# Cogito2012/OpenTAL

Hardware: AMD Instinct MI355X
Metric: clips/sec training step, 256-frame THUMOS14 clips (higher is better)
Workload: dtype bf16

## Files before the change

include/opental_hip.h:

```cpp
#ifndef OPENTAL_HIP_H
#define OPENTAL_HIP_H

#include <stdint.h>
#include <stddef.h>

#ifdef __cplusplus
extern "C" {
#endif

#define OTAL_ABI_VERSION 26

#define OTAL_E_NULL      (-1)
#define OTAL_E_SHAPE     (-2)
#define OTAL_E_ODD_C     (-3)
#define OTAL_E_BATCH     (-4)
#define OTAL_E_DTYPE     (-5)
#define OTAL_E_LEVELS    (-6)
#define OTAL_E_UNSUPPORTED (-7)

#define OTAL_F32  0
#define OTAL_BF16 1
#define OTAL_F16  2
#define OTAL_F64  3

#define OTAL_MAX_LEVELS 8

int otal_abi_version(void);
const char* otal_error_string(int code);
int otal_set_option(const char* name, int value);
int otal_get_option(const char* name, int dflt);
int otal_stream_wait(void* waiter, void* signaler);

int otal_bmp_fwd(const void* in, const float* seg, void* out,
                 int B, int C, int T, int N, int seg_batch, int dtype, void* stream);

int otal_bmp_bwd(const void* grad_out, const void* in, const float* seg, void* grad_in,
                 int B, int C, int T, int N, int seg_batch, int compat_ref_stride,
                 int dtype, void* stream);

int otal_bmp_fwd_levels(const void* in, const float* seg, void* out,
                        int B, int C, int nlev, const int* t_start, const int* n_start,
                        int dtype, void* stream);
int otal_bmp_bwd_levels(const void* grad_out, const void* in, const float* seg, void* grad_in,
                        int B, int C, int nlev, const int* t_start, const int* n_start,
                        int dtype, void* stream);

int otal_conv_half_storage(const int* geom, const int64_t* strides, int mode, int precision);
size_t otal_conv_workspace_bytes(const int* geom, int mode);

int otal_conv_fwd(const int* geom, const int64_t* strides, const float* x, const float* w,
                  const float* scale, const float* shift, float* y, int relu, int precision,
                  const void* prologue, void* ws, size_t ws_bytes, void* stream);

int otal_conv_dgrad(const int* geom, const int64_t* strides, const float* dy, const float* wt_packed,
                    float* dx, int accumulate, const float* out_mask, const float* out_scale,
                    int precision, const void* prologue, void* ws, size_t ws_bytes, void* stream);

int otal_conv_wgrad(const int* geom, const int64_t* strides, const float* x, const float* dy,
                    float* dw, int accumulate, int precision, const void* prologue, void* ws, size_t ws_bytes,
                    void* stream);

int otal_conv_fwd_pair(const int* geom, const int64_t* strides, const float* const* x, const float* const* w,
                       const float* const* scale, const float* const* shift, float* const* y, int relu, int precision,
                       const void* const* prologue, void* ws, size_t ws_bytes, void* stream);
int otal_conv_dgrad_pair(const int* geom, const int64_t* strides, const float* const* dy, const float* const* w,
                         float* const* dx, int precision, const void* const* prologue, void* ws, size_t ws_bytes, void* stream);
int otal_conv_wgrad_pair(const int* geom, const int64_t* strides, const float* const* x, const float* const* dy,
                         float* const* dw, int precision, void* ws, size_t ws_bytes, void* stream);

size_t otal_conv_prologue_bytes(const int* geom, const int64_t* strides, int mode, int precision);
size_t otal_conv_prologue_desc_bytes(void);
int otal_conv_prologue(const int* geom, const int64_t* strides, int mode, const float* w, int precision, void* region,
                       size_t region_bytes, void* host_desc, void* stream);
int otal_conv_prologue_batch(int n, const void* device_descs, const int* device_starts, int total_blocks, void* stream);

int otal_conv_defer_reduces(int on);
size_t otal_conv_deferred_end(void);
int otal_conv_deferred_count(void);
int otal_conv_flush_reduces(void* stream);

const char* otal_conv_last_kernel(void);

int otal_conv_pack_wt(const float* w, float* wt, int Cout, int Cin, int kvol, void* stream);

int otal_gn_relu_fwd(const float* x, const float* gamma, const float* beta, float* y, float* stats,
                     int B, int C, int T, int G, float eps, int relu, int nlev, const int* lev, void* stream);
int otal_gn_relu_bwd(const float* dy, int64_t dy_batch_stride, const float* x, const float* gamma, const float* beta,
                     const float* stats, float* dx, float* partial, int B, int C, int T, int G,
                     int relu, int nlev, const int* lev, void* stream);
int otal_gn_relu_fwd_pair(const float* const* x, const float* const* gamma, const float* const* beta, float* const* y,
                          float* const* stats, int B, int C, int T, int G, float eps, int relu, int nlev, const int* lev,
                          void* stream);
int otal_gn_relu_bwd_pair(const float* const* dy, const int64_t* dy_batch_stride, const float* const* x,
                          const float* const* gamma, const float* const* beta, const float* const* stats, float* const* dx,
                          float* const* partial, int B, int C, int T, int G, int relu, int nlev, const int* lev, void* stream);
int otal_sum_partials(int n_items, const float* const* partial, float* const* dst0, float* const* dst1,
                      float* const* dst2, const int* channels, const int* batches, void* stream);

const char* otal_layer_last_kernel(void);

int otal_maxpool3d_fwd(const int* geom, const int64_t* strides, const float* x, float* y,
                       unsigned char* argtap, void* stream);
int otal_maxpool3d_bwd(const int* geom, const int64_t* strides, const float* dy,
                       const unsigned char* argtap, float* dx, int accumulate,
                       const float* out_mask, const float* out_scale, void* stream);
size_t otal_maxpool3d_signbits_bytes(const int* geom, const int64_t* strides);
int otal_maxpool3d_fwd_signbits(const int* geom, const int64_t* strides, const float* x, float* y,
                                unsigned char* argtap, unsigned char* signbits, void* stream);
int otal_maxpool3d_bwd_signbits(const int* geom, const int64_t* strides, const float* dy, const unsigned char* argtap,
                                float* dx, int accumulate, const unsigned char* signbits, const float* out_scale,
                                void* stream);
int otal_maxpool3d_fwd_signbits_h(const int* geom, const int64_t* strides, const void* x_bf16, float* y,
                                  unsigned char* argtap, unsigned char* signbits, void* stream);
int otal_maxpool3d_bwd_signbits_h(const int* geom, const int64_t* strides, const float* dy, const unsigned char* argtap,
                                  void* dx_bf16, const unsigned char* signbits, const float* out_scale, void* stream);
int otal_maxpool3d_fwd_io(const int* geom, const int64_t* strides, const void* x, void* y, unsigned char* argtap,
                          unsigned char* signbits, int io, void* stream);
int otal_maxpool3d_bwd_io(const int* geom, const int64_t* strides, const void* dy, const unsigned char* argtap, void* dx,
                          int accumulate, const void* out_mask, const float* out_scale, const unsigned char* signbits, int io,
                          void* stream);
int otal_convert_storage(const void* src, int64_t src_bs, int64_t src_cs, void* dst, int64_t dst_bs, int64_t dst_cs,
                         int to_bf16, int B, int C, int P, void* stream);

int otal_head_outputs_fwd(int n_items, const int* channels, const int* modes, const float* const* raw, float* const* out,
                          float* const* unct, const float* scales, int B, int N, int nlev, const int* lev,
                          const float* level_strides, void* stream);
int otal_head_outputs_bwd(int n_items, const int* channels, const int* modes, const float* const* raw,
                          const float* const* out, const float* const* unct, const float* const* dout,
                          const float* const* dunct, float* const* draw, const float* scales, float* dscales, int B,
                          int N, int nlev, const int* lev, const float* level_strides, void* stream);

int otal_boundary_bce(const float* x, int64_t x_batch_stride, int64_t x_channel_stride, const float* mask,
                      int64_t mask_batch_stride, int64_t mask_row_stride, int mask_row0, int mask_step, float* terms,
                      float* dx, int B, int C, int T, void* stream);

int otal_boundary_finish(int n, const float* const* terms, const float* weights, const int* T, int B, float* out2, void* stream);
int otal_boundary_scale(int n, const float* const* dx, float* const* out, const float* weights, const int* C, const int* T,
                        int B, const float* g_start, const float* g_end, void* stream);

int otal_proposal_windows(const float* loc, float* seg, float* frame_seg, int B, int nlev,
                          const int* lev, float frame_num, void* stream);

int otal_decode_clips(const float* loc, const float* prop_loc, const float* priors, const float* conf,
                      const float* prop_conf, const float* center, const float* act, const float* prop_act,
                      const float* offsets, const float* fps, float* seg, float* score, float* unct,
                      float* actn, unsigned char* flag, int nclips, int A, int K, float clip_length,
                      float conf_thresh, void* stream);
int otal_decode_clips_ex(const float* loc, const float* prop_loc, const float* priors, const float* conf,
                         const float* prop_conf, const float* center, const float* act, const float* prop_act,
                         const float* offsets, const float* fps, float* seg, float* score, float* unct,
                         float* actn, unsigned char* flag, int nclips, int A, int K, float clip_length,
                         float conf_thresh, int score_fn, int first_class, void* stream);
int otal_softnms_classes(const float* seg, const float* score, const float* unct, const float* actn,
                         const unsigned char* flag, const int* clip_start, int nvideos, int max_clips,
                         int A, int K, float sigma, int top_k, float score_threshold, float* out,
                         int* counts, int* out_index, int out_cols, void* stream);
size_t otal_softnms_scratch_bytes(int total_clips, int max_clips, int A, int K);
int otal_softnms_classes_ws(const float* seg, const float* score, const float* unct, const float* actn,
                            const unsigned char* flag, const int* clip_start, int nvideos, int max_clips,
                            int A, int K, float sigma, int top_k, float score_threshold, float* out,
                            int* counts, int* out_index, int out_cols, void* scratch, size_t scratch_bytes,
                            int total_clips, void* stream);
int otal_detection_table(const float* rows, const int* counts, const double* durations, int V, int K, int top_k, int cols,
                         int drop_empty, int scoring, int* video, int* cls, double* seg, float* sup, double* known,
                         int* list_start, void* stream);

int otal_openmax_dist(const float* feat, int N, int rows_per_batch, int64_t sb, int64_t sr, int64_t sc, const float* mav,
                      int K, int D, const int* labels, float* dist, void* stream);
int otal_openmax_class_means(const float* feat, int N, int rows_per_batch, int64_t sb, int64_t sr, int64_t sc,
                             const int* labels, int K, int D, float* means, int* counts, void* stream);
int otal_openmax_probs(const float* logits, int64_t ldl, const float* feat, int N, int rows_per_batch, int64_t sb, int64_t sr,
                       int64_t sc, const float* mav, const float* wb, int K, int D, int R, float* probs, void* stream);
int otal_decode_clips_openmax(const float* loc, const float* prop_loc, const float* priors, const float* conf,
                              const float* prop_conf, const float* center, const float* offsets, const float* fps,
                              const float* feat, const float* prop_feat, const int64_t* feat_strides,
                              const int64_t* prop_feat_strides, const float* mav, const float* mav_prop, const float* wb,
                              const float* wb_prop, float* seg, float* score, float* unknown, unsigned char* flag,
                              int nclips, int A, int C, int first_class, int D, int R, int refined_feature,
                              float clip_length, float conf_thresh, void* stream);

int otal_head_convs_supported(int n_heads, int n_inputs, const int* in_idx, const int* cout, const int* ksize, int B, int C, int N);
int otal_head_convs_fwd(int n_heads, int n_inputs, const int* in_idx, const int* cout, const int* ksize,
                        const float* const* x, const float* const* w, const float* const* bias, float* const* y, int B, int C,
                        int N, int nlev, const int* lev, void* stream);
int otal_head_convs_bwd(int n_heads, int n_inputs, const int* in_idx, const int* cout, const int* ksize,
                        const float* const* x, const float* const* w, const float* const* dy, float* const* dx,
                        float* const* dw, float* const* db, int B, int C, int N, int nlev, const int* lev, void* stream);
int otal_head_convs_bwd_parts(int n_heads, int n_inputs, const int* in_idx, const int* cout, const int* ksize,
                        const float* const* x, const float* const* w, const float* const* dy, float* const* dx,
                        float* const* dw, float* const* db, int B, int C, int N, int nlev, const int* lev, int parts, void* stream);

int otal_rpl_head_fwd(const float* x, const float* centers, float* dist, int B, int C, int D, int N, void* stream);
int otal_rpl_head_bwd(const float* x, const float* centers, const float* g, float* dx, float* dcenters, int B, int C, int D,
                      int N, int parts, void* stream);

int otal_masked_scale_copy(const float* src, const int64_t* src_strides, const float* z, const int64_t* z_strides,
                           const float* scale, float* dst, const int64_t* dst_strides, int accumulate, int B, int C,
                           int T, int S, void* stream);

int otal_adam_flat(float* p, const float* g, float* m, float* v, int64_t n, float lr, float beta1,
                   float beta2, float eps, float weight_decay, int step, float grad_scale, void* stream);

int otal_adam_flat_dev(float* p, const float* g, float* m, float* v, int64_t n, float lr, float beta1,
                       float beta2, float eps, float weight_decay, const float* bias_corr, float grad_scale,
                       void* stream);

size_t otal_detection_loss_scratch_floats(int B, int K);
size_t otal_detection_loss_grad_floats(int B, int K, int C);
int otal_detection_loss(const float* loc, const float* conf, const float* prop_loc, const float* prop_conf,
                        const float* center, const float* act, const float* prop_act, const float* priors,
                        const float* gt, const unsigned char* gvalid, float* weight_accum, int B, int K, int C, int G,
                        float clip_length, float overlap_thresh, int ibm_active, int num_bins, float momentum,
                        int iou_aware, int cls_mode, float focal_alpha, float* losses, float* grads, float* scratch,
                        void* stream);

int otal_detection_loss_ex(const float* loc, const float* conf, const float* prop_loc, const float* prop_conf,
                           const float* center, const float* act, const float* prop_act, const float* priors,
                           const float* gt, const unsigned char* gvalid, float* weight_accum, int B, int K, int C, int G,
                           float clip_length, float overlap_thresh, int ibm_active, int num_bins, float momentum,
                           int iou_aware, int cls_mode, float focal_alpha, int reweight, float rw_gamma, float* losses,
                           float* grads, float* scratch, void* stream);
// ... 58 lines not shown
```

opental_amd/common/i3d_backbone.py:

```python
import torch
import torch.nn as nn
import torch.nn.functional as F
from torch.autograd import Function

from . import ops
from .layers import MaxPool3dSamePadding

ONE, THREE = (1, 1, 1), (3, 3, 3)
BN_EPS = 1e-3


class Unit3D(nn.Module):

    def __init__(self, in_channels, output_channels, kernel_shape=(1, 1, 1), stride=(1, 1, 1), padding=0,
                 activation_fn=F.relu, use_batch_norm=True, use_bias=False, padding_valid_spatial=False,
                 name='unit_3d'):
        super(Unit3D, self).__init__()
        if not use_batch_norm or use_bias or activation_fn is not F.relu or padding_valid_spatial or padding == -1:
            raise NotImplementedError("backbone Unit3D is conv(no bias) + BN + ReLU with SAME padding")
        self._output_channels = output_channels
        self._kernel_shape = tuple(kernel_shape)
        self._stride = tuple(stride)
        self.name = name
        self.conv3d = nn.Conv3d(in_channels, output_channels, self._kernel_shape, self._stride, padding=0, bias=False)
# ... 301 lines not shown
                    (y, arg), bits = ops.maxpool3d_forward(cur, k, s), None
                tape.append(("pool", k, s, cur, (arg, bits, half_grads.get(si, False)), cur_scale, None))
                cur, cur_scale = y, None
            else:
                _, w0, oc, _ = step
                B, _, T, H, W = cur.shape
                ctot = oc[0] + oc[2] + oc[4] + oc[5]
                o1, o13 = oc[1], oc[1] + oc[3]
                Z = torch.empty((B, o13 + ctot, T, H, W), dtype=cur.dtype, device=cur.device)
                h1, h2, Y = Z[:, :o1], Z[:, o1:o13], Z[:, o13:]
                c1, c2, c3 = oc[0], oc[0] + oc[2], oc[0] + oc[2] + oc[4]
                wf = _fused_weight(weights[w0 + 1].detach(), weights[w0 + 3].detach(), weights[w0].detach())
                scf, shf = _fused_affine(scale, shift, offs, w0)
                ops.conv_forward(cur, wf, ONE, ONE, scale=scf, shift=shf, relu=True, out=Z[:, :o13 + c1])
                lane = ops.branch_lane(cur.device)
                if lane.on:
                    lane.fork()
                    with lane:
                        ops.conv_forward(h2, weights[w0 + 4], THREE, ONE, scale=sc(w0 + 4), shift=sh(w0 + 4), relu=True,
                                         out=Y[:, c2:c3])
                        pm, argm = ops.maxpool3d_forward(cur, THREE, ONE, half_out=chain)
                        ops.conv_forward(pm, weights[w0 + 5], ONE, ONE, scale=sc(w0 + 5), shift=sh(w0 + 5), relu=True,
                                         out=Y[:, c3:])
                    ops.conv_forward(h1, weights[w0 + 2], THREE, ONE, scale=sc(w0 + 2), shift=sh(w0 + 2), relu=True,
                                     out=Y[:, c1:c2])
                    lane.join()
                else:
                    ops.conv_forward(h1, weights[w0 + 2], THREE, ONE, scale=sc(w0 + 2), shift=sh(w0 + 2), relu=True,
                                     out=Y[:, c1:c2])
                    ops.conv_forward(h2, weights[w0 + 4], THREE, ONE, scale=sc(w0 + 4), shift=sh(w0 + 4), relu=True,
                                     out=Y[:, c2:c3])
                    pm, argm = ops.maxpool3d_forward(cur, THREE, ONE, half_out=chain)
                    ops.conv_forward(pm, weights[w0 + 5], ONE, ONE, scale=sc(w0 + 5), shift=sh(w0 + 5), relu=True,
                                     out=Y[:, c3:])
                out_scale = _cat_cached(_OUT_SCALE, scale, w0, [sc(w0), sc(w0 + 2), sc(w0 + 4), sc(w0 + 5)])
                tape.append(("mixed", w0, (c1, c2, c3), cur, h1, h2, pm, argm, Y, cur_scale, (wf, o1, o13), out_scale))
                cur, cur_scale = Y, out_scale
            if name in endpoints:
                if cur.dtype == BF and name not in raw_out:
                    ends = si + 1 == len(plan) or not _step_half_ok(plan[si + 1], cur.shape, weights)
                    if need_grad or ends:
                        leave_half()
                        found[name] = (cur, len(tape))
                    else:
                        found[name] = (ops.convert_storage(cur, torch.float32), len(tape))
                else:
                    found[name] = (cur, len(tape))
                hooks = ops.STEP.endpoint_hooks
                hook = hooks.get(name) if hooks else None
                if hook is not None:
                    hook(found[name][0])
        missing = [e for e in endpoints if e not in found]
        if missing:
            raise RuntimeError(f"unknown endpoints {missing}")
        ctx.tape = tape
        ctx.meta = (scale, offs, [found[e][1] for e in endpoints], len(weights), x.requires_grad)
        ctx.weights = weights
        ctx.outs = [found[e][0] for e in endpoints]
        return tuple(ctx.outs)

    @staticmethod
    def backward(ctx, *douts):
        tape, weights = ctx.tape, ctx.weights
        scale, offs, out_pos, nw, need_dx = ctx.meta
        sc = lambda i: scale[offs[i]:offs[i + 1]]
        dws = [None] * nw
        pending = {}
        for pos, g, z in zip(out_pos, douts, ctx.outs):
            if g is not None:
                pending.setdefault(pos, []).append((g, z, tape[pos - 1][-1]))
        zg = {}

        def out_grad_buffer(p, shape, like):
            if p >= 1 and tape[p - 1][0] == "mixed":
                o13 = tape[p - 1][10][2]
                B, ct, T, H, W = shape
                buf = torch.empty((B, o13 + ct, T, H, W), dtype=like.dtype, device=like.device)
                zg[p] = buf
                return buf[:, o13:]
            return torch.empty(tuple(shape), dtype=like.dtype, device=like.device)

        side = ops.side_wgrads(weights[0].device)
        in_slots = True
        dcur = None
        cloned = True
        mixed_pos = [p for p in range(1, len(tape) + 1) if tape[p - 1][0] == "mixed"]
        tail_below = min(mixed_pos) if mixed_pos and not need_dx else 0
        for pos in range(len(tape), 0, -1):
            if pos == tail_below - 1 and not any(pending.get(q) for q in range(1, pos + 1)):
                ops.late_mark([weights[st[1]] for st in tape[:pos] if st[0] == "conv"])
            for g, z, zs in pending.pop(pos, ()):
                ops.join_pending(g)
                dense = g.dim() == 5 and (g.shape[4] == 1 or g.stride(4) == 1) and (g.shape[3] == 1 or g.stride(3) == g.shape[4])
                if zs is not None and not dense:
                    g = g.contiguous()
                if dcur is None:
                    if zs is not None:
                        dcur = out_grad_buffer(pos, g.shape, g)
                        ops.masked_scale_copy(g, z, zs, dcur)
                    elif tape[pos - 1][0] == "mixed":
                        dcur = out_grad_buffer(pos, g.shape, g)
                        dcur.copy_(g)
                    else:
                        dcur = g.contiguous()
                        cloned = False
                elif zs is not None:
                    ops.masked_scale_copy(g, z, zs, dcur, accumulate=True)
                else:
                    if not cloned:
                        dcur, cloned = dcur.clone(), True
                    dcur.add_(g)
            if dcur is None:
                continue
            step = tape[pos - 1]
            first = pos == 1
            if step[0] == "cvt":
                _, xh, _, _ = step
                dcur = ops.convert_storage(dcur.contiguous(), xh.dtype, out=out_grad_buffer(pos - 1, xh.shape, xh))
            elif step[0] == "conv":
                _, wi, k, s, xin, y, in_scale, _ = step
                slot = ops.grad_slot(weights[wi])
                in_slots = in_slots and slot is not None
                if first and not need_dx:
                    side.issue()
                    dws[wi] = ops.conv_wgrad(xin, dcur, weights[wi].shape, k, s, out=slot)
                else:
                    dws[wi] = side.wgrad(xin, dcur, weights[wi].shape, k, s, out=slot)
                if first and not need_dx:
                    dcur = None
                else:
                    dcur = ops.conv_dgrad(dcur, weights[wi], xin.shape, k, s, out=out_grad_buffer(pos - 1, xin.shape, xin),
                                          out_mask=xin if in_scale is not None else None, out_scale=in_scale)
                side.flush()
                ops.grads_ready([(weights[wi], dws[wi])])
            elif step[0] == "pool":
                _, k, s, xin, (arg, bits, grad_half), in_scale, _ = step
                if dcur.dtype == torch.bfloat16:
                    masked = in_scale is not None and bits is not None
                    dcur = ops.maxpool3d_backward(dcur, arg, xin.shape, k, s, out=out_grad_buffer(pos - 1, xin.shape, xin),
                                                  out_scale=in_scale if masked else None, out_signbits=bits if masked else None)
                elif grad_half:
                    dcur = ops.maxpool3d_backward(dcur, arg, xin.shape, k, s, out_scale=in_scale, out_signbits=bits, half_out=True)
                else:
                    dcur = ops.maxpool3d_backward(dcur, arg, xin.shape, k, s, out=out_grad_buffer(pos - 1, xin.shape, dcur),
                                                  out_mask=xin if (in_scale is not None and bits is None) else None,
                                                  out_scale=in_scale, out_signbits=bits)
            else:
                _, w0, (c1, c2, c3), xin, h1, h2, pm, argm, Y, in_scale, (wf, o1, o13), _ = step
                Zg = zg.pop(pos)
                dY = Zg[:, o13:]
                dX = out_grad_buffer(pos - 1, xin.shape, xin)
                xm = xin if in_scale is not None else None
                sl = (slice(0, c1), slice(c1, c2), slice(c2, c3), slice(c3, Y.shape[1]))
                for a, b, hid, sli, dst in ((w0 + 1, w0 + 2, h1, sl[1], Zg[:, :o1]), (w0 + 3, w0 + 4, h2, sl[2], Zg[:, o1:o13])):
                    g = dY[:, sli]
                    slot = ops.grad_slot(weights[b])
                    in_slots = in_slots and slot is not None
                    dws[b] = side.wgrad(hid, g, weights[b].shape, THREE, ONE, out=slot)
                    ops.conv_dgrad(g, weights[b], hid.shape, THREE, ONE, out=dst, out_mask=hid, out_scale=sc(a))
                gf = Zg[:, :o13 + c1]
                slot = ops.grad_slot(wf)
                in_slots = in_slots and slot is not None
                dwf = side.wgrad(xin, gf, wf.shape, ONE, ONE, out=slot)
                dws[w0 + 1], dws[w0 + 3], dws[w0] = dwf[:o1], dwf[o1:o13], dwf[o13:]
                ops.conv_dgrad(gf, wf, xin.shape, ONE, ONE, out=dX, out_mask=xm, out_scale=in_scale)
                g3 = dY[:, sl[3]]
                slot = ops.grad_slot(weights[w0 + 5])
                in_slots = in_slots and slot is not None
                dws[w0 + 5] = side.wgrad(pm, g3, weights[w0 + 5].shape, ONE, ONE, out=slot)
                dpm = ops.conv_dgrad(g3, weights[w0 + 5], pm.shape, ONE, ONE)
                ops.maxpool3d_backward(dpm, argm, xin.shape, THREE, ONE, out=dX, accumulate=True,
                                       out_mask=xm, out_scale=in_scale)
                dcur = dX
                side.flush()
                ops.grads_ready([(weights[w0 + q], dws[w0 + q]) for q in range(6)])
        side.node_end(in_slots)
        ctx.tape = None
        ctx.outs = None
        dx = dcur if need_dx else None
        return (dx, None, None, None, None, None) + tuple(dws)
```

opental_amd/common/ops.py:

```python
import bisect
import ctypes
import os
import warnings

import torch

from .. import _lib as L
from .conv_geom import make_geom

_WORKSPACE = {}
WORKSPACE_BYTES = 192 << 20
WORKSPACE_TOTAL = 512 << 20

CONV_PROFILE = None

CONV_PRECISION = 0
HALF_STORAGE = os.environ.get("OTAL_HALF_STORAGE", "1") != "0"
HALF_ACT_DIRECT = os.environ.get("OTAL_HALF_ACT_DIRECT", "0") != "0"
HALF_CHAIN = os.environ.get("OTAL_HALF_CHAIN", "1") != "0"


def _prof_begin():
    if CONV_PROFILE is None:
        return None
    ev = torch.cuda.Event(enable_timing=True)
    ev.record()
    return ev


def _prof_end(ev, mode, g, problems=1):
    if ev is None:
        return
    end = torch.cuda.Event(enable_timing=True)
    end.record()
    B, Cin, Cout = g[0], g[1], g[2]
    flops = 2.0 * B * Cout * g[6] * g[7] * g[8] * Cin * g[9] * g[10] * g[11] * problems
    CONV_PROFILE.append((mode, flops, ev, end))


def workspace(device, side=False):
    key = (device.type, device.index, side)
    ws = _WORKSPACE.get(key)
    if ws is None:
        ws = torch.empty(WORKSPACE_TOTAL, dtype=torch.uint8, device=device)
        _WORKSPACE[key] = ws
    return ws


class StepState:
    def __init__(self):
        self.lanes = None
        self.slots = None
        self.ready = None
        self.defer_join = False
        self.pending_sums = None
        self.prologues = None
        self.late_weights = None
        self.endpoint_hooks = None
        self.early_results = {}
        self.pending_joins = {}
        self.defer = False
        self.defer_owner = None
        self.ws_cursor = [0, 0, 0, 0]
        self.ws_index = 0
        self.stream = None

    def begin_backward(self, slots, ready, early):
        if self.slots is not None:
            raise RuntimeError("a trainer's backward is already running in this process (one at a time)")
        self.slots, self.ready = slots, ready
        self.defer_join = early
        self.pending_sums = [] if early else None
        defer_reduces(early and CONV_PROFILE is None)

    def end_backward(self):
        self.defer_join = False
        defer_reduces(False)
        flush_pending_sums()
        self.pending_sums = self.slots = self.ready = None

    def reset(self, failed_capture=False):
        self.prologues = None
        self.slots = self.ready = self.pending_sums = None
        self.defer_join = False
        self.late_weights = None
        self.lanes = None
        for sd in _SIDES.values():
            sd.pending.clear()
            sd.keep.clear()
        self.early_results.clear()
        self.pending_joins.clear()
        try:
            defer_reduces(False)
        except RuntimeError:
            if not failed_capture:
                raise


STEP = StepState()


class issue_on:
    __slots__ = ("ws", "stream", "ctx", "saved")

    def __init__(self, ws_index, stream, current=False):
        self.ws, self.stream = ws_index, stream
        self.ctx = torch.cuda.stream(stream) if current else None

    def __enter__(self):
        s = STEP
        self.saved = (s.ws_index, s.stream, L.STREAM_OVERRIDE)
        s.ws_index, s.stream, L.STREAM_OVERRIDE = self.ws, self.stream, self.stream.cuda_stream
        if self.ctx is not None:
            self.ctx.__enter__()
        return self

    def __exit__(self, *exc):
        if self.ctx is not None:
            self.ctx.__exit__(*exc)
        STEP.ws_index, STEP.stream, L.STREAM_OVERRIDE = self.saved
        return False


def _ws_args(device):
    s = STEP
    ws = workspace(device, s.ws_index)
    cur = s.ws_cursor[s.ws_index]
    return ctypes.c_void_p(ws.data_ptr() + cur), ctypes.c_size_t(min(ws.numel() - cur, WORKSPACE_BYTES))


def defer_reduces(on):
    if not on:
        flush_reduces()
    L.check(L.lib().otal_conv_defer_reduces(int(bool(on))), "otal_conv_defer_reduces")
    STEP.defer = bool(on)


def _stream_wait(stream):
    L.check(L.lib().otal_stream_wait(L.stream(), ctypes.c_void_p(stream.cuda_stream)), "otal_stream_wait")


def flush_reduces(wait=True):
    s = STEP
    own = s.defer_owner
    if s.defer and own is not None:
        stream = own[1]
        if stream is None:
            L.check(L.lib().otal_conv_flush_reduces(L.stream()), "otal_conv_flush_reduces")
        else:
            L.check(L.lib().otal_conv_flush_reduces(ctypes.c_void_p(stream.cuda_stream)), "otal_conv_flush_reduces")
            if wait and L.STREAM_OVERRIDE != stream.cuda_stream:
                _stream_wait(stream)
    s.defer_owner = None
    s.ws_cursor[0] = s.ws_cursor[1] = 0


def _after_wgrad(device):
    s = STEP
    lib = L.lib()
    lib.otal_conv_deferred_end.restype = ctypes.c_size_t
    end = int(lib.otal_conv_deferred_end())
    if end:
        i = s.ws_index
        s.defer_owner = (i, s.stream)
        s.ws_cursor[i] = (end - workspace(device, i).data_ptr() + 255) & ~255
        if s.ws_cursor[i] > WORKSPACE_TOTAL - WORKSPACE_BYTES:
            flush_reduces()


WGRAD_STREAM = os.environ.get("OTAL_WGRAD_STREAM", "1") != "0"
_SIDES = {}


class LanePlan:

    def __init__(self, side_stream):
        self.entries = []
        self.pool = None
        self.cur = None
        self.side = side_stream
        self.keep = []
        self.mark_event = None

    def begin_main(self):
        g = torch.cuda.CUDAGraph()
        if self.pool is None:
            self.pool = torch.cuda.graph_pool_handle()
        g.capture_begin(pool=self.pool, capture_error_mode="relaxed")
        self.cur = g
# ... 539 lines not shown


class GradSlots:

    def __init__(self, flat, grad, offsets, numels):
        self.base, self.n, self.grad = flat.data_ptr(), flat.numel(), grad
        self.offsets, self.numels = list(offsets), list(numels)
        self.written = [False] * len(self.offsets)

    def reset(self):
        self.written = [False] * len(self.offsets)

    def take(self, w):
        if w.dtype != torch.float32 or not w.is_contiguous():
            return None
        off = w.data_ptr() - self.base
        if off < 0 or off % 4 or off // 4 + w.numel() > self.n:
            return None
        off //= 4
        i = bisect.bisect_left(self.offsets, off)
        if i == len(self.offsets) or self.offsets[i] != off:
            return None
        j, cur, end = i, off, off + w.numel()
        while j < len(self.offsets) and cur < end:
            cur += self.numels[j]
            j += 1
        if cur != end:
            return None
        if any(self.written[i:j]):
            flush_pending_sums()
            flush_reduces()
            return None
        for q in range(i, j):
            self.written[q] = True
        return self.grad[off:end].view(w.shape)

    def release(self, w):
        off = (w.data_ptr() - self.base) // 4
        i = bisect.bisect_left(self.offsets, off)
        j, cur, end = i, off, off + w.numel()
        while j < len(self.offsets) and cur < end:
            self.written[j] = False
            cur += self.numels[j]
            j += 1


def grads_ready(pairs):
    flush_reduces()
    cb = STEP.ready
    if cb is not None:
        cb(pairs)


def grad_slot(w):
    slots = STEP.slots
    return slots.take(w) if slots is not None and "OTAL_NO_GRAD_SLOTS" not in os.environ else None


def conv_wgrad(x, dy, w_shape, k, s, spatial_valid=False, levels=None, out=None, accumulate=False):
    k, s = _k3(k), _k3(s)
    if levels is not None:
        levels = tuple(levels)
    Cout = w_shape[0]
    half_dy = dy.dtype == torch.bfloat16
    half_x = x.dtype == torch.bfloat16
    if not (half_x or x.dtype == torch.float32) or not (half_dy or dy.dtype == torch.float32) or (half_x and not half_dy):
        raise RuntimeError("conv_wgrad: float32 x with a float32 or bfloat16 dy, or both bfloat16")
    g, ga, sa, pkey, _ = _plan(2, x, dy, Cout, k, s, levels, spatial_valid, "x", "dy")
    if out is None:
        if accumulate:
            raise RuntimeError("accumulate needs an existing buffer")
        out = torch.empty(tuple(w_shape), dtype=torch.float32, device=x.device)
    if not out.is_contiguous():
        raise RuntimeError("dw must be contiguous")
    st = STEP
    if st.defer and (accumulate or (st.defer_owner is not None and st.defer_owner[0] != st.ws_index)):
        flush_reduces()
    wsp, wsn = _ws_args(x.device)
    ev = _prof_begin()
    prec = int(CONV_PRECISION)
    pre = _prologue(2, ga, sa, pkey, x, prec) if (half_x or not half_dy) else None
    L.check(L.lib().otal_conv_wgrad(ga, sa, L.ptr(x), L.ptr(dy), L.ptr(out),
                                    int(accumulate), prec | (4 if half_dy else 0) | (8 if half_x else 0), pre, wsp, wsn, L.stream()),
            "otal_conv_wgrad")
    if st.defer:
        _after_wgrad(x.device)
    _prof_end(ev, "wgrad", g)
    return out


PAIR_LAUNCHES = os.environ.get("OTAL_PAIR_LAUNCHES", "1") != "0"
_VP2 = ctypes.c_void_p * 2


def _pp(a, b):
    return _VP2(a.data_ptr() if a is not None else None, b.data_ptr() if b is not None else None)


def _same_layout(a, b):
    return a.shape == b.shape and a.stride() == b.stride() and a.dtype == b.dtype and a.device == b.device


def conv_forward_pair(xs, ws, k, s, shifts=None, levels=None):
    k, s = _k3(k), _k3(s)
    if levels is not None:
        levels = tuple(levels)
    if not PAIR_LAUNCHES or not (int(CONV_PRECISION) & 1) or not _same_layout(xs[0], xs[1]) or ws[0].shape != ws[1].shape:
        return None
    if xs[0].dtype != torch.float32 or not (ws[0].is_contiguous() and ws[1].is_contiguous()):
        return None
    Cout = ws[0].shape[0]
    outn = _out_positions(xs[0], Cout, k, s, levels, False)
    ys = [torch.empty((x.shape[0], Cout) + outn[:1], dtype=x.dtype, device=x.device) for x in xs]
    g, ga, sa, pkey, _ = _plan(0, xs[0], ys[0], Cout, k, s, levels, False, "x", "y")
    prec = int(CONV_PRECISION)
    pres = [_prologue(0, ga, sa, pkey, w, prec) for w in ws]
    if (pres[0] is None) != (pres[1] is None):
        return None
    wsp, wsn = _ws_args(xs[0].device)
    ev = _prof_begin()
    sh = None if shifts is None or shifts[0] is None else _pp(shifts[0], shifts[1])
    rc = L.lib().otal_conv_fwd_pair(ga, sa, _pp(*xs), _pp(*ws), None, sh, _pp(*ys), 0, prec,
                                    None if pres[0] is None else _VP2(pres[0].value, pres[1].value), wsp, wsn, L.stream())
    if rc == L.E_UNSUPPORTED:
        return None
    L.check(rc, "otal_conv_fwd_pair")
    _prof_end(ev, "fwd", g, 2)
    return ys


def conv_dgrad_pair(dys, ws, x_shape, k, s, levels=None):
    k, s = _k3(k), _k3(s)
    if levels is not None:
        levels = tuple(levels)
    if not PAIR_LAUNCHES or not (int(CONV_PRECISION) & 1) or not _same_layout(dys[0], dys[1]) or ws[0].shape != ws[1].shape:
        return None
    if dys[0].dtype != torch.float32 or not (ws[0].is_contiguous() and ws[1].is_contiguous()):
        return None
    Cout = ws[0].shape[0]
    outs = [torch.empty(tuple(x_shape), dtype=dy.dtype, device=dy.device) for dy in dys]
    g, ga, sa, pkey, _ = _plan(1, outs[0], dys[0], Cout, k, s, levels, False, "dx", "dy")
    prec = int(CONV_PRECISION) | 2
    pres = [_prologue(1, ga, sa, pkey, w, prec) for w in ws]
    if (pres[0] is None) != (pres[1] is None):
        return None
    wsp, wsn = _ws_args(dys[0].device)
    ev = _prof_begin()
    rc = L.lib().otal_conv_dgrad_pair(ga, sa, _pp(*dys), _pp(*ws), _pp(*outs), prec,
                                      None if pres[0] is None else _VP2(pres[0].value, pres[1].value), wsp, wsn, L.stream())
    if rc == L.E_UNSUPPORTED:
        return None
    L.check(rc, "otal_conv_dgrad_pair")
    _prof_end(ev, "dgrad", g, 2)
    return outs


def conv_wgrad_pair(xs, dys, w_shape, k, s, levels=None, outs=(None, None)):
    k, s = _k3(k), _k3(s)
    if levels is not None:
        levels = tuple(levels)
    if not PAIR_LAUNCHES or not (int(CONV_PRECISION) & 1) or not _same_layout(xs[0], xs[1]) or not _same_layout(dys[0], dys[1]):
        return None
    if xs[0].dtype != torch.float32 or dys[0].dtype != torch.float32:
        return None
    Cout = w_shape[0]
    g, ga, sa, pkey, _ = _plan(2, xs[0], dys[0], Cout, k, s, levels, False, "x", "dy")
    outs = [o if o is not None else torch.empty(tuple(w_shape), dtype=torch.float32, device=xs[0].device) for o in outs]
    if not (outs[0].is_contiguous() and outs[1].is_contiguous()):
        return None
    st = STEP
    if st.defer and st.defer_owner is not None and st.defer_owner[0] != st.ws_index:
        flush_reduces()
    wsp, wsn = _ws_args(xs[0].device)
    ev = _prof_begin()
    rc = L.lib().otal_conv_wgrad_pair(ga, sa, _pp(*xs), _pp(*dys), _pp(*outs), int(CONV_PRECISION), wsp, wsn, L.stream())
    if rc == L.E_UNSUPPORTED:
        return None
    L.check(rc, "otal_conv_wgrad_pair")
    if st.defer:
        _after_wgrad(xs[0].device)
    _prof_end(ev, "wgrad", g, 2)
    return outs


def gn_relu_forward_pair(xs, gammas, betas, groups=32, eps=1e-5, relu=True, levels=None, outs=None):
    if not PAIR_LAUNCHES or not _same_layout(xs[0], xs[1]) or not xs[0].is_contiguous():
        return None
    L.require_device(*xs, *gammas, *betas)
    B, C, T = xs[0].shape
    nlev, lev = _lev_arg(levels)
    stats = [torch.empty((B, groups, nlev, 2), dtype=torch.float32, device=x.device) for x in xs]
    if outs is not None:
        st0, st1 = _dest_strides(outs[0], B, C, T), _dest_strides(outs[1], B, C, T)
        if st0 != st1:
            return None
        rc = L.lib().otal_gn_relu_fwd_pair_to(_pp(*xs), _pp(*gammas), _pp(*betas), _pp(*outs), ctypes.c_int64(st0[0]),
                                              ctypes.c_int64(st0[1]), _pp(*stats), B, C, T, groups, ctypes.c_float(eps), int(relu),
                                              nlev, lev, L.stream())
        if rc == L.E_UNSUPPORTED:
            return None
        L.check(rc, "otal_gn_relu_fwd_pair_to")
        return list(zip(outs, stats))
    ys = [torch.empty_like(x) for x in xs]
    rc = L.lib().otal_gn_relu_fwd_pair(_pp(*xs), _pp(*gammas), _pp(*betas), _pp(*ys), _pp(*stats), B, C, T, groups,
                                       ctypes.c_float(eps), int(relu), nlev, lev, L.stream())
    if rc == L.E_UNSUPPORTED:
        return None
    L.check(rc, "otal_gn_relu_fwd_pair")
    return list(zip(ys, stats))


def _lev_arg(levels):
    if levels is None or len(levels) <= 2:
        return 1, None
    return len(levels) - 1, L.int_array(list(levels))


def _dest_strides(out, B, C, T):
    if tuple(out.shape) != (B, C, T) or out.dtype != torch.float32 or not out.is_cuda or (T > 1 and out.stride(2) != 1):
        raise RuntimeError("gn_relu_forward: `out` must be a float32 (B,C,T) GPU tensor with dense positions")
    cs = out.stride(1) if C > 1 else T
    return (out.stride(0) if B > 1 else cs * C), cs


def gn_relu_forward(x, gamma, beta, groups=32, eps=1e-5, relu=True, levels=None, out=None):
    L.require_device(x, gamma, beta)
    B, C, T = x.shape
    nlev, lev = _lev_arg(levels)
    stats = torch.empty((B, groups, nlev, 2), dtype=torch.float32, device=x.device)
    if out is not None:
        bs, cs = _dest_strides(out, B, C, T)
        L.check(L.lib().otal_gn_relu_fwd_to(L.ptr(x), L.ptr(gamma), L.ptr(beta), L.ptr(out), ctypes.c_int64(bs), ctypes.c_int64(cs),
                                            L.ptr(stats), B, C, T, groups, ctypes.c_float(eps), int(relu), nlev, lev, L.stream()),
                "otal_gn_relu_fwd_to")
        return out, stats
    y = torch.empty_like(x)
    L.check(L.lib().otal_gn_relu_fwd(L.ptr(x), L.ptr(gamma), L.ptr(beta), L.ptr(y), L.ptr(stats), B, C, T, groups,
                                     ctypes.c_float(eps), int(relu), nlev, lev, L.stream()), "otal_gn_relu_fwd")
    return y, stats


def pyramid_merge_forward(p0, p1, total, up):
    L.require_device(p0, p1)
    B, C, t0 = p0.shape
    if tuple(p1.shape) != (B, C, t0 // 2):
        raise RuntimeError("pyramid_merge_forward: p1 must have half of p0's positions")
    packed = torch.empty((B, C, total), dtype=torch.float32, device=p0.device)
    frame = torch.empty((B, C, t0 * up), dtype=torch.float32, device=p0.device)
    L.check(L.lib().otal_pyramid_merge_fwd(L.ptr(p0), L.ptr(p1), L.ptr(packed), L.ptr(frame), B, C, t0, total, up, L.stream()),
            "otal_pyramid_merge_fwd")
    return packed, frame


def pyramid_merge_backward(da, db, dframe, dnext, t0, up):
    L.require_device(da, dframe)
    B, C, T = da.shape
    dp0 = torch.empty((B, C, t0), dtype=torch.float32, device=da.device)
    dp1 = torch.empty((B, C, t0 // 2), dtype=torch.float32, device=da.device)
    for t in (db, dnext):
        if t is not None:
            L.require_device(t)
    L.check(L.lib().otal_pyramid_merge_bwd(L.ptr(da), _opt(db), L.ptr(dframe), _opt(dnext), L.ptr(dp0), L.ptr(dp1), B, C, t0, T, up,
                                           L.stream()), "otal_pyramid_merge_bwd")
    return dp0, dp1


def gn_relu_backward(dy, x, gamma, beta, stats, groups=32, relu=True, levels=None, bias=None):
    B, C, T = x.shape
    if dy.dim() != 3 or tuple(dy.shape) != (B, C, T) or dy.stride(2) != 1 or dy.stride(1) != T or dy.stride(0) < C * T:
        dy = dy.contiguous()
    L.require_device(x, gamma, beta, stats)
    if not dy.is_cuda:
        raise RuntimeError("opental_amd ops run on the GPU only")
    nlev, lev = _lev_arg(levels)
    dx = torch.empty_like(x)
    partial = torch.empty((B, 3, C), dtype=torch.float32, device=x.device)
    L.check(L.lib().otal_gn_relu_bwd(L.ptr(dy), ctypes.c_int64(dy.stride(0)), L.ptr(x), L.ptr(gamma), L.ptr(beta), L.ptr(stats),
                                     L.ptr(dx), L.ptr(partial), B, C, T, groups, int(relu), nlev, lev, L.stream()),
            "otal_gn_relu_bwd")
    return (dx,) + _gn_sums(partial, gamma, beta, bias, C, B)


def _gn_sums(partial, gamma, beta, bias, C, B):
    s = STEP
    if s.pending_sums is not None and bias is not None and s.slots is not None:
        slots = [s.slots.take(t) for t in (gamma, beta, bias)]
        if all(sl is not None for sl in slots):
            s.pending_sums.append((partial, tuple(sl.data_ptr() for sl in slots), C, B))
            return slots[0], slots[1], slots[2]
        for t, sl in zip((gamma, beta, bias), slots):
            if sl is not None:
                s.slots.release(t)
    red = partial.sum(0)
    return red[0], red[1], red[2]


def gn_relu_backward_pair(dys, xs, gammas, betas, stats, groups=32, relu=True, levels=None, biases=(None, None)):
    if not PAIR_LAUNCHES or not _same_layout(xs[0], xs[1]):
        return None
    B, C, T = xs[0].shape
    dys = list(dys)
    for i in range(2):
        dy = dys[i]
        if dy.dim() != 3 or tuple(dy.shape) != (B, C, T) or dy.stride(2) != 1 or dy.stride(1) != T or dy.stride(0) < C * T:
            dys[i] = dy.contiguous()
        if not dys[i].is_cuda:
# ... 687 lines not shown
```

opental_amd/csrc/conv_gemm.hip:

```cpp
#include "common.h"
#include "conv_index.h"
#include "conv_select.h"
#include <cstdlib>
#include <cstring>
#include <mutex>
#include <type_traits>

#ifndef OTAL_CONV_PART
#define OTAL_CONV_PART 0
#endif

#include "conv1a_tile.h"
namespace otal_conv {
struct ConvArgs;
__attribute__((visibility("hidden"))) int launch_half(int mode, int kernel, int cw, ConvArgs& a, void* ws, size_t ws_bytes, hipStream_t st);
}

namespace {

constexpr int NT = 256;
enum { EPI_RELU = 1, EPI_ACCUM = 2, NO_STORE = 8, NO_BARRIER = 16, EPI_NPAD8 = 32 };

typedef float f32x16 __attribute__((ext_vector_type(16)));

}
struct otal_conv::ConvArgs {
    ConvGeom g;
    ConvFastDiv fd;
    const float* x;
    const float* w;
    const float* dy;
    float* out;
    const float* scale;
    const float* shift;
    float* slab;
    const float* zero;
    const int2* tab;
    const float* emask;
    const float* escale;
    int M, N, K;
    int splits, k_per_split;
    int flags;
    int a_vec4;
    int prec;
    const int2* ctab;
    const unsigned short* wp;
    unsigned src_bytes;
    unsigned wp_bytes;
    int Kp;
    const int2* ptab;
    unsigned dy_bytes;
    int P;
    int w_natural;
    unsigned out_bytes, slab_bytes;
    const void* pre;
    int half;
    int pair;
    const float* x2;
    const float* dy2;
    float* out2;
    const float* scale2;
    const float* shift2;
    const unsigned short* wp2;
    float* slab2;
    const void* pre2;
    const float* w2;
    int xhalf, mhalf;
};
namespace {
using otal_conv::ConvArgs;

__device__ __attribute__((aligned(16))) float g_zero4[4] = {0.f, 0.f, 0.f, 0.f};

__device__ __forceinline__ float ld_or_zero(const float* base, int64_t off, bool ok) {
    const float* p = ok ? base + off : g_zero4;
    return *p;
}

struct Anchor {
    const float* base;
    unsigned mask;
};
__device__ __forceinline__ Anchor anchor_of_output(const ConvGeom& g, const float* x, const PosDec& o, bool live) {
    const int t0 = o.t * g.st - g.pt, h0 = o.h * g.sh - g.ph, w0 = o.w * g.sw - g.pw;
    int lo, up;
    level_bounds(g, o.t, g.Ti, lo, up);
    unsigned m = 0;
#pragma unroll
    for (int d = 0; d < 8; ++d) {
        m |= (unsigned)(d < g.kt && t0 + d >= lo && t0 + d < up) << d;
        m |= (unsigned)(d < g.kh && (unsigned)(h0 + d) < (unsigned)g.Hi) << (8 + d);
        m |= (unsigned)(d < g.kw && (unsigned)(w0 + d) < (unsigned)g.Wi) << (16 + d);
    }
    Anchor r;
    r.base = x + ((int64_t)o.b * g.x_bs + ((int64_t)t0 * g.Hi + h0) * g.Wi + w0);
    r.mask = live ? m : 0u;
    return r;
}
__device__ __forceinline__ Anchor anchor_of_input(const ConvGeom& g, const float* dy, const PosDec& i, bool live) {
    const int tn = i.t + g.pt, hn = i.h + g.ph, wn = i.w + g.pw;
    const int st1 = g.st - 1, sh1 = g.sh - 1, sw1 = g.sw - 1;
    int lo, up;
    level_bounds(g, i.t, g.Ti, lo, up);
    if (g.nlev <= 1) { lo = 0; up = g.To; }
    unsigned m = 0;
#pragma unroll
    for (int d = 0; d < 8; ++d) {
        const int vt = tn - d, vh = hn - d, vw = wn - d;
        m |= (unsigned)(d < g.kt && vt >= 0 && (vt & st1) == 0 && (vt >> st1) >= lo && (vt >> st1) < up) << d;
        m |= (unsigned)(d < g.kh && vh >= 0 && (vh & sh1) == 0 && (vh >> sh1) < g.Ho) << (8 + d);
        m |= (unsigned)(d < g.kw && vw >= 0 && (vw & sw1) == 0 && (vw >> sw1) < g.Wo) << (16 + d);
    }
    Anchor r;
    r.base = dy + ((int64_t)i.b * g.y_bs + ((int64_t)(tn >> st1) * g.Ho + (hn >> sh1)) * g.Wo + (wn >> sw1));
    r.mask = live ? m : 0u;
    return r;
}
__device__ __forceinline__ bool tap_ok(unsigned mask, int dt, int dh, int dw) {
    return ((mask >> dt) & (mask >> (8 + dh)) & (mask >> (16 + dw)) & 1u) != 0;
}
__device__ __forceinline__ float ld_sel(const float* p, bool ok, const float* zero) {
    const float* q = ok ? p : zero;
    return *q;
}

typedef short bf16x8 __attribute__((ext_vector_type(8)));
struct Words4 { unsigned a, b, c, d; };
struct Words2 { unsigned a, b; };
__device__ __forceinline__ unsigned wrap_add(unsigned a, unsigned b) {
    unsigned r = a + b;
    asm volatile("" : "+v"(r));
    return r;
}
typedef __bf16 hw_bf16x2 __attribute__((ext_vector_type(2)));
typedef float hw_f32x2 __attribute__((ext_vector_type(2)));
__device__ __forceinline__ unsigned cvt_pk_bf16(float lo, float hi) {
    const hw_f32x2 f = {lo, hi};
    return __builtin_bit_cast(unsigned, __builtin_convertvector(f, hw_bf16x2));
}

__device__ __forceinline__ unsigned pair_lo(unsigned ch_a, unsigned ch_b) { return __builtin_amdgcn_perm(ch_b, ch_a, 0x05040100u); }
__device__ __forceinline__ unsigned pair_hi(unsigned ch_a, unsigned ch_b) { return __builtin_amdgcn_perm(ch_b, ch_a, 0x07060302u); }
__device__ __forceinline__ bool bf16_pos(unsigned bits16) { return bits16 - 1u < 0x7f80u; }
__device__ __forceinline__ unsigned bf16_relu_mask2(unsigned w) {
    return (bf16_pos(w & 0xffffu) ? 0x0000ffffu : 0u) | (bf16_pos(w >> 16) ? 0xffff0000u : 0u);
}
__device__ __forceinline__ float bf16lo_f32(unsigned w) { return __uint_as_float(w << 16); }
__device__ __forceinline__ float bf16hi_f32(unsigned w) { return __uint_as_float(w & 0xffff0000u); }

__device__ __forceinline__ unsigned pack_bf16x2(float lo, float hi) {
    unsigned a = __float_as_uint(lo), b = __float_as_uint(hi);
    a += 0x7fffu + ((a >> 16) & 1u);
    b += 0x7fffu + ((b >> 16) & 1u);
    return (a >> 16) | (b & 0xffff0000u);
}

template <int MODE, int WM, int WN>
__device__ __forceinline__ void store_acc_slow(const ConvArgs& a, const f32x16 (&acc)[WM][WN], int m0, int n0, int wm0, int wn0,
                                               int lane, int split) {
    const ConvGeom& g = a.g;
    const ConvFastDiv& fd = a.fd;
#pragma unroll
    for (int j = 0; j < WN; ++j) {
        const int n = n0 + wn0 + j * 32 + (lane & 31);
        if (n >= a.N) continue;
        int64_t nbase = 0;
        if (a.splits == 1) {
            if constexpr (MODE == MODE_FWD) nbase = conv_out_offset(g, dec_pos_fd(n, fd.To, fd.Ho, fd.Wo), 0);
// ... 1566 lines not shown
    int item = 0;
#pragma unroll 1
    while (item + 1 < DEFER_MAX && b.start[item + 1] <= (int)blockIdx.x) ++item;
    const DeferItem& d = b.it[item];
    const int wg = (int)blockIdx.x - b.start[item];
    const int lane = threadIdx.x & 63, q = threadIdx.x >> 6;
    const int64_t base = ((int64_t)wg * 64 + lane) * 4;
    const bool live = base < d.total;
    const int per = (d.splits + 3) / 4;
    const int s_lo = q * per, s_hi = min(d.splits, s_lo + per);
    float4 acc = make_float4(0.f, 0.f, 0.f, 0.f);
    if (live) {
        for (int s0 = s_lo; s0 < s_hi; s0 += 8) {
            float4 tmp[8];
#pragma unroll
            for (int u = 0; u < 8; ++u) {
                const int sidx = min(s0 + u, s_hi - 1);
                tmp[u] = *reinterpret_cast<const float4*>(d.slab + (int64_t)sidx * d.total + base);
            }
#pragma unroll
            for (int u = 0; u < 8; ++u)
                if (s0 + u < s_hi) { acc.x += tmp[u].x; acc.y += tmp[u].y; acc.z += tmp[u].z; acc.w += tmp[u].w; }
        }
    }
    if (q > 0) part[q - 1][lane] = acc;
    __syncthreads();
    if (q > 0 || !live) return;
    const float4 p1 = part[0][lane], p2 = part[1][lane], p3 = part[2][lane];
    float r[4] = {(acc.x + p1.x) + (p2.x + p3.x), (acc.y + p1.y) + (p2.y + p3.y), (acc.z + p1.z) + (p2.z + p3.z), (acc.w + p1.w) + (p2.w + p3.w)};
#pragma unroll
    for (int e = 0; e < 4; ++e) {
        const int64_t idx = base + e;
        float v = r[e];
        int64_t off = idx;
        if (d.flags & EPI_NPAD8) {
            const int m = (int)(idx / d.N), n = (int)(idx - (int64_t)m * d.N);
            if ((n & 7) >= d.kw) continue;
            off = (int64_t)m * ((d.N >> 3) * d.kw) + (n >> 3) * d.kw + (n & 7);
        }
        if (d.flags & EPI_ACCUM) v += d.out[off];
        d.out[off] = v;
    }
}

static int flush_deferred(hipStream_t st) {
    std::lock_guard<std::recursive_mutex> lock(g_defer.mu);
    if (g_defer.n == 0) return 0;
    int blocks = 0;
    for (int i = 0; i <= DEFER_MAX; ++i) {
        g_defer.batch.start[i] = blocks;
        if (i < g_defer.n) blocks += (int)((g_defer.batch.it[i].total + 255) / 256);
    }
    hipLaunchKernelGGL(splitk_reduce_batch_kernel, dim3((unsigned)blocks), dim3(256), 0, st, g_defer.batch);
    g_defer.n = 0;
    return otal_launch_status();
}

template <int MODE, bool H = false>
static int launch_splitk_reduce(const ConvArgs& a, hipStream_t st) {
    static_assert(!(H && MODE == MODE_WGRAD), "weight gradients are fp32");
    const int64_t total = (int64_t)a.M * a.N;
    const bool v4 = (total % 4 == 0) && (((uintptr_t)a.slab & 15) == 0);
    if (MODE == MODE_WGRAD) {
        std::lock_guard<std::recursive_mutex> lock(g_defer.mu);
        g_defer.last_end = 0;
        if (g_defer.on && v4 && total <= (1 << 23)) {
            if (g_defer.n == DEFER_MAX)
                if (int e = flush_deferred(st)) return e;
            DeferItem& d = g_defer.batch.it[g_defer.n++];
            d.slab = a.slab; d.out = a.out; d.total = total; d.splits = a.splits; d.flags = a.flags; d.N = a.N; d.kw = a.g.kw;
            g_defer.last_end = reinterpret_cast<uintptr_t>(a.slab + (int64_t)a.splits * total);
            return 0;
        }
    }
    if (v4 && a.splits >= 16 && total <= (1 << 21)) {
        const int blocks = (int)((total / 4 + 63) / 64);
        hipLaunchKernelGGL((splitk_reduce_tall_kernel<MODE, H>), dim3(blocks), dim3(256), 0, st, a);
        return otal_launch_status();
    }
    const int64_t work = v4 ? total / 4 : total;
    const int blocks = (int)((work + 255) / 256 < 4096 ? (work + 255) / 256 : 4096);
    if (v4) hipLaunchKernelGGL((splitk_reduce_kernel<MODE, 4, H>), dim3(blocks), dim3(256), 0, st, a);
    else hipLaunchKernelGGL((splitk_reduce_kernel<MODE, 1, H>), dim3(blocks), dim3(256), 0, st, a);
    return otal_launch_status();
}

__global__ __launch_bounds__(256) void pack_wt_kernel(const float* __restrict__ w, float* __restrict__ wt,
                                                      int Cout, int Cin, int kvol) {
    const int64_t total = (int64_t)Cout * Cin * kvol;
    for (int64_t idx = (int64_t)blockIdx.x * 256 + threadIdx.x; idx < total; idx += (int64_t)gridDim.x * 256) {
        const int r = (int)(idx % kvol);
        const int64_t q = idx / kvol;
        const int co = (int)(q % Cout), ci = (int)(q / Cout);
        wt[idx] = w[((int64_t)co * Cin + ci) * kvol + r];
    }
}

int fill_geom(ConvGeom& g, const int* d) {
    g.B = d[0]; g.Cin = d[1]; g.Cout = d[2];
    g.Ti = d[3]; g.Hi = d[4]; g.Wi = d[5];
    g.To = d[6]; g.Ho = d[7]; g.Wo = d[8];
    g.kt = d[9]; g.kh = d[10]; g.kw = d[11];
    g.st = d[12]; g.sh = d[13]; g.sw = d[14];
    g.pt = d[15]; g.ph = d[16]; g.pw = d[17];
    g.nlev = d[18];
    for (int i = 0; i <= OTAL_CONV_MAX_LEVELS; ++i) g.lev[i] = d[19 + i];
    const int v[] = {g.B, g.Cin, g.Cout, g.Ti, g.Hi, g.Wi, g.To, g.Ho, g.Wo, g.kt, g.kh, g.kw, g.st, g.sh, g.sw};
    for (int x : v) if (x <= 0) return OTAL_E_SHAPE;
    if (g.pt < 0 || g.ph < 0 || g.pw < 0) return OTAL_E_SHAPE;
    if (g.kt > 8 || g.kh > 8 || g.kw > 8) return OTAL_E_UNSUPPORTED;
    if (g.st > 2 || g.sh > 2 || g.sw > 2) return OTAL_E_UNSUPPORTED;
    if (g.nlev > 1) {
        if (g.nlev > OTAL_CONV_MAX_LEVELS || g.Hi != 1 || g.Wi != 1 || g.st != 1 || g.Ti != g.To) return OTAL_E_LEVELS;
        if (g.lev[0] != 0 || g.lev[g.nlev] != g.Ti) return OTAL_E_LEVELS;
        for (int i = 0; i < g.nlev; ++i) if (g.lev[i + 1] <= g.lev[i]) return OTAL_E_LEVELS;
    }
    if ((int64_t)g.Cin * g.Ti * g.Hi * g.Wi >= (1LL << 31) || (int64_t)g.Cout * g.To * g.Ho * g.Wo >= (1LL << 31) ||
        (int64_t)g.Cout * g.Cin * g.kt * g.kh * g.kw >= (1LL << 31)) return OTAL_E_SHAPE;
    if ((int64_t)g.B * g.To * g.Ho * g.Wo >= (1LL << 31) || (int64_t)g.B * g.Ti * g.Hi * g.Wi >= (1LL << 31) ||
        (int64_t)g.Cin * g.kt * g.kh * g.kw >= (1LL << 31) || (int64_t)g.Cout * g.kt * g.kh * g.kw >= (1LL << 31)) return OTAL_E_SHAPE;
    return 0;
}

static const float* zero_word_address() {
    static const float* z = nullptr;
    if (!z) {
        void* p = nullptr;
        if (hipGetSymbolAddress(&p, HIP_SYMBOL(g_zero4)) == hipSuccess) z = static_cast<const float*>(p);
    }
    return z;
}

template <int MODE>
static void set_epilogue_extents(ConvArgs& a) {
    const ConvGeom& g = a.g;
    int64_t out;
    if (MODE == MODE_FWD) out = 4 * ((int64_t)(g.B - 1) * g.y_bs + (int64_t)(g.Cout - 1) * g.y_cs + conv_out_positions(g));
    else if (MODE == MODE_DGRAD) out = 4 * ((int64_t)(g.B - 1) * g.x_bs + (int64_t)(g.Cin - 1) * g.x_cs + conv_in_positions(g));
    else out = 4 * (int64_t)g.Cout * g.Cin * conv_kvol(g);
    a.out_bytes = (out > 0 && out < (int64_t)0xfffffff0u) ? (unsigned)out : 0u;
    const int64_t slab = 4 * (int64_t)a.splits * a.M * a.N;
    a.slab_bytes = (a.splits > 1 && slab < (int64_t)0xfffffff0u) ? (unsigned)slab : 0u;
}

struct DirectArgs {
    ConvArgs c;
    const unsigned short* wp;
    int C, Ktot;
    unsigned wp_bytes;
};

template <int BM, int MODE, int BNP, int WN, int PX = 48, int MINW = 1, bool XPF2 = false, bool H = false>
__global__ __launch_bounds__(BNP * 2 / WN, MINW) void conv3_direct_kernel(const DirectArgs d) {
    constexpr int DNT = BNP * 2 / WN;
    constexpr int WM = BM / 32, PA = 304, SPAN_MAX = BNP + (H ? 56 : 52);
    constexpr int ESZ = H ? 2 : 4, XV = H ? 8 : 4;
    static_assert(PX == 48 || PX == 32, "position pitch");
    constexpr int A_PIECES = (BM * 18 + DNT - 1) / DNT;
    constexpr int X_ITEMS = (SPAN_MAX / XV + 1) * 8;
    constexpr int X_ITERS = (X_ITEMS + DNT - 1) / DNT;
    extern __shared__ __attribute__((aligned(16))) unsigned char dsm[];
    unsigned char* const smA0 = dsm;
    unsigned char* const smX0 = dsm + 2 * BM * PA;
    const unsigned char* const smZero = dsm + 2 * BM * PA + 2 * SPAN_MAX * PX;
    if (threadIdx.x < 4) reinterpret_cast<unsigned*>(dsm + 2 * BM * PA + 2 * SPAN_MAX * PX)[threadIdx.x] = 0u;
    auto smA = [&](int buf) { return smA0 + buf * (BM * PA); };
    auto smX = [&](int buf) { return smX0 + buf * (SPAN_MAX * PX); };
    const ConvArgs& a = d.c;
    const ConvGeom& g = a.g;
    const ConvFastDiv& fd = a.fd;
    const int tid = threadIdx.x, lane = tid & 63;
    const int wave = __builtin_amdgcn_readfirstlane(tid >> 6);
    const TileId tile = xcd_tile(true);
    const int m0 = tile.y * BM, n0 = tile.x * BNP;
    const int W = g.Wi, HW = g.Hi * g.Wi;
    const int XO = H ? W + 2 : W + 1;
    const int span = BNP + XO + W + 1, nq = (span + XV - 1) / XV;
    const float* src = MODE == MODE_FWD ? a.x : a.dy;
    const int64_t sbs = MODE == MODE_FWD ? g.x_bs : g.y_bs, scs = MODE == MODE_FWD ? g.x_cs : g.y_cs;
    const auto rs = __builtin_amdgcn_make_buffer_rsrc(const_cast<float*>(src), 0, (int)a.src_bytes, 0x00020000);
    const auto rw = __builtin_amdgcn_make_buffer_rsrc(const_cast<unsigned short*>(d.wp), 0, (int)d.wp_bytes, 0x00020000);
    const uint32_t bsm = fd_div(fd.P, (uint32_t)n0);
    const int p0 = n0 - (int)(bsm * fd.P.d);
    const unsigned tile_off = (unsigned)(((int64_t)bsm * sbs + p0 - XO) * ESZ);

    unsigned tmask[WN], hwmask[WN];
#pragma unroll
    for (int j = 0; j < WN; ++j) {
        const int nl = n0 + (wave * WN + j) * 32 + (lane & 31);
        const PosDec o = dec_pos_fd(nl < a.N ? nl : 0, fd.To, fd.Ho, fd.Wo);
        const bool live = nl < a.N;
        tmask[j] = 0; hwmask[j] = 0;
#pragma unroll
        for (int dt = 0; dt < 3; ++dt) tmask[j] |= (unsigned)(live && (unsigned)(o.t + dt - 1) < (unsigned)g.Ti) << dt;
#pragma unroll
        for (int dh = 0; dh < 3; ++dh)
#pragma unroll
            for (int dw = 0; dw < 3; ++dw)
                hwmask[j] |= (unsigned)((unsigned)(o.h + dh - 1) < (unsigned)g.Hi && (unsigned)(o.w + dw - 1) < (unsigned)g.Wi) << (dh * 3 + dw);
    }
    unsigned xvo[X_ITERS];
    int xlds[X_ITERS];
#pragma unroll
    for (int i = 0; i < X_ITERS; ++i) {
        const int item = tid + DNT * i;
        const int cp = item & 7, q = item >> 3;
        const bool used = q < nq;
        xvo[i] = used ? tile_off + (unsigned)((2 * cp * scs + XV * q) * ESZ) : 0xffffffffu;
        if constexpr (H)
            xlds[i] = PX == 48 ? (8 * q) * PX + cp * 4 : (8 * q) * PX + ((((cp >> 2) ^ q) & 1) << 4) + (cp & 3) * 4;
        else
            xlds[i] = PX == 48 ? (4 * q) * PX + cp * 4
                               : (4 * q) * PX + ((((cp >> 2) ^ (q >> 1)) & 1) << 4) + (cp & 3) * 4;
    }
    unsigned avo[A_PIECES];
#pragma unroll
    for (int j = 0; j < A_PIECES; ++j) {
        const int p = tid + DNT * j;
        avo[j] = (unsigned)(((m0 + p / 18) * d.Ktot * 2) + (p % 18) * 16);
    }
    unsigned rxs[XPF2 ? 2 : 1][X_ITERS][2][4];
    Words4 ra[A_PIECES];
    const int nsteps = (d.C >> 4) * 3;
    auto load_x = [&](int s, auto SET) {
        unsigned (&rx)[X_ITERS][2][4] = rxs[decltype(SET)::value];
        const int cb = s / 3, dt = s - cb * 3;
        const unsigned so = (unsigned)(((int64_t)cb * 16 * scs + (int64_t)(dt - 1) * HW) * ESZ);
#pragma unroll
        for (int i = 0; i < X_ITERS; ++i) {
            const unsigned vo = xvo[i] == 0xffffffffu ? a.src_bytes : xvo[i] + so;
#pragma unroll
            for (int h = 0; h < 2; ++h) {
                const Words4 v = __builtin_bit_cast(Words4, __builtin_amdgcn_raw_buffer_load_b128(rs, vo, h ? (int)(scs * ESZ) : 0, 0));
                rx[i][h][0] = v.a; rx[i][h][1] = v.b; rx[i][h][2] = v.c; rx[i][h][3] = v.d;
            }
        }
    };
    auto load_a = [&](int s) {
#pragma unroll
        for (int j = 0; j < A_PIECES; ++j)
            if ((BM * 18) % DNT == 0 || tid + DNT * j < BM * 18)
                ra[j] = __builtin_bit_cast(Words4, __builtin_amdgcn_raw_buffer_load_b128(rw, avo[j], s * 288, 0));
    };
    auto store = [&](int buf, int s, auto SET) {
        unsigned (&rx)[X_ITERS][2][4] = rxs[decltype(SET)::value];
        const int cb = s / 3, dt = s - cb * 3;
        const unsigned so = (unsigned)(((int64_t)cb * 16 * scs + (int64_t)(dt - 1) * HW) * ESZ);
#pragma unroll
        for (int i = 0; i < X_ITERS; ++i) {
            if (xvo[i] == 0xffffffffu) continue;
            const unsigned vo = xvo[i] + so;
            const bool neg = vo >= 0xfffffff0u;
            if (__builtin_amdgcn_ballot_w64(neg) != 0ull) {
#pragma unroll
                for (int h = 0; h < 2; ++h) {
                    if constexpr (H) {
#pragma unroll
                        for (int e = 1; e < 4; ++e) {
                            const unsigned v = __builtin_amdgcn_raw_buffer_load_b32(rs, neg ? wrap_add(vo, 4u * e) : a.src_bytes,
                                                                                     h ? (int)(scs * ESZ) : 0, 0);
                            rx[i][h][e] = neg ? v : rx[i][h][e];
                        }
                    } else {
#pragma unroll
                        for (int e = 1; e < 4; ++e) {
                            const unsigned v = __builtin_amdgcn_raw_buffer_load_b32(rs, neg ? wrap_add(vo, 4u * e) : a.src_bytes,
                                                                                     h ? (int)(scs * 4) : 0, 0);
                            rx[i][h][e] = neg ? v : rx[i][h][e];
                        }
                    }
                }
            }
            if constexpr (H) {
#pragma unroll
                for (int e = 0; e < 8; ++e)
                    *reinterpret_cast<unsigned*>(smX(buf) + xlds[i] + e * PX) =
                        (e & 1) ? pair_hi(rx[i][0][e >> 1], rx[i][1][e >> 1]) : pair_lo(rx[i][0][e >> 1], rx[i][1][e >> 1]);
            } else {
#pragma unroll
                for (int e = 0; e < 4; ++e)
                    *reinterpret_cast<unsigned*>(smX(buf) + xlds[i] + e * PX) =
                        cvt_pk_bf16(__uint_as_float(rx[i][0][e]), __uint_as_float(rx[i][1][e]));
            }
        }
#pragma unroll
        for (int j = 0; j < A_PIECES; ++j) {
            const int p = tid + DNT * j;
            if ((BM * 18) % DNT == 0 || p < BM * 18) *reinterpret_cast<Words4*>(smA(buf) + (p / 18) * PA + (p % 18) * 16) = ra[j];
        }
    };

    f32x16 acc[WM][WN];
#pragma unroll
    for (int i = 0; i < WM; ++i)
#pragma unroll
        for (int j = 0; j < WN; ++j)
#pragma unroll
            for (int r = 0; r < 16; ++r) acc[i][j][r] = 0.f;

    using Set0 = std::integral_constant<int, 0>;
    using Set1 = std::integral_constant<int, XPF2 ? 1 : 0>;
    load_x(0, Set0{});
    load_a(0);
    store(0, 0, Set0{});
    if constexpr (XPF2) load_x(nsteps > 1 ? 1 : 0, Set1{});
    __syncthreads();
    const int xpos = wave * WN * 32 + (lane & 31) + XO;
    const int xrow = xpos * PX + (lane >> 5) * 16;
    auto frag_a = [&](int buf, int g9, int i) -> bf16x8 {
        return *reinterpret_cast<const bf16x8*>(smA(buf) + (i * 32 + (lane & 31)) * PA + g9 * 32 + (lane >> 5) * 16);
    };
    auto frag_b = [&](int buf, int dt, int g9, int j) -> bf16x8 {
        const int dh = g9 / 3, dw = g9 - dh * 3;
        const unsigned char* src;
        if (PX == 48) {
            src = smX(buf) + xrow + (j * 32 + (dh - 1) * W + (dw - 1)) * PX;
        } else {
            const int p = xpos + j * 32 + (dh - 1) * W + (dw - 1);
            src = smX(buf) + p * PX + ((((lane >> 5) ^ (p >> 3)) & 1) << 4);
        }
        const bool ok = ((tmask[j] >> dt) & 1u) && ((hwmask[j] >> g9) & 1u);
        return *reinterpret_cast<const bf16x8*>(ok ? src : smZero);
    };
    auto kstep = [&](int s, auto CUR, auto OTHER) {
        const int buf = s & 1;
        const int dt = s % 3;
        const int sn = s + 1 < nsteps ? s + 1 : s;
        const int sx = XPF2 ? (s + 2 < nsteps ? s + 2 : nsteps - 1) : sn;
        bf16x8 avA[WM], bvA[WN], avB[WM], bvB[WN];
#pragma unroll
        for (int i = 0; i < WM; ++i) avA[i] = frag_a(buf, 0, i);
#pragma unroll
        for (int j = 0; j < WN; ++j) bvA[j] = frag_b(buf, dt, 0, j);
#pragma unroll
        for (int g9 = 0; g9 < 9; ++g9) {
            if (g9 == 0) load_x(sx, OTHER);
            if (g9 == 1) load_a(sn);
            bf16x8 (&av)[WM] = (g9 & 1) ? avB : avA;
            bf16x8 (&bv)[WN] = (g9 & 1) ? bvB : bvA;
            bf16x8 (&avn)[WM] = (g9 & 1) ? avA : avB;
            bf16x8 (&bvn)[WN] = (g9 & 1) ? bvA : bvB;
            int n = 0;
#pragma unroll
            for (int i = 0; i < WM; ++i)
#pragma unroll
                for (int j = 0; j < WN; ++j) {
                    acc[i][j] = __builtin_amdgcn_mfma_f32_32x32x16_bf16(av[i], bv[j], acc[i][j], 0, 0, 0);
                    if (g9 < 8) {
                        if (n < WM) avn[n] = frag_a(buf, g9 + 1, n);
                        else if (n < WM + WN) bvn[n - WM] = frag_b(buf, dt, g9 + 1, n - WM);
                    }
                    ++n;
                }
            if (WM * WN < WM + WN && g9 < 8) {
#pragma unroll
                for (int r = WM * WN; r < WM + WN; ++r) {
                    if (r < WM) avn[r] = frag_a(buf, g9 + 1, r);
                    else bvn[r - WM] = frag_b(buf, dt, g9 + 1, r - WM);
                }
            }
            __builtin_amdgcn_sched_barrier(0);
        }
        store(buf ^ 1, sn, CUR);
        __syncthreads();
    };
    if constexpr (XPF2) {
        for (int s = 0; s < nsteps; s += 2) {
            kstep(s, Set1{}, Set0{});
            if (s + 1 < nsteps) kstep(s + 1, Set0{}, Set1{});
        }
    } else {
        for (int s = 0; s < nsteps; ++s) kstep(s, Set0{}, Set0{});
    }
    if ((MODE == MODE_FWD && a.half) || (MODE == MODE_DGRAD && a.xhalf)) {
        constexpr int PT = BNP * 2 + 16;
        static_assert(BM * PT + BM * 8 <= 2 * BM * PA + 2 * SPAN_MAX * PX, "staging tile fits in the operand buffers");
        unsigned char* tile = dsm;
        float* rows = reinterpret_cast<float*>(dsm + BM * PT);
        __syncthreads();
        for (int r = tid; r < BM; r += DNT) {
            const int m = m0 + r;
            if constexpr (MODE == MODE_FWD) {
                rows[2 * r] = (m < a.M && a.scale) ? a.scale[m] : 1.f;
                rows[2 * r + 1] = (m < a.M && a.shift) ? a.shift[m] : 0.f;
            } else {
                rows[2 * r] = (m < a.M && a.escale) ? a.escale[m] : 1.f;
                rows[2 * r + 1] = 0.f;
            }
        }
        __syncthreads();
        const bool relu = MODE == MODE_FWD && (a.flags & EPI_RELU) != 0;
#pragma unroll
        for (int i = 0; i < WM; ++i)
#pragma unroll
            for (int j = 0; j < WN; ++j) {
                const int nl = (wave * WN + j) * 32 + (lane & 31);
#pragma unroll
                for (int r = 0; r < 16; ++r) {
                    const int lr = i * 32 + (r & 3) + 8 * (r >> 2) + 4 * (lane >> 5);
                    float v = acc[i][j][r] * rows[2 * lr] + rows[2 * lr + 1];
                    if (relu) v = fmaxf(v, 0.f);
                    *reinterpret_cast<unsigned short*>(tile + lr * PT + nl * 2) = (unsigned short)(cvt_pk_bf16(v, 0.f) & 0xffffu);
                }
            }
        __syncthreads();
        unsigned short* yh = reinterpret_cast<unsigned short*>(a.out);
        const unsigned short* mk = MODE == MODE_DGRAD ? reinterpret_cast<const unsigned short*>(a.emask) : nullptr;
        const int64_t ocs = MODE == MODE_FWD ? g.y_cs : g.x_cs;
        const int64_t ybase = (int64_t)bsm * (MODE == MODE_FWD ? g.y_bs : g.x_bs) + p0;
        constexpr int U = 4;
        for (int p0 = tid; p0 < BM * (BNP / 8); p0 += U * DNT) {
            int64_t off[U];
            bool ok[U];
            Words4 m4[U];
#pragma unroll
            for (int u = 0; u < U; ++u) {
                const int p = p0 + u * DNT;
                const int row = p / (BNP / 8), q = p - row * (BNP / 8);
                ok[u] = p < BM * (BNP / 8) && m0 + row < a.M && n0 + q * 8 < a.N;
                off[u] = ok[u] ? ybase + (int64_t)(m0 + row) * ocs + q * 8 : 0;
                if (mk) m4[u] = *reinterpret_cast<const Words4*>(mk + off[u]);
            }
#pragma unroll
            for (int u = 0; u < U; ++u) {
                if (!ok[u]) continue;
                const int p = p0 + u * DNT;
                const int row = p / (BNP / 8), q = p - row * (BNP / 8);
                Words4 v = *reinterpret_cast<const Words4*>(tile + row * PT + q * 16);
                if (mk) {
                    v.a &= bf16_relu_mask2(m4[u].a); v.b &= bf16_relu_mask2(m4[u].b);
                    v.c &= bf16_relu_mask2(m4[u].c); v.d &= bf16_relu_mask2(m4[u].d);
                }
                *reinterpret_cast<Words4*>(yh + off[u]) = v;
            }
        }
        return;
    }
    store_acc<MODE, WM, WN, BM>(a, acc, m0, n0, 0, wave * WN * 32, lane, 0, reinterpret_cast<float*>(smA(0)));
}

template <int MODE>
__global__ __launch_bounds__(256) void pack_direct_kernel(unsigned* __restrict__ wp, const float* __restrict__ w, int M, int Mpad,
                                                          int C, int natural, FastDiv fh) {
    pack_direct_body<MODE>(wp, w, M, Mpad, C, natural, blockIdx.x, gridDim.x, fh);
}

constexpr int C1_NPL = 9, C1_NR = 9, C1_NC = 104, C1_PITCH = C1_NC * 8;
constexpr int C1_BNP = C1_TT * C1_TR * C1_WO, C1_NT = C1_BNP * 2, C1_PA = 80, C1_STEPS = 49;

struct Conv1aArgs {
    ConvArgs c;
    const unsigned short* wp;
};

__global__ __launch_bounds__(256) void pack_conv1a_kernel(unsigned* __restrict__ wp, const float* __restrict__ w, int M, int Mpad) {
    const int pairs = Mpad * C1_STEPS * 16;
    for (int p = blockIdx.x * 256 + threadIdx.x; p < pairs; p += gridDim.x * 256) {
        const int m = p / (C1_STEPS * 16), r = p - m * (C1_STEPS * 16), s = r >> 4, k = (r & 15) * 2;
        float v[2];
#pragma unroll
        for (int i = 0; i < 2; ++i) {
            const int kk = k + i, dw = kk >> 2, ci = kk & 3;
            v[i] = (m < M && dw < 7 && ci < 3) ? w[((int64_t)m * 3 + ci) * 343 + s * 7 + dw] : 0.f;
        }
        wp[p] = cvt_pk_bf16(v[0], v[1]);
    }
}

__global__ __launch_bounds__(C1_NT) void conv1a_direct_fwd_kernel(const Conv1aArgs d) {
    constexpr int BM = 64, WM = 2;
    __shared__ __attribute__((aligned(16))) unsigned char patch[C1_NPL * C1_NR * C1_PITCH];
    __shared__ __attribute__((aligned(16))) unsigned char smA[2][BM * C1_PA];
    const ConvArgs& a = d.c;
    const ConvGeom& g = a.g;
    const int tid = threadIdx.x, lane = tid & 63;
    const int wave = __builtin_amdgcn_readfirstlane(tid >> 6);
    const int tiles_h = g.Ho / C1_TR, tiles_t = g.To / C1_TT;
    int bid = blockIdx.x;
    if ((gridDim.x & 7) == 0) bid = (bid & 7) * (gridDim.x >> 3) + (bid >> 3);
    const int th = bid % tiles_h; bid /= tiles_h;
    const int tt0 = bid % tiles_t;
    const int b = bid / tiles_t;
    const int to0 = tt0 * C1_TT, ho0 = th * C1_TR;
    const int m0 = blockIdx.y * BM;
    const float* xb = a.x + (int64_t)b * g.x_bs;

    constexpr int ITEMS = C1_NPL * C1_NR * 24, ITERS = (ITEMS + C1_NT - 1) / C1_NT;
#pragma unroll
    for (int it0 = 0; it0 < ITERS; it0 += 3) {
        float4 v[3][3];
        int lds_off[3];
#pragma unroll
        for (int u = 0; u < 3; ++u) {
            const int item = tid + C1_NT * (it0 + u);
            const int pl = item / (C1_NR * 24), rem = item - pl * (C1_NR * 24), rr = rem / 24, q = rem - rr * 24;
            const int ti = 2 * to0 - g.pt + pl, hi = 2 * ho0 - g.ph + rr;
            const bool ok = it0 + u < ITERS && item < ITEMS && (unsigned)ti < (unsigned)g.Ti && (unsigned)hi < (unsigned)g.Hi;
            lds_off[u] = item < ITEMS && it0 + u < ITERS ? (pl * C1_NR + rr) * C1_PITCH + (4 * q + 2) * 8 : -1;
            const float* src = xb + ((int64_t)(ok ? ti : 0) * g.Hi + (ok ? hi : 0)) * g.Wi + 4 * q;
#pragma unroll
            for (int ci = 0; ci < 3; ++ci)
                v[u][ci] = ok ? *reinterpret_cast<const float4*>(src + ci * g.x_cs) : make_float4(0.f, 0.f, 0.f, 0.f);
        }
#pragma unroll
        for (int u = 0; u < 3; ++u) {
            if (lds_off[u] < 0) continue;
            uint2* dst = reinterpret_cast<uint2*>(patch + lds_off[u]);
            dst[0] = make_uint2(cvt_pk_bf16(v[u][0].x, v[u][1].x), cvt_pk_bf16(v[u][2].x, 0.f));
            dst[1] = make_uint2(cvt_pk_bf16(v[u][0].y, v[u][1].y), cvt_pk_bf16(v[u][2].y, 0.f));
            dst[2] = make_uint2(cvt_pk_bf16(v[u][0].z, v[u][1].z), cvt_pk_bf16(v[u][2].z, 0.f));
            dst[3] = make_uint2(cvt_pk_bf16(v[u][0].w, v[u][1].w), cvt_pk_bf16(v[u][2].w, 0.f));
        }
    }
    for (int i = tid; i < C1_NPL * C1_NR * 8; i += C1_NT) {
        const int row = i >> 3, e = i & 7;
        *reinterpret_cast<uint2*>(patch + row * C1_PITCH + (e < 2 ? e : 96 + e) * 8) = make_uint2(0u, 0u);
    }
    const auto rw = __builtin_amdgcn_make_buffer_rsrc(const_cast<unsigned short*>(d.wp), 0,
                                                      (int)((int64_t)gridDim.y * BM * C1_STEPS * 64), 0x00020000);
    const unsigned avo = (unsigned)(((m0 + (tid >> 2)) * C1_STEPS) * 64 + (tid & 3) * 16);
    Words4 rq[7];
    auto load_a = [&](int s) { if (tid < 256) rq[s % 7] = __builtin_bit_cast(Words4, __builtin_amdgcn_raw_buffer_load_b128(rw, avo, s * 64, 0)); };
    auto store_a = [&](int s) { if (tid < 256) *reinterpret_cast<Words4*>(smA[s & 1] + (tid >> 2) * C1_PA + (tid & 3) * 16) = rq[s % 7]; };
    load_a(0);
    load_a(1);
#pragma unroll
    for (int s = 2; s < 7; ++s) load_a(s);
    store_a(0);
    store_a(1);
    load_a(7);
    load_a(8);
    __syncthreads();

    const int nl = wave * 32 + (lane & 31);
    const int lt = nl / (C1_TR * C1_WO), lrem = nl - lt * (C1_TR * C1_WO), lr = lrem / C1_WO, wo = lrem - lr * C1_WO;
    const int xbase = ((2 * lt) * C1_NR + 2 * lr) * C1_PITCH + (2 * wo) * 8 + (lane >> 5) * 16;
    const int abase = (lane & 31) * C1_PA + (lane >> 5) * 16;
    f32x16 acc[WM][1];
#pragma unroll
    for (int i = 0; i < WM; ++i)
#pragma unroll
        for (int r = 0; r < 16; ++r) acc[i][0][r] = 0.f;
    bf16x8 av[2][2][WM], bv[2][2];
    auto read_ops = [&](int set, int s) {
        const int dt = s / 7, dh = s - dt * 7;
        const unsigned char* xrow = patch + xbase + (dt * C1_NR + dh) * C1_PITCH;
        const unsigned char* arow = smA[s & 1] + abase;
#pragma unroll
        for (int kk = 0; kk < 2; ++kk) {
#pragma unroll
            for (int i = 0; i < WM; ++i) av[set][kk][i] = *reinterpret_cast<const bf16x8*>(arow + i * 32 * C1_PA + kk * 32);
            bv[set][kk] = *reinterpret_cast<const bf16x8*>(xrow + kk * 32);
        }
    };
    read_ops(0, 0);
    __syncthreads();
#pragma unroll
    for (int s = 0; s < C1_STEPS; ++s) {
        const int set = s & 1;
        if (s + 1 < C1_STEPS) read_ops(set ^ 1, s + 1);
#pragma unroll
        for (int kk = 0; kk < 2; ++kk)
#pragma unroll
            for (int i = 0; i < WM; ++i)
                acc[i][0] = __builtin_amdgcn_mfma_f32_32x32x16_bf16(av[set][kk][i], bv[set][kk], acc[i][0], 0, 0, 0);
        if (s + 2 < C1_STEPS) store_a(s + 2);
        if (s + 9 < C1_STEPS) load_a(s + 9);
        __syncthreads();
    }
    if (a.half) {
        constexpr int PT = 192 * 2 + 16;
        float* rows = reinterpret_cast<float*>(smA[0]);
        if (tid < BM) {
            const int m = m0 + tid;
            rows[2 * tid] = (m < a.M && a.scale) ? a.scale[m] : 1.f;
            rows[2 * tid + 1] = (m < a.M && a.shift) ? a.shift[m] : 0.f;
        }
        __syncthreads();
        const bool relu = (a.flags & EPI_RELU) != 0;
#pragma unroll
        for (int i = 0; i < WM; ++i)
#pragma unroll
            for (int r = 0; r < 16; ++r) {
                const int lr = i * 32 + (r & 3) + 8 * (r >> 2) + 4 * (lane >> 5);
                float v = acc[i][0][r] * rows[2 * lr] + rows[2 * lr + 1];
                if (relu) v = fmaxf(v, 0.f);
                *reinterpret_cast<unsigned short*>(patch + lr * PT + nl * 2) = (unsigned short)(cvt_pk_bf16(v, 0.f) & 0xffffu);
            }
        __syncthreads();
        unsigned short* yh = reinterpret_cast<unsigned short*>(a.out);
        for (int p = tid; p < BM * 24; p += C1_NT) {
// ... 249 lines not shown
        ctab = reinterpret_cast<int2*>(ws);
        wp = reinterpret_cast<unsigned short*>(reinterpret_cast<char*>(ws) + tb);
        PrepDesc d;
        fill_prep_desc<MODE>(d, a, ctab, wp);
        launch_prep(d, st);
        if (int e = otal_launch_status()) return e;
        ws = reinterpret_cast<char*>(ws) + tb + wb;
        ws_bytes -= tb + wb;
    }
    a.ctab = ctab; a.wp = wp;
#if OTAL_CONV_PART == 1
    if constexpr (H) {
        if (conv1x1_stream_eligible(a.g, MODE)) {
            const int e = launch_conv1x1_stream<MODE>(a, wp, wb, (a.M + BMpack - 1) / BMpack * BMpack, st);
            if (e != OTAL_E_UNSUPPORTED) return e;
        }
    }
#endif
    a.src_bytes = (unsigned)gather_extent_bytes(a.g, MODE, H ? 2 : 4);
    a.wp_bytes = (unsigned)wb;
    a.fd = make_conv_fastdiv(a.g);
    int splits = choose_splits(tm * tn, a.Kp);
    if (splits > 1) {
        const size_t need = (size_t)splits * a.M * a.N * sizeof(float);
        if (ws_bytes < need) {
            splits = (int)(ws_bytes / ((size_t)a.M * a.N * sizeof(float)));
            if (splits < 2) splits = 1;
        }
    }
    const int kps = ((a.Kp + splits - 1) / splits + 31) / 32 * 32;
    splits = (a.Kp + kps - 1) / kps;
    a.splits = splits;
    a.k_per_split = kps;
    a.slab = splits > 1 ? (float*)ws : nullptr;
    set_epilogue_extents<MODE>(a);
    const dim3 grid(tn, tm, splits);
    const int cw = chunk_vector_width(a.g);
#define OTAL_LAUNCH_C(BM_, WM_, WN_)                                                                                   \
    do {                                                                                                               \
        if (cw == 4) hipLaunchKernelGGL((conv_gemm_bf16c_kernel<BM_, WM_, WN_, MODE, 4, false, H>), grid, dim3(NT), 0, st, a);   \
        else if (cw == 2) hipLaunchKernelGGL((conv_gemm_bf16c_kernel<BM_, WM_, WN_, MODE, 2, false, H>), grid, dim3(NT), 0, st, a); \
        else hipLaunchKernelGGL((conv_gemm_bf16c_kernel<BM_, WM_, WN_, MODE, 1, false, H>), grid, dim3(NT), 0, st, a);           \
    } while (0)
    if constexpr (MODE == MODE_FWD && !H) {
        if (kwv) {
            if (BMsel == 128) hipLaunchKernelGGL((conv_gemm_bf16c_kernel<128, 2, 2, MODE_FWD, 1, true>), grid, dim3(NT), 0, st, a);
            else if (BMsel == 96) hipLaunchKernelGGL((conv_gemm_bf16c_kernel<96, 3, 1, MODE_FWD, 1, true>), grid, dim3(NT), 0, st, a);
            else if (BMsel == 64) hipLaunchKernelGGL((conv_gemm_bf16c_kernel<64, 2, 1, MODE_FWD, 1, true>), grid, dim3(NT), 0, st, a);
            else hipLaunchKernelGGL((conv_gemm_bf16c_kernel<32, 1, 1, MODE_FWD, 1, true>), grid, dim3(NT), 0, st, a);
        }
    }
    if (kwv) {
    } else if (BMsel == 192) OTAL_LAUNCH_C(192, 6, 1);
    else if (BMsel == 128) { if constexpr (!H) OTAL_LAUNCH_C(128, 2, 2); }
    else if (BMsel == 96) OTAL_LAUNCH_C(96, 3, 1);
    else if (BMsel == 64) OTAL_LAUNCH_C(64, 2, 1);
    else OTAL_LAUNCH_C(32, 1, 1);
#undef OTAL_LAUNCH_C
    if (int e = otal_launch_status()) return e;
    if (splits > 1) {
        return launch_splitk_reduce<MODE, H>(a, st);
    }
    return 0;
}

template <bool H = false>
int launch_wgrad_vector(ConvArgs& a, int cw, void* ws, size_t ws_bytes, hipStream_t st) {
    const bool pair = a.g.sw == 2;
    if (H && pair) return OTAL_E_UNSUPPORTED;
    if (pair) {
        a.N = a.g.Cin * a.g.kt * a.g.kh * 8;
        a.flags |= EPI_NPAD8;
    }
    const int BMsel = choose_bm(a.M);
    const int tm = (a.M + BMsel - 1) / BMsel, tn = (a.N + 127) / 128;
    const size_t tb = ptab_bytes(a.g, cw);
    a.fd = make_conv_fastdiv(a.g);
    a.P = conv_out_positions(a.g);
    a.src_bytes = (unsigned)gather_extent_bytes(a.g, MODE_FWD, H ? 2 : 4);
    a.dy_bytes = (unsigned)gather_extent_bytes(a.g, MODE_DGRAD, H ? 2 : 4);
    int2* ptab;
    if (a.pre) {
        ptab = reinterpret_cast<int2*>(const_cast<void*>(a.pre));
    } else {
        if (!ws || ws_bytes < tb) return OTAL_E_UNSUPPORTED;
        ptab = reinterpret_cast<int2*>(ws);
        const int ngroups = a.K / cw, npad = ngroups + PTAB_PAD;
        hipLaunchKernelGGL(build_pos_table_kernel, dim3((npad + 255) / 256), dim3(256), 0, st, ptab, a.g, a.fd, cw, ngroups, npad);
        if (int e = otal_launch_status()) return e;
        ws = reinterpret_cast<char*>(ws) + tb;
        ws_bytes -= tb;
    }
    a.ptab = ptab;
    int splits = choose_splits(tm * tn, a.K, 1, true);
    if (splits > 1) {
        const size_t need = (size_t)splits * a.M * a.N * sizeof(float);
        if (ws_bytes < need) {
            splits = (int)(ws_bytes / ((size_t)a.M * a.N * sizeof(float)));
            if (splits < 2) splits = 1;
        }
    }
    const int kps = ((a.K + splits - 1) / splits + 31) / 32 * 32;
    splits = (a.K + kps - 1) / kps;
    a.splits = splits;
    a.k_per_split = kps;
    a.slab = splits > 1 ? (float*)ws : nullptr;
    set_epilogue_extents<MODE_WGRAD>(a);
    const dim3 grid(tn, tm, splits);
#define OTAL_LAUNCH_W(BM_, WM_, WN_)                                                                                   \
    do {                                                                                                               \
        if (cw == 8) hipLaunchKernelGGL((conv_wgrad_bf16v_kernel<BM_, WM_, WN_, 8, false, H>), grid, dim3(NT), 0, st, a);        \
        else if (cw == 4) hipLaunchKernelGGL((conv_wgrad_bf16v_kernel<BM_, WM_, WN_, 4, false, H>), grid, dim3(NT), 0, st, a);   \
        else hipLaunchKernelGGL((conv_wgrad_bf16v_kernel<BM_, WM_, WN_, 2, false, H>), grid, dim3(NT), 0, st, a);                \
    } while (0)
    if constexpr (!H) {
        if (pair) {
            if (BMsel == 128) hipLaunchKernelGGL((conv_wgrad_bf16v_kernel<128, 2, 2, 8, true>), grid, dim3(NT), 0, st, a);
            else if (BMsel == 96) hipLaunchKernelGGL((conv_wgrad_bf16v_kernel<96, 3, 1, 8, true>), grid, dim3(NT), 0, st, a);
            else if (BMsel == 64) hipLaunchKernelGGL((conv_wgrad_bf16v_kernel<64, 2, 1, 8, true>), grid, dim3(NT), 0, st, a);
            else hipLaunchKernelGGL((conv_wgrad_bf16v_kernel<32, 1, 1, 8, true>), grid, dim3(NT), 0, st, a);
        }
    }
    if (pair) {
    } else if (BMsel == 192) OTAL_LAUNCH_W(192, 6, 1);
    else if (BMsel == 128) OTAL_LAUNCH_W(128, 2, 2);
    else if (BMsel == 96) OTAL_LAUNCH_W(96, 3, 1);
    else if (BMsel == 64) OTAL_LAUNCH_W(64, 2, 1);
    else OTAL_LAUNCH_W(32, 1, 1);
#undef OTAL_LAUNCH_W
    if (int e = otal_launch_status()) return e;
    if (splits > 1) {
        return launch_splitk_reduce<MODE_WGRAD>(a, st);
    }
    return 0;
}

template <int BM, int BNP, int PX = 48, bool H = false>
constexpr int direct_lds_bytes() { return 2 * BM * 304 + 2 * (BNP + (H ? 56 : 52)) * PX + 16; }
template <int BM, int MODE, bool XPF2 = false, bool H = false>
static int launch_direct512(const DirectArgs& d, dim3 grid, hipStream_t st) {
    constexpr int lds = direct_lds_bytes<BM, 512, 48, H>();
    static bool configured = false;
    if (!configured) {
        hipError_t e = hipFuncSetAttribute(reinterpret_cast<const void*>(conv3_direct_kernel<BM, MODE, 512, 2, 48, 1, XPF2, H>),
                                           hipFuncAttributeMaxDynamicSharedMemorySize, lds);
        if (e != hipSuccess) return (int)e;
        configured = true;
    }
    hipLaunchKernelGGL((conv3_direct_kernel<BM, MODE, 512, 2, 48, 1, XPF2, H>), grid, dim3(512), lds, st, d);
    return otal_launch_status();
}

template <int MODE, bool H = false>
int launch_direct(ConvArgs& a, void* ws, size_t ws_bytes, hipStream_t st) {
    if (H && ((a.g.Wi & 1) || (a.flags & EPI_ACCUM))) return OTAL_E_UNSUPPORTED;
    const int C = MODE == MODE_FWD ? a.g.Cin : a.g.Cout;
    const int BM = direct_bm(a.g, a.M);
    const int tm = (a.M + BM - 1) / BM, Mpad = tm * BM;
    const size_t wb = direct_wp_bytes(a.g, a.M, C);
    if (a.pre) {
        ws = const_cast<void*>(a.pre);
    } else {
        if (!ws || ws_bytes < wb) return OTAL_E_UNSUPPORTED;
        const int64_t pairs = (int64_t)Mpad * C * 27 / 2;
        const int blocks = (int)((pairs + 255) / 256 < 2048 ? (pairs + 255) / 256 : 2048);
        hipLaunchKernelGGL((pack_direct_kernel<MODE>), dim3(blocks), dim3(256), 0, st, reinterpret_cast<unsigned*>(ws), a.w,
                           a.M, Mpad, C, a.w_natural, make_fastdiv((uint32_t)(C * 27 / 2)));
        if (int e = otal_launch_status()) return e;
    }
    DirectArgs d;
    a.fd = make_conv_fastdiv(a.g);
    a.src_bytes = (unsigned)gather_extent_bytes(a.g, MODE, H ? 2 : 4);
    a.splits = 1; a.k_per_split = 0; a.slab = nullptr;
    set_epilogue_extents<MODE>(a);
    d.c = a;
    d.wp = reinterpret_cast<const unsigned short*>(ws);
    d.C = C; d.Ktot = C * 27; d.wp_bytes = (unsigned)wb;
    const int bnp = direct_bnp(a.g, a.M);
    if (bnp == 128) {
        const dim3 grid(a.N / 128, tm, 1);
        if (BM == 96) hipLaunchKernelGGL((conv3_direct_kernel<96, MODE, 128, 1, 48, 1, false, H>), grid, dim3(256), (direct_lds_bytes<96, 128, 48, H>()), st, d);
        else if (BM == 32) hipLaunchKernelGGL((conv3_direct_kernel<32, MODE, 128, 1, 48, 1, false, H>), grid, dim3(256), (direct_lds_bytes<32, 128, 48, H>()), st, d);
        else hipLaunchKernelGGL((conv3_direct_kernel<64, MODE, 128, 1, 48, 1, false, H>), grid, dim3(256), (direct_lds_bytes<64, 128, 48, H>()), st, d);
        return otal_launch_status();
    }
    const int xpf2 = OTAL_OPT("OTAL_CONV_DIRECT_XPF2");
    if (bnp == 512) {
        const dim3 grid(a.N / 512, tm, 1);
        if constexpr (MODE == MODE_FWD) {
            if (BM == 96 && (xpf2 & 2)) return launch_direct512<96, MODE, true, H>(d, grid, st);
        }
        if (BM == 96) return launch_direct512<96, MODE, false, H>(d, grid, st);
        return launch_direct512<64, MODE, false, H>(d, grid, st);
    }
    const dim3 grid(a.N / 256, tm, 1);
    if (BM == 96 && (xpf2 & 1)) hipLaunchKernelGGL((conv3_direct_kernel<96, MODE, 256, 1, 48, 1, true, H>), grid, dim3(512), (direct_lds_bytes<96, 256, 48, H>()), st, d);
    else if (BM == 64 && ((xpf2 & 4) || ((xpf2 & 1) && (int64_t)grid.x * grid.y <= 256))) hipLaunchKernelGGL((conv3_direct_kernel<64, MODE, 256, 1, 48, 1, true, H>), grid, dim3(512), (direct_lds_bytes<64, 256, 48, H>()), st, d);
    else if (BM == 96) hipLaunchKernelGGL((conv3_direct_kernel<96, MODE, 256, 1, 48, 1, false, H>), grid, dim3(512), (direct_lds_bytes<96, 256, 48, H>()), st, d);
    else if (BM == 32) hipLaunchKernelGGL((conv3_direct_kernel<32, MODE, 256, 1, 48, 1, false, H>), grid, dim3(512), (direct_lds_bytes<32, 256, 48, H>()), st, d);
    else hipLaunchKernelGGL((conv3_direct_kernel<64, MODE, 256, 1, 48, 1, false, H>), grid, dim3(512), (direct_lds_bytes<64, 256, 48, H>()), st, d);
    return otal_launch_status();
}

#include "conv_wgrad_direct.inc"
#include "conv1d_tile.inc"
#include "conv1a_wgrad.inc"
#include "proj_gemm.inc"
#include "wgrad1x1.inc"

#if OTAL_CONV_PART == 1
}
int otal_conv::launch_half(int mode, int kernel, int cw, ConvArgs& a, void* ws, size_t ws_bytes, hipStream_t st) {
    switch (kernel) {
        case CK_DIRECT:
            if (mode == MODE_FWD) return launch_direct<MODE_FWD, true>(a, ws, ws_bytes, st);
            return launch_direct<MODE_DGRAD, true>(a, ws, ws_bytes, st);
        case CK_CHUNKED:
            if (mode == MODE_FWD) return launch_chunked<MODE_FWD, true>(a, ws, ws_bytes, st);
            return launch_chunked<MODE_DGRAD, true>(a, ws, ws_bytes, st);
        case CK_WGRAD_DIRECT: return launch_wgrad_direct<true>(a, ws, ws_bytes, st);
        case CK_WGRAD1X1: return launch_wgrad1x1_wide<true>(a, ws, ws_bytes, st);
        case CK_WGRAD_VECTOR: return launch_wgrad_vector<true>(a, cw, ws, ws_bytes, st);
        default: return OTAL_E_UNSUPPORTED;
    }
}
namespace {
#endif

#if OTAL_CONV_PART == 0
template <int MODE>
int launch_generic(ConvArgs& a, void* ws, size_t ws_bytes, hipStream_t st) {
    if constexpr (MODE == MODE_DGRAD) {
        if (a.w_natural) {
            const int kvol = conv_kvol(a.g);
            const size_t wb = align256((size_t)a.g.Cin * a.g.Cout * kvol * sizeof(float));
            if (!ws || ws_bytes < wb) return OTAL_E_UNSUPPORTED;
            const int64_t total = (int64_t)a.g.Cout * a.g.Cin * kvol;
            const int blocks = (int)((total + 255) / 256 < 8192 ? (total + 255) / 256 : 8192);
            hipLaunchKernelGGL(pack_wt_kernel, dim3(blocks), dim3(256), 0, st, a.w, reinterpret_cast<float*>(ws), a.g.Cout, a.g.Cin, kvol);
            if (int e = otal_launch_status()) return e;
            a.w = reinterpret_cast<const float*>(ws);
            a.w_natural = 0;
            ws = reinterpret_cast<char*>(ws) + wb;
            ws_bytes -= wb;
        }
    }
    a.zero = zero_word_address();
    if (!a.zero) return OTAL_E_UNSUPPORTED;
    if (MODE != MODE_WGRAD) {
        const size_t tb = tab_bytes(a.K);
        if (!ws || ws_bytes < tb) return OTAL_E_UNSUPPORTED;
        int2* tab = reinterpret_cast<int2*>(ws);
        const int Kpad = a.K + (int)TAB_PAD;
        hipLaunchKernelGGL((build_tap_table_kernel<MODE>), dim3((Kpad + 255) / 256), dim3(256), 0, st, tab, a.g, a.K, Kpad);
        if (int e = otal_launch_status()) return e;
        a.tab = tab;
        ws = reinterpret_cast<char*>(ws) + tb;
        ws_bytes -= tb;
    }
    const int BMsel = choose_bm(a.M);
    const int BN = 128;
    const int tm = (a.M + BMsel - 1) / BMsel, tn = (a.N + BN - 1) / BN;
    a.fd = make_conv_fastdiv(a.g);
    if (MODE == MODE_WGRAD) {
        const int64_t P = conv_out_positions(a.g);
        a.a_vec4 = (P % 4 == 0) && (a.g.y_bs % 4 == 0) && (a.g.y_cs % 4 == 0) && (((uintptr_t)a.dy & 15) == 0) && BMsel >= 64;
    } else {
        a.a_vec4 = (a.K % 4 == 0) && (((uintptr_t)a.w & 15) == 0) && BMsel >= 64;
    }
    int splits = choose_splits(tm * tn, a.K, a.prec);
    if (MODE == MODE_WGRAD && a.prec) {
        const int ms = 4;
        const int tg = 512;
        const int tiles = tm * tn;
        int want = (tg + tiles - 1) / tiles, maxs = a.K / (ms * 32);
        if (maxs < 1) maxs = 1;
        splits = tiles >= tg * 3 / 4 ? 1 : (want < maxs ? want : maxs);
        if (splits > 384) splits = 384;
    }
    if (splits > 1) {
        const size_t need = (size_t)splits * a.M * a.N * sizeof(float);
        if (!ws || ws_bytes < need) {
            splits = ws ? (int)(ws_bytes / ((size_t)a.M * a.N * sizeof(float))) : 1;
            if (splits < 2) splits = 1;
        }
    }
    int kps = ((a.K + splits - 1) / splits + 31) / 32 * 32;
    splits = (a.K + kps - 1) / kps;
    a.splits = splits;
    a.k_per_split = kps;
    a.slab = splits > 1 ? (float*)ws : nullptr;
    set_epilogue_extents<MODE>(a);
    const dim3 grid(tn, tm, splits);
#define OTAL_LAUNCH(BM_, WM_, WN_, AV_)                                                                       \
    do {                                                                                                       \
        if (a.prec) hipLaunchKernelGGL((conv_gemm_kernel<BM_, 128, WM_, WN_, MODE, AV_, 1>), grid, dim3(NT), 0, st, a); \
        else hipLaunchKernelGGL((conv_gemm_kernel<BM_, 128, WM_, WN_, MODE, AV_, 0>), grid, dim3(NT), 0, st, a);        \
    } while (0)
    const bool av = a.a_vec4 != 0;
    if (BMsel == 128) { if (av) OTAL_LAUNCH(128, 2, 2, true); else OTAL_LAUNCH(128, 2, 2, false); }
    else if (BMsel == 96) { if (av) OTAL_LAUNCH(96, 3, 1, true); else OTAL_LAUNCH(96, 3, 1, false); }
    else if (BMsel == 64) { if (av) OTAL_LAUNCH(64, 2, 1, true); else OTAL_LAUNCH(64, 2, 1, false); }
    else OTAL_LAUNCH(32, 1, 1, false);
#undef OTAL_LAUNCH
    if (int e = otal_launch_status()) return e;
    if (splits > 1) {
        return launch_splitk_reduce<MODE>(a, st);
    }
    return 0;
}

template <int MODE>
int launch_kernel(const ConvStep& s, ConvArgs& a, void* ws, size_t ws_bytes, hipStream_t st) {
    if constexpr (MODE == MODE_WGRAD) {
        switch (s.kernel) {
            case CK_CONV1A_WGRAD: return launch_conv1a_wgrad(a, ws, ws_bytes, st);
            case CK_PROJ_WGRAD: return launch_proj_wgrad(a, st);
            case CK_WGRAD_DIRECT: return launch_wgrad_direct(a, ws, ws_bytes, st);
            case CK_WGRAD1X1: return launch_wgrad1x1_wide(a, ws, ws_bytes, st);
            case CK_WGRAD_VECTOR: return launch_wgrad_vector(a, s.cw, ws, ws_bytes, st);
            case CK_WGRAD1D: return launch_wgrad1d(a, ws, ws_bytes, st);
        }
    } else {
        switch (s.kernel) {
            case CK_PROJ: if constexpr (MODE == MODE_FWD) return launch_proj_fwd(a, ws, ws_bytes, st); break;
            case CK_CONV1A: if constexpr (MODE == MODE_FWD) return launch_conv1a_direct(a, ws, ws_bytes, st); break;
            case CK_CONV1D_TILE: return launch_conv1d_tile<MODE>(a, ws, ws_bytes, st);
            case CK_DIRECT: return launch_direct<MODE>(a, ws, ws_bytes, st);
            case CK_CHUNKED: return launch_chunked<MODE>(a, ws, ws_bytes, st);
        }
    }
    if (s.kernel == CK_GENERIC) return launch_generic<MODE>(a, ws, ws_bytes, st);
    return OTAL_E_UNSUPPORTED;
}

thread_local const char* g_last_kernel = "";

template <int MODE>
int launch_mode(ConvArgs& a, int precision, void* ws, size_t ws_bytes, hipStream_t st) {
    ConvQuery q = {};
    q.g = a.g;
    q.mode = MODE;
    q.precision = precision;
    q.accumulate = (a.flags & EPI_ACCUM) ? 1 : 0;
    q.has_mask = a.emask ? 1 : 0;
    q.x = (uintptr_t)a.x; q.w = (uintptr_t)a.w; q.dy = (uintptr_t)a.dy; q.out = (uintptr_t)a.out; q.mask = (uintptr_t)a.emask;
    const ConvPlan p = conv_plan(q);
    const void* pre = a.pre;
    int e = OTAL_E_UNSUPPORTED;
    for (int i = 0; i < p.n; ++i) {
        const ConvStep& s = p.step[i];
        a.pre = conv_step_prologue(s.kernel) == p.prologue ? pre : nullptr;
        e = a.xhalf ? otal_conv::launch_half(MODE, s.kernel, s.cw, a, ws, ws_bytes, st) : launch_kernel<MODE>(s, a, ws, ws_bytes, st);
        if (e == 0) g_last_kernel = conv_kernel_name(s.kernel);
        if (e != OTAL_E_UNSUPPORTED || !s.next) return e;
    }
    return e;
}
#endif

}

#if OTAL_CONV_PART == 0
extern "C" size_t otal_conv_workspace_bytes(const int* geom, int mode) {
    ConvGeom g;
    if (!geom || fill_geom(g, geom)) return 0;
    const int kvol = conv_kvol(g);
    int64_t M, N, K;
    if (mode == MODE_FWD) { M = g.Cout; N = (int64_t)g.B * conv_out_positions(g); K = (int64_t)g.Cin * kvol; }
    else if (mode == MODE_DGRAD) { M = g.Cin; N = (int64_t)g.B * conv_in_positions(g); K = (int64_t)g.Cout * kvol; }
    else {
        M = g.Cout; N = (int64_t)g.Cin * kvol; K = (int64_t)g.B * conv_out_positions(g);
        if (g.sw == 2 && g.kw <= 7) N = (int64_t)g.Cin * g.kt * g.kh * 8;
    }
    const int BMsel = choose_bm((int)M);
    const int BN = 128;
    const int tiles = (int)(((M + BMsel - 1) / BMsel) * ((N + BN - 1) / BN));
    int s = choose_splits(tiles, (int)K, 0);
    if (mode == MODE_WGRAD) { const int sw = choose_splits(tiles, (int)K, 1, true); if (sw > s) s = sw; }
    size_t front = mode == MODE_WGRAD ? ptab_bytes(g, 2) : tab_bytes((int)K);
    if (mode != MODE_WGRAD) {
        const int Kc = mode == MODE_FWD && g.Cin * g.kt * g.kh * 8 > K ? g.Cin * g.kt * g.kh * 8 : (int)K;
        size_t cf = chunk_tab_bytes(Kc) + chunk_wp_bytes((int)M, BMsel, Kc);
        if (M % 192 == 0) { const size_t ct = chunk_tab_bytes(Kc) + chunk_wp_bytes((int)M, 192, Kc); if (ct > cf) cf = ct; }
        if (direct_eligible(g, mode, 1, (int)M)) { const size_t dd = direct_wp_bytes(g, (int)M, mode == MODE_FWD ? g.Cin : g.Cout); if (dd > cf) cf = dd; }
        if (cf > front) front = cf;
    }
    if (mode == MODE_DGRAD) front += align256((size_t)g.Cin * g.Cout * kvol * sizeof(float));
    return front + (s > 1 ? (size_t)(s + 1) * M * N * sizeof(float) : 0);
}

extern "C" int otal_conv_fwd(const int* geom, const int64_t* strides, const float* x, const float* w,
                             const float* scale, const float* shift, float* y, int relu, int precision,
                             const void* prologue, void* ws, size_t ws_bytes, void* stream) {
    g_last_kernel = "";
    if (!geom || !strides || !x || !w || !y) return OTAL_E_NULL;
    ConvArgs a = {};
    if (int e = fill_geom(a.g, geom)) return e;
    a.g.x_bs = strides[0]; a.g.x_cs = strides[1]; a.g.y_bs = strides[2]; a.g.y_cs = strides[3];
    a.x = x; a.w = w; a.out = y; a.scale = scale; a.shift = shift;
    a.M = a.g.Cout; a.N = a.g.B * conv_out_positions(a.g); a.K = a.g.Cin * conv_kvol(a.g);
    a.flags = relu ? EPI_RELU : 0;
    a.prec = (precision & 1) ? 1 : 0;
    a.half = (precision & 4) ? 1 : 0;
    a.xhalf = (precision & 8) ? 1 : 0;
    if ((a.half || a.xhalf) && !a.prec) return OTAL_E_UNSUPPORTED;
    if (a.xhalf && !a.half) return OTAL_E_UNSUPPORTED;
    a.pre = prologue;
    return launch_mode<MODE_FWD>(a, precision, ws, ws_bytes, (hipStream_t)stream);
}

extern "C" int otal_conv_dgrad(const int* geom, const int64_t* strides, const float* dy, const float* wt_packed,
                               float* dx, int accumulate, const float* out_mask, const float* out_scale,
                               int precision, const void* prologue, void* ws, size_t ws_bytes, void* stream) {
    g_last_kernel = "";
    if (!geom || !strides || !dy || !wt_packed || !dx) return OTAL_E_NULL;
    if ((out_mask == nullptr) != (out_scale == nullptr)) return OTAL_E_NULL;
    ConvArgs a = {};
    if (int e = fill_geom(a.g, geom)) return e;
    a.g.x_bs = strides[0]; a.g.x_cs = strides[1]; a.g.y_bs = strides[2]; a.g.y_cs = strides[3];
    a.dy = dy; a.w = wt_packed; a.out = dx;
    if (a.g.st > 2 || a.g.sh > 2 || a.g.sw > 2) return OTAL_E_UNSUPPORTED;
    a.emask = out_mask; a.escale = out_scale;
    a.M = a.g.Cin; a.N = a.g.B * conv_in_positions(a.g); a.K = a.g.Cout * conv_kvol(a.g);
    a.flags = accumulate ? EPI_ACCUM : 0;
    a.prec = (precision & 1) ? 1 : 0;
    a.w_natural = (precision & 2) ? 1 : 0;
    a.half = (precision & 4) ? 1 : 0;
    a.xhalf = (precision & 8) ? 1 : 0;
    a.mhalf = (precision & 16) ? 1 : 0;
    if ((a.half || a.xhalf || a.mhalf) && !a.prec) return OTAL_E_UNSUPPORTED;
    if (a.half != a.xhalf || (a.mhalf && !a.xhalf) || (out_mask && a.xhalf && !a.mhalf)) return OTAL_E_UNSUPPORTED;
    a.pre = prologue;
    return launch_mode<MODE_DGRAD>(a, precision, ws, ws_bytes, (hipStream_t)stream);
}

extern "C" int otal_conv_wgrad(const int* geom, const int64_t* strides, const float* x, const float* dy,
                               float* dw, int accumulate, int precision,
                               const void* prologue, void* ws, size_t ws_bytes, void* stream) {
    g_last_kernel = "";
    if (!geom || !strides || !x || !dy || !dw) return OTAL_E_NULL;
    ConvArgs a = {};
    if (int e = fill_geom(a.g, geom)) return e;
    a.g.x_bs = strides[0]; a.g.x_cs = strides[1]; a.g.y_bs = strides[2]; a.g.y_cs = strides[3];
    a.x = x; a.dy = dy; a.out = dw;
    a.M = a.g.Cout; a.N = a.g.Cin * conv_kvol(a.g); a.K = a.g.B * conv_out_positions(a.g);
    a.flags = accumulate ? EPI_ACCUM : 0;
    a.prec = (precision & 1) ? 1 : 0;
    a.half = (precision & 4) ? 1 : 0;
    a.xhalf = (precision & 8) ? 1 : 0;
    if ((a.half || a.xhalf) && !a.prec) return OTAL_E_UNSUPPORTED;
    if (a.xhalf && !a.half) return OTAL_E_UNSUPPORTED;
    a.pre = prologue;
    return launch_mode<MODE_WGRAD>(a, precision, ws, ws_bytes, (hipStream_t)stream);
}

namespace {
int pair_geom(ConvArgs& a, const int* geom, const int64_t* strides) {
    if (int e = fill_geom(a.g, geom)) return e;
    a.g.x_bs = strides[0]; a.g.x_cs = strides[1]; a.g.y_bs = strides[2]; a.g.y_cs = strides[3];
    a.pair = 1;
    return 0;
}
}

extern "C" int otal_conv_fwd_pair(const int* geom, const int64_t* strides, const float* const* x, const float* const* w,
                                  const float* const* scale, const float* const* shift, float* const* y, int relu, int precision,
                                  const void* const* prologue, void* ws, size_t ws_bytes, void* stream) {
    if (!geom || !strides || !x || !w || !y || !x[0] || !x[1] || !w[0] || !w[1] || !y[0] || !y[1]) return OTAL_E_NULL;
    ConvArgs a = {};
    if (int e = pair_geom(a, geom, strides)) return e;
    a.x = x[0]; a.x2 = x[1]; a.w = w[0]; a.w2 = w[1]; a.out = y[0]; a.out2 = y[1];
    a.scale = scale ? scale[0] : nullptr; a.scale2 = scale ? scale[1] : nullptr;
    a.shift = shift ? shift[0] : nullptr; a.shift2 = shift ? shift[1] : nullptr;
    if ((a.scale == nullptr) != (a.scale2 == nullptr) || (a.shift == nullptr) != (a.shift2 == nullptr)) return OTAL_E_NULL;
    a.M = a.g.Cout; a.N = a.g.B * conv_out_positions(a.g); a.K = a.g.Cin * conv_kvol(a.g);
    a.flags = relu ? EPI_RELU : 0;
    a.prec = (precision & 1) ? 1 : 0;
    a.pre = prologue ? prologue[0] : nullptr; a.pre2 = prologue ? prologue[1] : nullptr;
    if (!conv1d_tile_eligible(a.g, MODE_FWD, a.prec, a.x, false) || ((uintptr_t)a.x2 & 3)) return OTAL_E_UNSUPPORTED;
    return launch_conv1d_tile<MODE_FWD>(a, ws, ws_bytes, (hipStream_t)stream);
}

extern "C" int otal_conv_dgrad_pair(const int* geom, const int64_t* strides, const float* const* dy, const float* const* w,
                                    float* const* dx, int precision, const void* const* prologue, void* ws, size_t ws_bytes,
                                    void* stream) {
    if (!geom || !strides || !dy || !w || !dx || !dy[0] || !dy[1] || !w[0] || !w[1] || !dx[0] || !dx[1]) return OTAL_E_NULL;
    ConvArgs a = {};
    if (int e = pair_geom(a, geom, strides)) return e;
    a.dy = dy[0]; a.dy2 = dy[1]; a.w = w[0]; a.w2 = w[1]; a.out = dx[0]; a.out2 = dx[1];
    a.M = a.g.Cin; a.N = a.g.B * conv_in_positions(a.g); a.K = a.g.Cout * conv_kvol(a.g);
    a.prec = (precision & 1) ? 1 : 0;
    a.w_natural = (precision & 2) ? 1 : 0;
    a.pre = prologue ? prologue[0] : nullptr; a.pre2 = prologue ? prologue[1] : nullptr;
    if (!a.w_natural) return OTAL_E_UNSUPPORTED;
    if (!conv1d_tile_eligible(a.g, MODE_DGRAD, a.prec, a.dy, false) || ((uintptr_t)a.dy2 & 3)) return OTAL_E_UNSUPPORTED;
    return launch_conv1d_tile<MODE_DGRAD>(a, ws, ws_bytes, (hipStream_t)stream);
}

extern "C" int otal_conv_wgrad_pair(const int* geom, const int64_t* strides, const float* const* x, const float* const* dy,
                                    float* const* dw, int precision, void* ws, size_t ws_bytes, void* stream) {
    if (!geom || !strides || !x || !dy || !dw || !x[0] || !x[1] || !dy[0] || !dy[1] || !dw[0] || !dw[1]) return OTAL_E_NULL;
    ConvArgs a = {};
    if (int e = pair_geom(a, geom, strides)) return e;
    a.x = x[0]; a.x2 = x[1]; a.dy = dy[0]; a.dy2 = dy[1]; a.out = dw[0]; a.out2 = dw[1];
    a.M = a.g.Cout; a.N = a.g.Cin * conv_kvol(a.g); a.K = a.g.B * conv_out_positions(a.g);
    a.prec = (precision & 1) ? 1 : 0;
    if (!wgrad1d_eligible(a.g, a.prec, a.x, a.dy) || !wgrad1d_eligible(a.g, a.prec, a.x2, a.dy2)) return OTAL_E_UNSUPPORTED;
    return launch_wgrad1d(a, ws, ws_bytes, (hipStream_t)stream);
}

extern "C" int otal_conv_half_storage(const int* geom, const int64_t* strides, int mode, int precision) {
    ConvGeom g;
    if (!geom || !strides || fill_geom(g, geom)) return 0;
    g.x_bs = strides[0]; g.x_cs = strides[1]; g.y_bs = strides[2]; g.y_cs = strides[3];
    return conv_half_storage(g, mode, precision);
}

extern "C" int otal_conv_pack_wt(const float* w, float* wt, int Cout, int Cin, int kvol, void* stream) {
    if (!w || !wt) return OTAL_E_NULL;
    if (Cout <= 0 || Cin <= 0 || kvol <= 0) return OTAL_E_SHAPE;
    const int64_t total = (int64_t)Cout * Cin * kvol;
    const int blocks = (int)((total + 255) / 256 < 8192 ? (total + 255) / 256 : 8192);
    hipLaunchKernelGGL(pack_wt_kernel, dim3(blocks), dim3(256), 0, (hipStream_t)stream, w, wt, Cout, Cin, kvol);
    return otal_launch_status();
}

namespace {
int fill_args_for_prologue(ConvArgs& a, const int* geom, const int64_t* strides, int mode, const float* w, int precision) {
    if (int e = fill_geom(a.g, geom)) return e;
    a.g.x_bs = strides[0]; a.g.x_cs = strides[1]; a.g.y_bs = strides[2]; a.g.y_cs = strides[3];
    a.w = w;
    a.prec = precision & 1;
    a.w_natural = (mode == MODE_DGRAD && (precision & 2)) ? 1 : 0;
    const int kvol = conv_kvol(a.g);
    if (mode == MODE_FWD) { a.M = a.g.Cout; a.K = a.g.Cin * kvol; if (a.g.Cin % 8) a.K = a.g.Cin * a.g.kt * a.g.kh * 8; }
    else if (mode == MODE_DGRAD) { a.M = a.g.Cin; a.K = a.g.Cout * kvol; }
    else { a.M = a.g.Cout; a.K = a.g.B * conv_out_positions(a.g); }
    return 0;
}
}

extern "C" size_t otal_conv_prologue_bytes(const int* geom, const int64_t* strides, int mode, int precision) {
    ConvGeom g;
    if (!geom || !strides || fill_geom(g, geom)) return 0;
    g.x_bs = strides[0]; g.x_cs = strides[1]; g.y_bs = strides[2]; g.y_cs = strides[3];
    return conv_prologue_bytes(g, mode, precision & 1);
}

extern "C" size_t otal_conv_prologue_desc_bytes(void) { return sizeof(PrepDesc); }

extern "C" int otal_conv_prologue(const int* geom, const int64_t* strides, int mode, const float* w, int precision,
                                  void* region, size_t region_bytes, void* host_desc, void* stream) {
    if (!geom || !strides || !region) return OTAL_E_NULL;
    ConvArgs a = {};
    if (int e = fill_args_for_prologue(a, geom, strides, mode, w, precision)) return e;
    const int layout = conv_prologue_layout(a.g, mode, a.prec);
    if (layout == PRO_NONE || region_bytes < otal_conv_prologue_bytes(geom, strides, mode, precision)) return OTAL_E_UNSUPPORTED;
    hipStream_t st = (hipStream_t)stream;
    if (layout == PRO_PTAB) {
        const int cw = a.g.sw == 2 ? 8 : wgrad_vector_width(a.g, a.prec);
        a.fd = make_conv_fastdiv(a.g);
        const int ngroups = a.K / cw, npad = ngroups + PTAB_PAD;
        hipLaunchKernelGGL(build_pos_table_kernel, dim3((npad + 255) / 256), dim3(256), 0, st, reinterpret_cast<int2*>(region),
                           a.g, a.fd, cw, ngroups, npad);
        if (int e = otal_launch_status()) return e > 0 ? -100 - e : e;
        return 0;
    }
    if (!w) return OTAL_E_NULL;
    PrepDesc d;
    if (layout == PRO_DIRECT) {
        d = PrepDesc{};
        const int BM = direct_bm(a.g, a.M);
        d.wp = reinterpret_cast<unsigned*>(region); d.wsrc = w; d.g = a.g; d.M = a.M; d.Mpad = (a.M + BM - 1) / BM * BM;
        d.C = mode == MODE_FWD ? a.g.Cin : a.g.Cout; d.natural = a.w_natural; d.mode = mode; d.direct = 1;
        d.fh = make_fastdiv((uint32_t)(d.C * 27 / 2));
        launch_prep(d, st);
        if (int e = otal_launch_status()) return e > 0 ? -100 - e : e;
        if (host_desc) memcpy(host_desc, &d, sizeof(d));
        return (int)prep_blocks(d);
    }
    int2* ctab = reinterpret_cast<int2*>(region);
    unsigned short* wp = reinterpret_cast<unsigned short*>(reinterpret_cast<char*>(region) + chunk_tab_bytes(a.K));
    if (mode == MODE_FWD) fill_prep_desc<MODE_FWD>(d, a, ctab, wp); else fill_prep_desc<MODE_DGRAD>(d, a, ctab, wp);
    launch_prep(d, st);
    if (int e = otal_launch_status()) return e > 0 ? -100 - e : e;
    if (host_desc) memcpy(host_desc, &d, sizeof(d));
// ... 28 lines not shown
```

opental_amd/csrc/conv_index.h:

```cpp
#pragma once
#include <stdint.h>

#if defined(__HIPCC__)
#define OTAL_HD __host__ __device__ __forceinline__
#else
#define OTAL_HD inline
#endif

#define OTAL_CONV_MAX_LEVELS 8

struct ConvGeom {
    int B, Cin, Cout;
    int Ti, Hi, Wi;
    int To, Ho, Wo;
    int kt, kh, kw;
    int st, sh, sw;
    int pt, ph, pw;
    int64_t x_bs, x_cs;
    int64_t y_bs, y_cs;
    int nlev;
    int lev[OTAL_CONV_MAX_LEVELS + 1];
};

struct FastDiv {
    uint32_t d, mul, sh, one;
};
OTAL_HD FastDiv make_fastdiv(uint32_t d) {
    FastDiv f;
    f.d = d;
    f.one = 0;
    if (d <= 1) { f.d = 1; f.mul = 0; f.sh = 0; f.one = 0xffffffffu; return f; }
    uint32_t s = 0;
    while ((1ull << s) < d) ++s;
    f.mul = (uint32_t)((((1ull << s) - d) << 32) / d + 1);
    f.sh = s - 1;
    return f;
}
OTAL_HD uint32_t otal_umulhi(uint32_t a, uint32_t b) {
#if defined(__HIP_DEVICE_COMPILE__)
    return __umulhi(a, b);
#else
    return (uint32_t)(((uint64_t)a * b) >> 32);
#endif
}
OTAL_HD uint32_t fd_div(const FastDiv& f, uint32_t n) {
    const uint32_t t = otal_umulhi(f.mul, n);
    const uint32_t q = (t + ((n - t) >> 1)) >> f.sh;
    return (q & ~f.one) | (n & f.one);
}

struct PosDec { int b, t, h, w; };
struct TapDec { int c, dt, dh, dw; };

OTAL_HD int conv_kvol(const ConvGeom& g) { return g.kt * g.kh * g.kw; }
OTAL_HD int conv_out_positions(const ConvGeom& g) { return g.To * g.Ho * g.Wo; }
OTAL_HD int conv_in_positions(const ConvGeom& g) { return g.Ti * g.Hi * g.Wi; }

OTAL_HD PosDec dec_pos(int n, int T, int H, int W) {
    PosDec p;
    p.w = n % W; n /= W;
    p.h = n % H; n /= H;
    p.t = n % T; p.b = n / T;
    return p;
}
OTAL_HD TapDec dec_tap(const ConvGeom& g, int k) {
    TapDec d;
    d.dw = k % g.kw; k /= g.kw;
    d.dh = k % g.kh; k /= g.kh;
    d.dt = k % g.kt; d.c = k / g.kt;
    return d;
}

struct ConvFastDiv { FastDiv kw, kh, kt, Wo, Ho, To, Wi, Hi, Ti, P; };
inline ConvFastDiv make_conv_fastdiv(const ConvGeom& g) {
    ConvFastDiv f;
    f.kw = make_fastdiv(g.kw); f.kh = make_fastdiv(g.kh); f.kt = make_fastdiv(g.kt);
    f.Wo = make_fastdiv(g.Wo); f.Ho = make_fastdiv(g.Ho); f.To = make_fastdiv(g.To);
    f.Wi = make_fastdiv(g.Wi); f.Hi = make_fastdiv(g.Hi); f.Ti = make_fastdiv(g.Ti);
    f.P = make_fastdiv((uint32_t)(g.To * g.Ho * g.Wo));
    return f;
}
OTAL_HD PosDec dec_pos_fd(uint32_t n, const FastDiv& T, const FastDiv& H, const FastDiv& W) {
    PosDec p;
    uint32_t q = fd_div(W, n); p.w = (int)(n - q * W.d); n = q;
    q = fd_div(H, n); p.h = (int)(n - q * H.d); n = q;
    q = fd_div(T, n); p.t = (int)(n - q * T.d); p.b = (int)q;
    return p;
}
OTAL_HD TapDec dec_tap_fd(const ConvFastDiv& f, uint32_t k) {
    TapDec d;
    uint32_t q = fd_div(f.kw, k); d.dw = (int)(k - q * f.kw.d); k = q;
    q = fd_div(f.kh, k); d.dh = (int)(k - q * f.kh.d); k = q;
    q = fd_div(f.kt, k); d.dt = (int)(k - q * f.kt.d); d.c = (int)q;
    return d;
}

OTAL_HD void level_bounds(const ConvGeom& g, int t, int extent, int& lo, int& hi) {
    lo = 0; hi = extent;
    if (g.nlev > 1) {
#if defined(__HIPCC__)
#pragma unroll
#endif
        for (int j = 0; j < OTAL_CONV_MAX_LEVELS; ++j)
            if (j < g.nlev && t >= g.lev[j]) { lo = g.lev[j]; hi = g.lev[j + 1]; }
    }
}

OTAL_HD bool conv_src_of_output(const ConvGeom& g, const PosDec& o, const TapDec& k, int64_t& off) {
    const int ti = o.t * g.st + k.dt - g.pt;
    const int hi = o.h * g.sh + k.dh - g.ph;
    const int wi = o.w * g.sw + k.dw - g.pw;
    int lo, up;
    level_bounds(g, o.t, g.Ti, lo, up);
    if (ti < lo || ti >= up || (unsigned)hi >= (unsigned)g.Hi || (unsigned)wi >= (unsigned)g.Wi) return false;
    off = (int64_t)o.b * g.x_bs + (int64_t)k.c * g.x_cs + ((int64_t)ti * g.Hi + hi) * g.Wi + wi;
    return true;
}

OTAL_HD bool div_stride(int num, int s, int extent, int& q) {
    if (num < 0) return false;
    if (s == 1) q = num;
    else if (s == 2) { if (num & 1) return false; q = num >> 1; }
    else { if (num % s) return false; q = num / s; }
    return q < extent;
}

OTAL_HD bool div_stride12(int num, int s, int extent, int& q) {
    const int sm1 = s - 1;
    q = num >> sm1;
    return (num >= 0) & ((num & sm1) == 0) & (q < extent);
}

OTAL_HD bool conv_src_of_input(const ConvGeom& g, const PosDec& i, const TapDec& k, int64_t& off) {
    int to, ho, wo;
    if (!div_stride(i.t + g.pt - k.dt, g.st, g.To, to)) return false;
    if (!div_stride(i.h + g.ph - k.dh, g.sh, g.Ho, ho)) return false;
    if (!div_stride(i.w + g.pw - k.dw, g.sw, g.Wo, wo)) return false;
    if (g.nlev > 1) {
        int lo, up;
        level_bounds(g, i.t, g.Ti, lo, up);
        if (to < lo || to >= up) return false;
    }
    off = (int64_t)i.b * g.y_bs + (int64_t)k.c * g.y_cs + ((int64_t)to * g.Ho + ho) * g.Wo + wo;
    return true;
}

OTAL_HD int64_t conv_out_offset(const ConvGeom& g, const PosDec& o, int co) {
    return (int64_t)o.b * g.y_bs + (int64_t)co * g.y_cs + ((int64_t)o.t * g.Ho + o.h) * g.Wo + o.w;
}
OTAL_HD int64_t conv_in_offset(const ConvGeom& g, const PosDec& i, int ci) {
    return (int64_t)i.b * g.x_bs + (int64_t)ci * g.x_cs + ((int64_t)i.t * g.Hi + i.h) * g.Wi + i.w;
}

inline void same_pad(int size, int k, int s, int& front, int& out) {
    int total = (size % s == 0) ? (k - s) : (k - size % s);
    if (total < 0) total = 0;
    front = total / 2;
    out = (size + total - k) / s + 1;
}
```

opental_amd/csrc/conv_select.h:

```cpp
#pragma once
#include <stddef.h>
#include <stdint.h>
#include "conv_index.h"
#include "options.h"

namespace {

enum { MODE_FWD = 0, MODE_DGRAD = 1, MODE_WGRAD = 2 };

constexpr int C1_TT = 2, C1_TR = 2, C1_WO = 48;
constexpr int C1T_TT = 4, C1T_TR = 4;
constexpr int W1_TC = 128;
constexpr int PJ_HW = 36;
constexpr int PW_KS = 32;
constexpr size_t TAB_PAD = 64;
constexpr int CHUNK_PAD = 16;
constexpr int PTAB_PAD = 64;

static inline size_t align256(size_t v) { return (v + 255) & ~(size_t)255; }
static inline size_t tab_bytes(int K) { return (((size_t)K + TAB_PAD) * (2 * sizeof(int)) + 255) & ~(size_t)255; }
static inline int chunk_kp(int K) { return (K + 31) / 32 * 32; }
static inline size_t chunk_tab_bytes(int K) { return align256(((size_t)chunk_kp(K) / 8 + CHUNK_PAD) * (2 * sizeof(int))); }
static inline size_t chunk_wp_bytes(int M, int BM, int K) {
    return align256(((size_t)((M + BM - 1) / BM * BM) * chunk_kp(K) + 64) * sizeof(unsigned short));
}
static inline size_t ptab_bytes(const ConvGeom& g, int cw) {
    return align256(((size_t)g.B * conv_out_positions(g) / cw + PTAB_PAD) * (2 * sizeof(int)));
}
static inline int64_t gather_extent_bytes(const ConvGeom& g, int mode, int esz = 4) {
    if (mode == MODE_FWD) return esz * ((int64_t)(g.B - 1) * g.x_bs + (int64_t)(g.Cin - 1) * g.x_cs + conv_in_positions(g));
    return esz * ((int64_t)(g.B - 1) * g.y_bs + (int64_t)(g.Cout - 1) * g.y_cs + conv_out_positions(g));
}

static inline int choose_bm(int M, bool tall = false) {
    if (tall && M % 192 == 0) return 192;
    const int cand[4] = {128, 96, 64, 32};
    const double pen[4] = {1.00, 1.03, 1.10, 1.30};
    int best = 128;
    double bc = 1e30;
    for (int i = 0; i < 4; ++i) {
        const double c = (double)((M + cand[i] - 1) / cand[i] * cand[i]) * pen[i];
        if (c < bc) { bc = c; best = cand[i]; }
    }
    return best;
}

static inline int choose_splits(int tiles, int K, int prec = 1, bool wgrad = false) {
    const bool wv = wgrad && prec;
    const int target = wv ? 2048 : 512;
    const int minsteps = wv ? 16 : (prec ? 8 : 4);
    const int cap = wv ? 1024 : 384;
    if (tiles >= target * 3 / 4) return 1;
    int want = (target + tiles - 1) / tiles;
    int maxs = K / (minsteps * 32);
    if (maxs < 1) maxs = 1;
    int s = want < maxs ? want : maxs;
    return s < 1 ? 1 : (s > cap ? cap : s);
}

static inline bool conv1a_half_out_ok(const ConvGeom& g, const void* y) {
    return g.y_bs % 8 == 0 && g.y_cs % 8 == 0 && (reinterpret_cast<uintptr_t>(y) & 15) == 0;
}
static inline bool conv1a_direct_eligible(const ConvGeom& g, int mode, int prec, const void* x) {
    if (!prec || mode != MODE_FWD || g.nlev > 1 || OTAL_OPT("OTAL_CONV_NO1A")) return false;
    if (g.Cin != 3 || g.kt != 7 || g.kh != 7 || g.kw != 7 || g.st != 2 || g.sh != 2 || g.sw != 2) return false;
    if (g.pt != 2 || g.ph != 2 || g.pw != 2 || g.Wi != 96 || g.Wo != C1_WO || g.Hi != 2 * g.Ho || g.Ti != 2 * g.To) return false;
    if (g.To % C1_TT || g.Ho % C1_TR || g.x_bs % 4 || g.x_cs % 4 || (reinterpret_cast<uintptr_t>(x) & 15)) return false;
    return (int64_t)g.B * g.To * g.Ho * g.Wo < (1LL << 31);
}
static inline int conv1a_tile_eligible(int To, int Ho) {
    return To % C1T_TT == 0 && Ho % C1T_TR == 0 && !OTAL_OPT("OTAL_CONV_1A_NOTILE");
}
static inline bool conv1a_wgrad_eligible(const ConvGeom& g, int prec, const void* x, const void* dy) {
    if (!prec || g.nlev > 1 || OTAL_OPT("OTAL_CONV_NO1AW")) return false;
    if (g.Cin != 3 || g.Cout > 64 || g.kt != 7 || g.kh != 7 || g.kw != 7 || g.st != 2 || g.sh != 2 || g.sw != 2) return false;
    if (g.pt != 2 || g.ph != 2 || g.pw != 2 || g.Wi != 96 || g.Wo != C1_WO || g.Hi != 2 * g.Ho || g.Ti != 2 * g.To) return false;
    if (g.To % 2 || g.Ho % 2 || g.x_bs % 4 || g.x_cs % 4 || g.y_bs % 4 || g.y_cs % 4) return false;
    if ((reinterpret_cast<uintptr_t>(x) & 15) || (reinterpret_cast<uintptr_t>(dy) & 15)) return false;
    const int64_t ex = gather_extent_bytes(g, MODE_FWD), ey = gather_extent_bytes(g, MODE_DGRAD);
    return ex > 0 && ey > 0 && ex < (1LL << 31) && ey < (1LL << 31);
}

static inline bool proj_fwd_eligible(const ConvGeom& g, int mode, int prec, const void* x, const void* w) {
    if (!prec || mode != MODE_FWD || g.nlev > 1 || OTAL_OPT("OTAL_CONV_NOPROJ")) return false;
    if (g.kt != 1 || g.st != 1 || g.kh != g.Hi || g.kw != g.Wi || g.Ho != 1 || g.Wo != 1 || g.To != g.Ti) return false;
    if (g.Hi * g.Wi != PJ_HW || g.ph != 0 || g.pw != 0 || g.pt != 0 || g.Cin % 4) return false;
    if (((uintptr_t)x & 3) || ((uintptr_t)w & 3)) return false;
    const int64_t ex = gather_extent_bytes(g, MODE_FWD), ew = 4 * (int64_t)g.Cout * g.Cin * PJ_HW;
    return ex > 0 && ex < (1LL << 31) && ew < (1LL << 31);
}
static inline bool proj_wgrad_eligible(const ConvGeom& g, int prec, const void* x, const void* dy) {
    if (!prec || g.nlev > 1 || OTAL_OPT("OTAL_CONV_NOPROJW")) return false;
    if (g.kt != 1 || g.st != 1 || g.kh != g.Hi || g.kw != g.Wi || g.Ho != 1 || g.Wo != 1 || g.To != g.Ti) return false;
    if (g.ph != 0 || g.pw != 0 || g.pt != 0 || g.Hi * g.Wi < 2) return false;
    if (g.To % PW_KS || g.y_cs < g.To || (g.y_cs & 3) || (g.y_bs & 3)) return false;
    if (((uintptr_t)x & 15) || ((uintptr_t)dy & 15) || (g.x_bs & 3) || (g.x_cs & 3)) return false;
    const int64_t ex = gather_extent_bytes(g, MODE_FWD), ey = gather_extent_bytes(g, MODE_DGRAD);
    const int64_t eo = 4 * (int64_t)g.Cout * g.Cin * g.Hi * g.Wi;
    return ex > 0 && ey > 0 && ex < (1LL << 31) && ey < (1LL << 31) && eo < (1LL << 31);
}

static inline bool conv1d_tile_eligible(const ConvGeom& g, int mode, int prec, const void* src, bool emask) {
    if (!prec || mode == MODE_WGRAD || OTAL_OPT("OTAL_CONV_NO1DTILE")) return false;
    if (g.Hi != 1 || g.Wi != 1 || g.Ho != 1 || g.Wo != 1 || g.kh != 1 || g.kw != 1 || g.st != 1 || g.To != g.Ti) return false;
    if (!((g.kt == 1 && g.pt == 0) || (g.kt == 3 && g.pt == 1))) return false;
    if (g.Ti > 4096) return false;
    if ((mode == MODE_FWD ? g.Cout : g.Cin) > 2048) return false;
    const int C = mode == MODE_FWD ? g.Cin : g.Cout;
    if (C % 128) return false;
    if (mode == MODE_DGRAD && emask) return false;
    if (((uintptr_t)src & 3)) return false;
    const int64_t ext = gather_extent_bytes(g, mode);
    return ext > 0 && ext < (1LL << 31);
}
static inline int wgrad1d_chunks(const ConvGeom& g) { return (g.Ti + W1_TC - 1) / W1_TC; }
static inline bool wgrad1d_eligible(const ConvGeom& g, int prec, const void* x, const void* dy) {
    if (!prec || OTAL_OPT("OTAL_CONV_NOW1D")) return false;
    if (g.Hi != 1 || g.Wi != 1 || g.Ho != 1 || g.Wo != 1 || g.kh != 1 || g.kw != 1 || g.st != 1 || g.To != g.Ti) return false;
    if (!((g.kt == 1 && g.pt == 0) || (g.kt == 3 && g.pt == 1))) return false;
    if (g.Cin % 64 || (g.x_bs | g.x_cs | g.y_bs | g.y_cs) & 1) return false;
    if ((reinterpret_cast<uintptr_t>(x) | reinterpret_cast<uintptr_t>(dy)) & 7) return false;
    return (int64_t)g.B * wgrad1d_chunks(g) <= 1024;
}

static inline bool chunk_eligible(const ConvGeom& g, int mode, int prec) {
    if (!prec || mode == MODE_WGRAD) return false;
    const int C = mode == MODE_FWD ? g.Cin : g.Cout;
    if (C % 8 && !(mode == MODE_FWD && g.kw >= 3)) return false;
    const int64_t ext = gather_extent_bytes(g, mode);
    return ext > 0 && ext < (int64_t)0xfffffff0u;
}
static inline bool conv1x1_stream_eligible(const ConvGeom& g, int mode) {
    if (OTAL_OPT("OTAL_CONV_NO1X1STREAM")) return false;
    if (g.kt != 1 || g.kh != 1 || g.kw != 1 || g.st != 1 || g.sh != 1 || g.sw != 1 || g.nlev > 1) return false;
    const int64_t P = conv_out_positions(g);
    if (P != conv_in_positions(g) || P % 128) return false;
    const int C = mode == MODE_FWD ? g.Cin : g.Cout;
    return C % 8 == 0;
}

static inline int direct_bm(const ConvGeom& g, int M) {
    if (M % 96 == 0) return 96;
    if (M > 96) {
        const int64_t nt = (int64_t)g.B * conv_out_positions(g) / 256;
        const int64_t w64 = (M + 63) / 64 * nt, w96 = (M + 95) / 96 * nt;
        if (w64 <= 512 && (w96 + 255) / 256 * 96 < (w64 + 255) / 256 * 64) return 96;
    }
    if (M % 64 == 0) return 64;
    if (M <= 32) return 32;
    const int pad64 = (M + 63) / 64 * 64;
    return (pad64 - M) * 100 <= M * 34 ? 64 : 0;
}
static inline int direct_bnp(const ConvGeom& g, int M) {
    const int BM = direct_bm(g, M);
    if (!BM) return 0;
    const int64_t tm = (M + BM - 1) / BM, NP = (int64_t)g.B * conv_out_positions(g);
    const int min_tiles = OTAL_OPT("OTAL_CONV_DIRECT_MINTILES");
    if (BM == 96 && conv_out_positions(g) % 512 == 0 && tm * (NP / 512) >= OTAL_OPT("OTAL_CONV_DIRECT_MINTILES512")) return 512;
    if (tm * (NP / 256) >= min_tiles) return 256;
    if (tm * (NP / 128) >= min_tiles) return 128;
    return 0;
}
static inline bool direct_eligible(const ConvGeom& g, int mode, int prec, int M) {
    if (OTAL_OPT("OTAL_CONV_NODIRECT") || !prec || mode == MODE_WGRAD || g.nlev > 1) return false;
    if (g.kt != 3 || g.kh != 3 || g.kw != 3 || g.st != 1 || g.sh != 1 || g.sw != 1 || g.pt != 1 || g.ph != 1 || g.pw != 1) return false;
    if (g.To != g.Ti || g.Ho != g.Hi || g.Wo != g.Wi || g.Wi > 24) return false;
    const int P = conv_out_positions(g);
    const int C = mode == MODE_FWD ? g.Cin : g.Cout;
    if (P % 256 || C % 16 || !direct_bnp(g, M)) return false;
    const int64_t ext = gather_extent_bytes(g, mode);
    return ext > 0 && ext < (1LL << 31);
}
static inline size_t direct_wp_bytes(const ConvGeom& g, int M, int C) {
    const int BM = direct_bm(g, M);
    return align256((size_t)((M + BM - 1) / BM * BM) * C * 27 * 2 + 1024);
}

static inline bool wgrad_direct_eligible(const ConvGeom& g, int prec, const void* x, const void* dy) {
    if (!prec || OTAL_OPT("OTAL_CONV_NOWDIRECT") || g.nlev > 1) return false;
    if (g.kt != 3 || g.kh != 3 || g.kw != 3 || g.st != 1 || g.sh != 1 || g.sw != 1 || g.pt != 1 || g.ph != 1 || g.pw != 1) return false;
    if (g.To != g.Ti || g.Ho != g.Hi || g.Wo != g.Wi) return false;
    const bool planes6 = g.Wi == 6 && g.Hi == 6 && g.Ti % 4 == 0;
    const bool planes3 = g.Wi == 3 && g.Hi == 3 && g.Ti % 16 == 0;
    if (!((g.Wi == 24 && g.Hi % 4 == 0) || (g.Wi == 12 && g.Hi == 12) || planes6 || planes3) || g.Cin % 2) return false;
    if (g.Cin < (planes3 ? 32 : 64) || g.Cout < 64) return false;
    if (((uintptr_t)x & 15) || ((uintptr_t)dy & 15) || g.x_cs % 4 || g.x_bs % 4 || g.y_cs % 4 || g.y_bs % 4) return false;
    const int64_t ex = gather_extent_bytes(g, MODE_FWD), ey = gather_extent_bytes(g, MODE_DGRAD);
    return ex > 0 && ey > 0 && ex < (1LL << 31) && ey < (1LL << 31);
}
static inline bool wgrad1x1_wide_eligible(const ConvGeom& g, int prec, const void* x, const void* dy) {
    if (!prec || g.nlev > 1 || OTAL_OPT("OTAL_CONV_NOW1X1")) return false;
    if (g.kt != 1 || g.kh != 1 || g.kw != 1 || g.st != 1 || g.sh != 1 || g.sw != 1) return false;
    if (g.To != g.Ti || g.Ho != g.Hi || g.Wo != g.Wi) return false;
    if (g.Hi == 1 && g.Wi == 1) return false;
    if (conv_out_positions(g) % 32 || (int64_t)g.Cout * g.Cin > (1 << 20)) return false;
    if (((uintptr_t)x & 3) || ((uintptr_t)dy & 3)) return false;
    const int64_t ex = gather_extent_bytes(g, MODE_FWD), ey = gather_extent_bytes(g, MODE_DGRAD);
    return ex > 0 && ey > 0 && ex < (1LL << 31) && ey < (1LL << 31);
}
static inline bool wgrad_pair_mode(const ConvGeom& g, int prec) {
    if (!prec || g.nlev > 1) return false;
    if (g.sw != 2 || g.st > 2 || g.sh > 2 || g.kw > 7 || g.pw > 3 || g.Wo % 8 || conv_out_positions(g) % 32) return false;
    if (g.Wi - (2 * (g.Wo - 8) - g.pw + 6) < 12) return false;
    const int64_t ex = 4 * ((int64_t)(g.B - 1) * g.x_bs + (int64_t)(g.Cin - 1) * g.x_cs + conv_in_positions(g));
    const int64_t ey = 4 * ((int64_t)(g.B - 1) * g.y_bs + (int64_t)(g.Cout - 1) * g.y_cs + conv_out_positions(g));
    return ex > 0 && ey > 0 && ex < (int64_t)0xffffff00u && ey < (int64_t)0xfffffff0u;
}
static inline int wgrad_vector_width(const ConvGeom& g, int prec) {
    if (!prec) return 0;
    if (g.st != 1 || g.sh != 1 || g.sw != 1 || g.nlev > 1) return 0;
    if (g.To != g.Ti || g.Ho != g.Hi || g.Wo != g.Wi) return 0;
    if ((g.kw != 1 && g.kw != 3) || g.pw != (g.kw - 1) / 2) return 0;
    if (conv_out_positions(g) % 32) return 0;
    const int64_t ex = 4 * ((int64_t)(g.B - 1) * g.x_bs + (int64_t)(g.Cin - 1) * g.x_cs + conv_in_positions(g));
    const int64_t ey = 4 * ((int64_t)(g.B - 1) * g.y_bs + (int64_t)(g.Cout - 1) * g.y_cs + conv_out_positions(g));
    if (ex <= 0 || ey <= 0 || ex >= (int64_t)0xfffffff0u || ey >= (int64_t)0xfffffff0u) return 0;
    if (g.kt == 1 && g.kh == 1 && g.kw == 1) return 8;
    if (g.Wi % 8 == 0) return 8;
    if (g.Wi % 4 == 0) return 4;
    if (g.Wi % 2 == 0) return 2;
    return 0;
}

enum ConvKernel {
    CK_GENERIC,
    CK_PROJ, CK_CONV1A, CK_CONV1D_TILE, CK_DIRECT, CK_CHUNKED,
    CK_CONV1A_WGRAD, CK_PROJ_WGRAD, CK_WGRAD_DIRECT, CK_WGRAD1X1, CK_WGRAD_VECTOR, CK_WGRAD1D,
};
static inline const char* conv_kernel_name(int kernel) {
    switch (kernel) {
        case CK_GENERIC: return "generic";
        case CK_PROJ: return "proj";
        case CK_CONV1A: return "conv1a";
        case CK_CONV1D_TILE: return "conv1d_tile";
        case CK_DIRECT: return "direct";
        case CK_CHUNKED: return "chunked";
        case CK_CONV1A_WGRAD: return "conv1a_wgrad";
        case CK_PROJ_WGRAD: return "proj_wgrad";
        case CK_WGRAD_DIRECT: return "wgrad_direct";
        case CK_WGRAD1X1: return "wgrad1x1_wide";
        case CK_WGRAD_VECTOR: return "vector";
        case CK_WGRAD1D: return "wgrad1d";
    }
    return "?";
}
enum ConvPrologue { PRO_NONE = 0, PRO_CHUNK = 1, PRO_PTAB = 2, PRO_DIRECT = 3 };

struct ConvQuery {
    ConvGeom g;
    int mode;
    int precision;
    int accumulate;
    int has_mask;
    uintptr_t x, w, dy, out, mask;
};
struct ConvStep {
    int kernel;
    int cw;
    bool next;
};
struct ConvPlan {
    int n;
    ConvStep step[8];
    int prologue;
};

static inline int conv_step_prologue(int kernel) {
    switch (kernel) {
        case CK_CONV1D_TILE: case CK_CHUNKED: return PRO_CHUNK;
        case CK_DIRECT: return PRO_DIRECT;
        case CK_WGRAD_VECTOR: return PRO_PTAB;
        default: return PRO_NONE;
    }
}

static inline int conv_prologue_layout(const ConvGeom& g, int mode, int prec) {
    if (mode == MODE_WGRAD) return wgrad_pair_mode(g, prec) || wgrad_vector_width(g, prec) ? PRO_PTAB : PRO_NONE;
    if (proj_fwd_eligible(g, mode, prec, nullptr, nullptr)) return PRO_NONE;
    if (conv1a_direct_eligible(g, mode, prec, nullptr)) return PRO_NONE;
    if (direct_eligible(g, mode, prec, mode == MODE_FWD ? g.Cout : g.Cin)) return PRO_DIRECT;
    return chunk_eligible(g, mode, prec) ? PRO_CHUNK : PRO_NONE;
}
static inline size_t conv_prologue_bytes(const ConvGeom& g, int mode, int prec) {
    const int layout = conv_prologue_layout(g, mode, prec);
    const int M = mode == MODE_FWD ? g.Cout : g.Cin;
    if (layout == PRO_CHUNK) {
        const bool kwv = mode == MODE_FWD && (g.Cin % 8) != 0;
        const int K = mode == MODE_FWD ? (kwv ? g.Cin * g.kt * g.kh * 8 : g.Cin * conv_kvol(g)) : g.Cout * conv_kvol(g);
        return chunk_tab_bytes(K) + chunk_wp_bytes(M, choose_bm(M, !kwv), K);
    }
    if (layout == PRO_PTAB) return ptab_bytes(g, g.sw == 2 ? 8 : wgrad_vector_width(g, prec));
    if (layout == PRO_DIRECT) return direct_wp_bytes(g, M, mode == MODE_FWD ? g.Cin : g.Cout);
    return 0;
}

static inline void conv_plan_half(const ConvQuery& q, ConvPlan& p) {
    const ConvGeom& g = q.g;
    const void* px = (const void*)(q.mode == MODE_DGRAD ? q.out : q.x);
    const void* py = (const void*)(q.mode == MODE_FWD ? q.out : q.dy);
    auto add = [&p](int kernel, bool next, int cw = 0) { p.step[p.n++] = ConvStep{kernel, cw, next}; };
    if (!(q.precision & 1) || !(q.precision & 4) || q.accumulate) return;
    if (((uintptr_t)px | (uintptr_t)py) & 15) return;
    if (q.mode == MODE_DGRAD && q.has_mask && (!(q.precision & 16) || (q.mask & 15))) return;
    if (g.nlev > 1) return;
    if (conv_out_positions(g) % 8 || conv_in_positions(g) % 8 || g.x_bs % 8 || g.x_cs % 8 || g.y_bs % 8 || g.y_cs % 8) return;
    if (q.mode == MODE_FWD || q.mode == MODE_DGRAD) {
        const int M = q.mode == MODE_FWD ? g.Cout : g.Cin, C = q.mode == MODE_FWD ? g.Cin : g.Cout;
        if (direct_eligible(g, q.mode, 1, M) && !(g.Wi & 1)) add(CK_DIRECT, false);
        else if (chunk_eligible(g, q.mode, 1) && C % 8 == 0 && conv_in_positions(g) == conv_out_positions(g)) add(CK_CHUNKED, false);
        return;
    }
    const int cw = wgrad_vector_width(g, 1);
    if (wgrad_direct_eligible(g, 1, px, py)) add(CK_WGRAD_DIRECT, true);
    else if (wgrad1x1_wide_eligible(g, 1, px, py)) add(CK_WGRAD1X1, true);
    if (cw) add(CK_WGRAD_VECTOR, false, cw);
}

static inline ConvPlan conv_plan(const ConvQuery& q) {
    ConvPlan p = {};
    const ConvGeom& g = q.g;
    const int prec = q.precision & 1, half = (q.precision >> 2) & 1;
    p.prologue = conv_prologue_layout(g, q.mode, prec);
    if (q.precision & 8) { conv_plan_half(q, p); return p; }
    const void *x = (const void*)q.x, *w = (const void*)q.w, *dy = (const void*)q.dy, *out = (const void*)q.out;
    auto add = [&p](int kernel, bool next, int cw = 0) { p.step[p.n++] = ConvStep{kernel, cw, next}; };
    if (q.mode == MODE_WGRAD) {
        if (conv1a_wgrad_eligible(g, prec, x, dy) && (!half || g.y_bs % 8 + g.y_cs % 8 == 0)) add(CK_CONV1A_WGRAD, !half);
        if (half) return p;
        if (proj_wgrad_eligible(g, prec, x, dy)) add(CK_PROJ_WGRAD, true);
        if (wgrad_direct_eligible(g, prec, x, dy)) add(CK_WGRAD_DIRECT, true);
        if (wgrad1x1_wide_eligible(g, prec, x, dy)) add(CK_WGRAD1X1, true);
        if (wgrad_pair_mode(g, prec)) { add(CK_WGRAD_VECTOR, false, 8); return p; }
        if (const int cw = wgrad_vector_width(g, prec)) { add(CK_WGRAD_VECTOR, false, cw); return p; }
        if (wgrad1d_eligible(g, prec, x, dy)) add(CK_WGRAD1D, true);
        add(CK_GENERIC, false);
        return p;
    }
    const int M = q.mode == MODE_FWD ? g.Cout : g.Cin;
    if (q.mode == MODE_FWD) {
        if (proj_fwd_eligible(g, q.mode, prec, x, w)) add(CK_PROJ, true);
        if (half) {
            if (conv1a_direct_eligible(g, q.mode, prec, x) && conv1a_half_out_ok(g, out)) add(CK_CONV1A, false);
            else if (direct_eligible(g, q.mode, prec, M) && conv1a_half_out_ok(g, out)) add(CK_DIRECT, false);
            return p;
        }
        if (conv1a_direct_eligible(g, q.mode, prec, x)) { add(CK_CONV1A, false); return p; }
    }
    if (half) return p;
    if (conv1d_tile_eligible(g, q.mode, prec, q.mode == MODE_FWD ? x : dy, q.has_mask)) add(CK_CONV1D_TILE, true);
    if (direct_eligible(g, q.mode, prec, M)) add(CK_DIRECT, false);
    else if (chunk_eligible(g, q.mode, prec)) add(CK_CHUNKED, false);
    else add(CK_GENERIC, false);
    return p;
}

static inline int conv_half_storage(const ConvGeom& g, int mode, int precision) {
    if (!(precision & 1) || g.y_bs % 8 || g.y_cs % 8) return 0;
    ConvQuery q = {};
    q.g = g;
    q.mode = mode;
    q.precision = precision | 4;
    const ConvPlan p = conv_plan(q);
    for (int i = 0; i < p.n; ++i)
        if (p.step[i].kernel != CK_PROJ) return 1;
    return 0;
}

}
```

opental_amd/csrc/options.h:

```cpp
#pragma once

struct OtalOption { const char* name; int dflt; };
constexpr OtalOption OTAL_OPTIONS[] = {
    {"OTAL_CONV_1A_NOTILE", 0},           {"OTAL_CONV_1A_WGS", 0},
    {"OTAL_CONV_DIRECT_MINTILES", 140},   {"OTAL_CONV_DIRECT_MINTILES512", 512},
    {"OTAL_CONV_DIRECT_XPF2", 3},         {"OTAL_CONV_NO1A", 0},
    {"OTAL_CONV_NO1AW", 0},               {"OTAL_CONV_NO1DTILE", 0},
    {"OTAL_CONV_NO1X1STREAM", 0},         {"OTAL_CONV_NODIRECT", 0},
    {"OTAL_CONV_NOPROJ", 0},              {"OTAL_CONV_NOPROJW", 0},
    {"OTAL_CONV_NOW1D", 0},               {"OTAL_CONV_NOW1X1", 0},
    {"OTAL_CONV_NOWDIRECT", 0},           {"OTAL_LOSS_NOSTAGE", 0},
    {"OTAL_POOL_NO133", 0},               {"OTAL_POOL_NOROWS", 0},
    {"OTAL_W1A_SPLITS", 0},               {"OTAL_WDIRECT_BLOCKS", 0},
};
constexpr int OTAL_NUM_OPTIONS = sizeof(OTAL_OPTIONS) / sizeof(OTAL_OPTIONS[0]);
constexpr bool otal_streq(const char* a, const char* b) { return *a == *b && (*a == 0 || otal_streq(a + 1, b + 1)); }
constexpr int otal_option_index(const char* name, int i = 0) {
    return i == OTAL_NUM_OPTIONS ? -1 : otal_streq(OTAL_OPTIONS[i].name, name) ? i : otal_option_index(name, i + 1);
}
int* otal_option_slot(int index);
#define OTAL_OPT(name) ([]() -> int {                                                                              \
    constexpr int index_ = otal_option_index(name);                                                              \
    static_assert(index_ >= 0, "unknown option " name " (options.h: OTAL_OPTIONS)");                               \
    static int* const slot_ = otal_option_slot(index_);                                                          \
    return *slot_;                                                                                               \
}())
```

Before: 1002.

## Launch both inception 3x3 dgrad convs as one grouped direct kernel

New measurement: 1013, median of 6. 1.0% higher.

```diff
diff --git a/include/opental_hip.h b/include/opental_hip.h
--- a/include/opental_hip.h
+++ b/include/opental_hip.h
@@ -67,6 +67,11 @@
                          float* const* dx, int precision, const void* const* prologue, void* ws, size_t ws_bytes, void* stream);
 int otal_conv_wgrad_pair(const int* geom, const int64_t* strides, const float* const* x, const float* const* dy,
                          float* const* dw, int precision, void* ws, size_t ws_bytes, void* stream);
+
+int otal_conv_dgrad_group(const int* const* geom, const int64_t* const* strides, const float* const* dy,
+                          const float* const* w, float* const* dx, const float* const* out_mask,
+                          const float* const* out_scale, int precision, const void* const* prologue, void* ws,
+                          size_t ws_bytes, void* stream);
 
 size_t otal_conv_prologue_bytes(const int* geom, const int64_t* strides, int mode, int precision);
 size_t otal_conv_prologue_desc_bytes(void);
diff --git a/opental_amd/common/i3d_backbone.py b/opental_amd/common/i3d_backbone.py
--- a/opental_amd/common/i3d_backbone.py
+++ b/opental_amd/common/i3d_backbone.py
@@ -477,12 +477,17 @@
                 dX = out_grad_buffer(pos - 1, xin.shape, xin)
                 xm = xin if in_scale is not None else None
                 sl = (slice(0, c1), slice(c1, c2), slice(c2, c3), slice(c3, Y.shape[1]))
-                for a, b, hid, sli, dst in ((w0 + 1, w0 + 2, h1, sl[1], Zg[:, :o1]), (w0 + 3, w0 + 4, h2, sl[2], Zg[:, o1:o13])):
+                br = ((w0 + 1, w0 + 2, h1, sl[1], Zg[:, :o1]), (w0 + 3, w0 + 4, h2, sl[2], Zg[:, o1:o13]))
+                gm = br if h1.shape[1] >= h2.shape[1] else br[::-1]
+                grouped = ops.conv_dgrad_group([dY[:, m[3]] for m in gm], [weights[m[1]] for m in gm], [m[2].shape for m in gm],
+                                               THREE, ONE, [m[4] for m in gm], [m[2] for m in gm], [sc(m[0]) for m in gm])
+                for a, b, hid, sli, dst in br:
                     g = dY[:, sli]
                     slot = ops.grad_slot(weights[b])
                     in_slots = in_slots and slot is not None
                     dws[b] = side.wgrad(hid, g, weights[b].shape, THREE, ONE, out=slot)
-                    ops.conv_dgrad(g, weights[b], hid.shape, THREE, ONE, out=dst, out_mask=hid, out_scale=sc(a))
+                    if grouped is None:
+                        ops.conv_dgrad(g, weights[b], hid.shape, THREE, ONE, out=dst, out_mask=hid, out_scale=sc(a))
                 gf = Zg[:, :o13 + c1]
                 slot = ops.grad_slot(wf)
                 in_slots = in_slots and slot is not None
diff --git a/opental_amd/common/ops.py b/opental_amd/common/ops.py
--- a/opental_amd/common/ops.py
+++ b/opental_amd/common/ops.py
@@ -28,13 +28,15 @@
     return ev
 
 
-def _prof_end(ev, mode, g, problems=1):
+def _prof_end(ev, mode, g, problems=1, more=()):
     if ev is None:
         return
     end = torch.cuda.Event(enable_timing=True)
     end.record()
     B, Cin, Cout = g[0], g[1], g[2]
     flops = 2.0 * B * Cout * g[6] * g[7] * g[8] * Cin * g[9] * g[10] * g[11] * problems
+    for h in more:
+        flops += 2.0 * h[0] * h[2] * h[6] * h[7] * h[8] * h[1] * h[9] * h[10] * h[11]
     CONV_PROFILE.append((mode, flops, ev, end))
 
 
@@ -880,6 +882,44 @@
         return None
     L.check(rc, "otal_conv_dgrad_pair")
     _prof_end(ev, "dgrad", g, 2)
+    return outs
+
+
+GROUP_LAUNCHES = 0
+
+
+def conv_dgrad_group(dys, ws, x_shapes, k, s, outs, out_masks, out_scales):
+    global GROUP_LAUNCHES
+    k, s = _k3(k), _k3(s)
+    fn = getattr(L.lib(), "otal_conv_dgrad_group", None)
+    if fn is None or not (int(CONV_PRECISION) & 1):
+        return None
+    if any(t.dtype != torch.bfloat16 for t in (*dys, *outs, *out_masks)):
+        return None
+    prec = int(CONV_PRECISION) | 2
+    plans, wts = [], []
+    for dy, w, xs, out, m in zip(dys, ws, x_shapes, outs, out_masks):
+        if tuple(out.shape) != tuple(xs):
+            raise RuntimeError(f"conv_dgrad_group: out has shape {tuple(out.shape)}, expected {tuple(xs)}")
+        plan = _plan(1, out, dy, w.shape[0], k, s, None, False, "dx", "dy")
+        m5 = _as5(m)
+        if (tuple(m5.shape), _bs(m5)) != plan[4]:
+            raise RuntimeError("out_mask must share dx's shape, layout and dtype")
+        plans.append(plan)
+        wts.append(w if w.is_contiguous() else w.contiguous())
+    wsp, wsn = _ws_args(dys[0].device)
+    ev = _prof_begin()
+    pres = [_prologue(1, pl[1], pl[2], pl[3], w, prec) for pl, w in zip(plans, wts)]
+    gas = _VP2(ctypes.addressof(plans[0][1]), ctypes.addressof(plans[1][1]))
+    sas = _VP2(ctypes.addressof(plans[0][2]), ctypes.addressof(plans[1][2]))
+    pre = _VP2(*(None if p is None else p.value for p in pres))
+    rc = fn(gas, sas, _pp(*dys), _pp(*wts), _pp(*outs), _pp(*out_masks), _pp(*out_scales), prec | 12 | 16, pre,
+            wsp, wsn, L.stream())
+    if rc == L.E_UNSUPPORTED:
+        return None
+    L.check(rc, "otal_conv_dgrad_group")
+    GROUP_LAUNCHES += 1
+    _prof_end(ev, "dgrad", plans[0][0], more=(plans[1][0],))
     return outs
 
 
diff --git a/opental_amd/csrc/conv3_direct_body.inc b/opental_amd/csrc/conv3_direct_body.inc
--- /dev/null
+++ b/opental_amd/csrc/conv3_direct_body.inc
@@ -0,0 +1,285 @@
+    constexpr int DNT = BNP * 2 / WN;
+    constexpr int WM = BM / 32, PA = 304, SPAN_MAX = BNP + (H ? 56 : 52);
+    constexpr int ESZ = H ? 2 : 4, XV = H ? 8 : 4;
+    static_assert(PX == 48 || PX == 32, "position pitch");
+    constexpr int A_PIECES = (BM * 18 + DNT - 1) / DNT;
+    constexpr int X_ITEMS = (SPAN_MAX / XV + 1) * 8;
+    constexpr int X_ITERS = (X_ITEMS + DNT - 1) / DNT;
+    extern __shared__ __attribute__((aligned(16))) unsigned char dsm[];
+    unsigned char* const smA0 = dsm;
+    unsigned char* const smX0 = dsm + 2 * BM * PA;
+    const unsigned char* const smZero = dsm + 2 * BM * PA + 2 * SPAN_MAX * PX;
+    if (threadIdx.x < 4) reinterpret_cast<unsigned*>(dsm + 2 * BM * PA + 2 * SPAN_MAX * PX)[threadIdx.x] = 0u;
+    auto smA = [&](int buf) { return smA0 + buf * (BM * PA); };
+    auto smX = [&](int buf) { return smX0 + buf * (SPAN_MAX * PX); };
+    const ConvArgs& a = d.c;
+    const ConvGeom& g = a.g;
+    const ConvFastDiv& fd = a.fd;
+    const int tid = threadIdx.x, lane = tid & 63;
+    const int wave = __builtin_amdgcn_readfirstlane(tid >> 6);
+    const TileId tile = OTAL_DIRECT_TILE;
+    const int m0 = tile.y * BM, n0 = tile.x * BNP;
+    const int W = g.Wi, HW = g.Hi * g.Wi;
+    const int XO = H ? W + 2 : W + 1;
+    const int span = BNP + XO + W + 1, nq = (span + XV - 1) / XV;
+    const float* src = MODE == MODE_FWD ? a.x : a.dy;
+    const int64_t sbs = MODE == MODE_FWD ? g.x_bs : g.y_bs, scs = MODE == MODE_FWD ? g.x_cs : g.y_cs;
+    const auto rs = __builtin_amdgcn_make_buffer_rsrc(const_cast<float*>(src), 0, (int)a.src_bytes, 0x00020000);
+    const auto rw = __builtin_amdgcn_make_buffer_rsrc(const_cast<unsigned short*>(d.wp), 0, (int)d.wp_bytes, 0x00020000);
+    const uint32_t bsm = fd_div(fd.P, (uint32_t)n0);
+    const int p0 = n0 - (int)(bsm * fd.P.d);
+    const unsigned tile_off = (unsigned)(((int64_t)bsm * sbs + p0 - XO) * ESZ);
+
+    unsigned tmask[WN], hwmask[WN];
+#pragma unroll
+    for (int j = 0; j < WN; ++j) {
+        const int nl = n0 + (wave * WN + j) * 32 + (lane & 31);
+        const PosDec o = dec_pos_fd(nl < a.N ? nl : 0, fd.To, fd.Ho, fd.Wo);
+        const bool live = nl < a.N;
+        tmask[j] = 0; hwmask[j] = 0;
+#pragma unroll
+        for (int dt = 0; dt < 3; ++dt) tmask[j] |= (unsigned)(live && (unsigned)(o.t + dt - 1) < (unsigned)g.Ti) << dt;
+#pragma unroll
+        for (int dh = 0; dh < 3; ++dh)
+#pragma unroll
+            for (int dw = 0; dw < 3; ++dw)
+                hwmask[j] |= (unsigned)((unsigned)(o.h + dh - 1) < (unsigned)g.Hi && (unsigned)(o.w + dw - 1) < (unsigned)g.Wi) << (dh * 3 + dw);
+    }
+    unsigned xvo[X_ITERS];
+    int xlds[X_ITERS];
+#pragma unroll
+    for (int i = 0; i < X_ITERS; ++i) {
+        const int item = tid + DNT * i;
+        const int cp = item & 7, q = item >> 3;
+        const bool used = q < nq;
+        xvo[i] = used ? tile_off + (unsigned)((2 * cp * scs + XV * q) * ESZ) : 0xffffffffu;
+        if constexpr (H)
+            xlds[i] = PX == 48 ? (8 * q) * PX + cp * 4 : (8 * q) * PX + ((((cp >> 2) ^ q) & 1) << 4) + (cp & 3) * 4;
+        else
+            xlds[i] = PX == 48 ? (4 * q) * PX + cp * 4
+                               : (4 * q) * PX + ((((cp >> 2) ^ (q >> 1)) & 1) << 4) + (cp & 3) * 4;
+    }
+    unsigned avo[A_PIECES];
+#pragma unroll
+    for (int j = 0; j < A_PIECES; ++j) {
+        const int p = tid + DNT * j;
+        avo[j] = (unsigned)(((m0 + p / 18) * d.Ktot * 2) + (p % 18) * 16);
+    }
+    unsigned rxs[XPF2 ? 2 : 1][X_ITERS][2][4];
+    Words4 ra[A_PIECES];
+    const int nsteps = (d.C >> 4) * 3;
+    auto load_x = [&](int s, auto SET) {
+        unsigned (&rx)[X_ITERS][2][4] = rxs[decltype(SET)::value];
+        const int cb = s / 3, dt = s - cb * 3;
+        const unsigned so = (unsigned)(((int64_t)cb * 16 * scs + (int64_t)(dt - 1) * HW) * ESZ);
+#pragma unroll
+        for (int i = 0; i < X_ITERS; ++i) {
+            const unsigned vo = xvo[i] == 0xffffffffu ? a.src_bytes : xvo[i] + so;
+#pragma unroll
+            for (int h = 0; h < 2; ++h) {
+                const Words4 v = __builtin_bit_cast(Words4, __builtin_amdgcn_raw_buffer_load_b128(rs, vo, h ? (int)(scs * ESZ) : 0, 0));
+                rx[i][h][0] = v.a; rx[i][h][1] = v.b; rx[i][h][2] = v.c; rx[i][h][3] = v.d;
+            }
+        }
+    };
+    auto load_a = [&](int s) {
+#pragma unroll
+        for (int j = 0; j < A_PIECES; ++j)
+            if ((BM * 18) % DNT == 0 || tid + DNT * j < BM * 18)
+                ra[j] = __builtin_bit_cast(Words4, __builtin_amdgcn_raw_buffer_load_b128(rw, avo[j], s * 288, 0));
+    };
+    auto store = [&](int buf, int s, auto SET) {
+        unsigned (&rx)[X_ITERS][2][4] = rxs[decltype(SET)::value];
+        const int cb = s / 3, dt = s - cb * 3;
+        const unsigned so = (unsigned)(((int64_t)cb * 16 * scs + (int64_t)(dt - 1) * HW) * ESZ);
+#pragma unroll
+        for (int i = 0; i < X_ITERS; ++i) {
+            if (xvo[i] == 0xffffffffu) continue;
+            const unsigned vo = xvo[i] + so;
+            const bool neg = vo >= 0xfffffff0u;
+            if (__builtin_amdgcn_ballot_w64(neg) != 0ull) {
+#pragma unroll
+                for (int h = 0; h < 2; ++h) {
+                    if constexpr (H) {
+#pragma unroll
+                        for (int e = 1; e < 4; ++e) {
+                            const unsigned v = __builtin_amdgcn_raw_buffer_load_b32(rs, neg ? wrap_add(vo, 4u * e) : a.src_bytes,
+                                                                                     h ? (int)(scs * ESZ) : 0, 0);
+                            rx[i][h][e] = neg ? v : rx[i][h][e];
+                        }
+                    } else {
+#pragma unroll
+                        for (int e = 1; e < 4; ++e) {
+                            const unsigned v = __builtin_amdgcn_raw_buffer_load_b32(rs, neg ? wrap_add(vo, 4u * e) : a.src_bytes,
+                                                                                     h ? (int)(scs * 4) : 0, 0);
+                            rx[i][h][e] = neg ? v : rx[i][h][e];
+                        }
+                    }
+                }
+            }
+            if constexpr (H) {
+#pragma unroll
+                for (int e = 0; e < 8; ++e)
+                    *reinterpret_cast<unsigned*>(smX(buf) + xlds[i] + e * PX) =
+                        (e & 1) ? pair_hi(rx[i][0][e >> 1], rx[i][1][e >> 1]) : pair_lo(rx[i][0][e >> 1], rx[i][1][e >> 1]);
+            } else {
+#pragma unroll
+                for (int e = 0; e < 4; ++e)
+                    *reinterpret_cast<unsigned*>(smX(buf) + xlds[i] + e * PX) =
+                        cvt_pk_bf16(__uint_as_float(rx[i][0][e]), __uint_as_float(rx[i][1][e]));
+            }
+        }
+#pragma unroll
+        for (int j = 0; j < A_PIECES; ++j) {
+            const int p = tid + DNT * j;
+            if ((BM * 18) % DNT == 0 || p < BM * 18) *reinterpret_cast<Words4*>(smA(buf) + (p / 18) * PA + (p % 18) * 16) = ra[j];
+        }
+    };
+
+    f32x16 acc[WM][WN];
+#pragma unroll
+    for (int i = 0; i < WM; ++i)
+#pragma unroll
+        for (int j = 0; j < WN; ++j)
+#pragma unroll
+            for (int r = 0; r < 16; ++r) acc[i][j][r] = 0.f;
+
+    using Set0 = std::integral_constant<int, 0>;
+    using Set1 = std::integral_constant<int, XPF2 ? 1 : 0>;
+    load_x(0, Set0{});
+    load_a(0);
+    store(0, 0, Set0{});
+    if constexpr (XPF2) load_x(nsteps > 1 ? 1 : 0, Set1{});
+    __syncthreads();
+    const int xpos = wave * WN * 32 + (lane & 31) + XO;
+    const int xrow = xpos * PX + (lane >> 5) * 16;
+    auto frag_a = [&](int buf, int g9, int i) -> bf16x8 {
+        return *reinterpret_cast<const bf16x8*>(smA(buf) + (i * 32 + (lane & 31)) * PA + g9 * 32 + (lane >> 5) * 16);
+    };
+    auto frag_b = [&](int buf, int dt, int g9, int j) -> bf16x8 {
+        const int dh = g9 / 3, dw = g9 - dh * 3;
+        const unsigned char* src;
+        if (PX == 48) {
+            src = smX(buf) + xrow + (j * 32 + (dh - 1) * W + (dw - 1)) * PX;
+        } else {
+            const int p = xpos + j * 32 + (dh - 1) * W + (dw - 1);
+            src = smX(buf) + p * PX + ((((lane >> 5) ^ (p >> 3)) & 1) << 4);
+        }
+        const bool ok = ((tmask[j] >> dt) & 1u) && ((hwmask[j] >> g9) & 1u);
+        return *reinterpret_cast<const bf16x8*>(ok ? src : smZero);
+    };
+    auto kstep = [&](int s, auto CUR, auto OTHER) {
+        const int buf = s & 1;
+        const int dt = s % 3;
+        const int sn = s + 1 < nsteps ? s + 1 : s;
+        const int sx = XPF2 ? (s + 2 < nsteps ? s + 2 : nsteps - 1) : sn;
+        bf16x8 avA[WM], bvA[WN], avB[WM], bvB[WN];
+#pragma unroll
+        for (int i = 0; i < WM; ++i) avA[i] = frag_a(buf, 0, i);
+#pragma unroll
+        for (int j = 0; j < WN; ++j) bvA[j] = frag_b(buf, dt, 0, j);
+#pragma unroll
+        for (int g9 = 0; g9 < 9; ++g9) {
+            if (g9 == 0) load_x(sx, OTHER);
+            if (g9 == 1) load_a(sn);
+            bf16x8 (&av)[WM] = (g9 & 1) ? avB : avA;
+            bf16x8 (&bv)[WN] = (g9 & 1) ? bvB : bvA;
+            bf16x8 (&avn)[WM] = (g9 & 1) ? avA : avB;
+            bf16x8 (&bvn)[WN] = (g9 & 1) ? bvA : bvB;
+            int n = 0;
+#pragma unroll
+            for (int i = 0; i < WM; ++i)
+#pragma unroll
+                for (int j = 0; j < WN; ++j) {
+                    acc[i][j] = __builtin_amdgcn_mfma_f32_32x32x16_bf16(av[i], bv[j], acc[i][j], 0, 0, 0);
+                    if (g9 < 8) {
+                        if (n < WM) avn[n] = frag_a(buf, g9 + 1, n);
+                        else if (n < WM + WN) bvn[n - WM] = frag_b(buf, dt, g9 + 1, n - WM);
+                    }
+                    ++n;
+                }
+            if (WM * WN < WM + WN && g9 < 8) {
+#pragma unroll
+                for (int r = WM * WN; r < WM + WN; ++r) {
+                    if (r < WM) avn[r] = frag_a(buf, g9 + 1, r);
+                    else bvn[r - WM] = frag_b(buf, dt, g9 + 1, r - WM);
+                }
+            }
+            __builtin_amdgcn_sched_barrier(0);
+        }
+        store(buf ^ 1, sn, CUR);
+        __syncthreads();
+    };
+    if constexpr (XPF2) {
+        for (int s = 0; s < nsteps; s += 2) {
+            kstep(s, Set1{}, Set0{});
+            if (s + 1 < nsteps) kstep(s + 1, Set0{}, Set1{});
+        }
+    } else {
+        for (int s = 0; s < nsteps; ++s) kstep(s, Set0{}, Set0{});
+    }
+    if ((MODE == MODE_FWD && a.half) || (MODE == MODE_DGRAD && a.xhalf)) {
+        constexpr int PT = BNP * 2 + 16;
+        static_assert(BM * PT + BM * 8 <= 2 * BM * PA + 2 * SPAN_MAX * PX, "staging tile fits in the operand buffers");
+        unsigned char* tile = dsm;
+        float* rows = reinterpret_cast<float*>(dsm + BM * PT);
+        __syncthreads();
+        for (int r = tid; r < BM; r += DNT) {
+            const int m = m0 + r;
+            if constexpr (MODE == MODE_FWD) {
+                rows[2 * r] = (m < a.M && a.scale) ? a.scale[m] : 1.f;
+                rows[2 * r + 1] = (m < a.M && a.shift) ? a.shift[m] : 0.f;
+            } else {
+                rows[2 * r] = (m < a.M && a.escale) ? a.escale[m] : 1.f;
+                rows[2 * r + 1] = 0.f;
+            }
+        }
+        __syncthreads();
+        const bool relu = MODE == MODE_FWD && (a.flags & EPI_RELU) != 0;
+#pragma unroll
+        for (int i = 0; i < WM; ++i)
+#pragma unroll
+            for (int j = 0; j < WN; ++j) {
+                const int nl = (wave * WN + j) * 32 + (lane & 31);
+#pragma unroll
+                for (int r = 0; r < 16; ++r) {
+                    const int lr = i * 32 + (r & 3) + 8 * (r >> 2) + 4 * (lane >> 5);
+                    float v = acc[i][j][r] * rows[2 * lr] + rows[2 * lr + 1];
+                    if (relu) v = fmaxf(v, 0.f);
+                    *reinterpret_cast<unsigned short*>(tile + lr * PT + nl * 2) = (unsigned short)(cvt_pk_bf16(v, 0.f) & 0xffffu);
+                }
+            }
+        __syncthreads();
+        unsigned short* yh = reinterpret_cast<unsigned short*>(a.out);
+        const unsigned short* mk = MODE == MODE_DGRAD ? reinterpret_cast<const unsigned short*>(a.emask) : nullptr;
+        const int64_t ocs = MODE == MODE_FWD ? g.y_cs : g.x_cs;
+        const int64_t ybase = (int64_t)bsm * (MODE == MODE_FWD ? g.y_bs : g.x_bs) + p0;
+        constexpr int U = 4;
+        for (int p0 = tid; p0 < BM * (BNP / 8); p0 += U * DNT) {
+            int64_t off[U];
+            bool ok[U];
+            Words4 m4[U];
+#pragma unroll
+            for (int u = 0; u < U; ++u) {
+                const int p = p0 + u * DNT;
+                const int row = p / (BNP / 8), q = p - row * (BNP / 8);
+                ok[u] = p < BM * (BNP / 8) && m0 + row < a.M && n0 + q * 8 < a.N;
+                off[u] = ok[u] ? ybase + (int64_t)(m0 + row) * ocs + q * 8 : 0;
+                if (mk) m4[u] = *reinterpret_cast<const Words4*>(mk + off[u]);
+            }
+#pragma unroll
+            for (int u = 0; u < U; ++u) {
+                if (!ok[u]) continue;
+                const int p = p0 + u * DNT;
+                const int row = p / (BNP / 8), q = p - row * (BNP / 8);
+                Words4 v = *reinterpret_cast<const Words4*>(tile + row * PT + q * 16);
+                if (mk) {
+                    v.a &= bf16_relu_mask2(m4[u].a); v.b &= bf16_relu_mask2(m4[u].b);
+                    v.c &= bf16_relu_mask2(m4[u].c); v.d &= bf16_relu_mask2(m4[u].d);
+                }
+                *reinterpret_cast<Words4*>(yh + off[u]) = v;
+            }
+        }
+        return;
+    }
+    store_acc<MODE, WM, WN, BM>(a, acc, m0, n0, 0, wave * WN * 32, lane, 0, reinterpret_cast<float*>(smA(0)));
diff --git a/opental_amd/csrc/conv_gemm.hip b/opental_amd/csrc/conv_gemm.hip
--- a/opental_amd/csrc/conv_gemm.hip
+++ b/opental_amd/csrc/conv_gemm.hip
@@ -14,6 +14,10 @@
 namespace otal_conv {
 struct ConvArgs;
 __attribute__((visibility("hidden"))) int launch_half(int mode, int kernel, int cw, ConvArgs& a, void* ws, size_t ws_bytes, hipStream_t st);
+}
+namespace otal_conv {
+__attribute__((visibility("hidden"))) int launch_direct_group_half(ConvArgs& a, ConvArgs& b, const int* plan, void* ws, size_t ws_bytes,
+                                                                 hipStream_t st);
 }
 
 namespace {
@@ -1886,291 +1890,32 @@
 
 template <int BM, int MODE, int BNP, int WN, int PX = 48, int MINW = 1, bool XPF2 = false, bool H = false>
 __global__ __launch_bounds__(BNP * 2 / WN, MINW) void conv3_direct_kernel(const DirectArgs d) {
-    constexpr int DNT = BNP * 2 / WN;
-    constexpr int WM = BM / 32, PA = 304, SPAN_MAX = BNP + (H ? 56 : 52);
-    constexpr int ESZ = H ? 2 : 4, XV = H ? 8 : 4;
-    static_assert(PX == 48 || PX == 32, "position pitch");
-    constexpr int A_PIECES = (BM * 18 + DNT - 1) / DNT;
-    constexpr int X_ITEMS = (SPAN_MAX / XV + 1) * 8;
-    constexpr int X_ITERS = (X_ITEMS + DNT - 1) / DNT;
-    extern __shared__ __attribute__((aligned(16))) unsigned char dsm[];
-    unsigned char* const smA0 = dsm;
-    unsigned char* const smX0 = dsm + 2 * BM * PA;
-    const unsigned char* const smZero = dsm + 2 * BM * PA + 2 * SPAN_MAX * PX;
-    if (threadIdx.x < 4) reinterpret_cast<unsigned*>(dsm + 2 * BM * PA + 2 * SPAN_MAX * PX)[threadIdx.x] = 0u;
-    auto smA = [&](int buf) { return smA0 + buf * (BM * PA); };
-    auto smX = [&](int buf) { return smX0 + buf * (SPAN_MAX * PX); };
-    const ConvArgs& a = d.c;
-    const ConvGeom& g = a.g;
-    const ConvFastDiv& fd = a.fd;
-    const int tid = threadIdx.x, lane = tid & 63;
-    const int wave = __builtin_amdgcn_readfirstlane(tid >> 6);
-    const TileId tile = xcd_tile(true);
-    const int m0 = tile.y * BM, n0 = tile.x * BNP;
-    const int W = g.Wi, HW = g.Hi * g.Wi;
-    const int XO = H ? W + 2 : W + 1;
-    const int span = BNP + XO + W + 1, nq = (span + XV - 1) / XV;
-    const float* src = MODE == MODE_FWD ? a.x : a.dy;
-    const int64_t sbs = MODE == MODE_FWD ? g.x_bs : g.y_bs, scs = MODE == MODE_FWD ? g.x_cs : g.y_cs;
-    const auto rs = __builtin_amdgcn_make_buffer_rsrc(const_cast<float*>(src), 0, (int)a.src_bytes, 0x00020000);
-    const auto rw = __builtin_amdgcn_make_buffer_rsrc(const_cast<unsigned short*>(d.wp), 0, (int)d.wp_bytes, 0x00020000);
-    const uint32_t bsm = fd_div(fd.P, (uint32_t)n0);
-    const int p0 = n0 - (int)(bsm * fd.P.d);
-    const unsigned tile_off = (unsigned)(((int64_t)bsm * sbs + p0 - XO) * ESZ);
-
-    unsigned tmask[WN], hwmask[WN];
-#pragma unroll
-    for (int j = 0; j < WN; ++j) {
-        const int nl = n0 + (wave * WN + j) * 32 + (lane & 31);
-        const PosDec o = dec_pos_fd(nl < a.N ? nl : 0, fd.To, fd.Ho, fd.Wo);
-        const bool live = nl < a.N;
-        tmask[j] = 0; hwmask[j] = 0;
-#pragma unroll
-        for (int dt = 0; dt < 3; ++dt) tmask[j] |= (unsigned)(live && (unsigned)(o.t + dt - 1) < (unsigned)g.Ti) << dt;
-#pragma unroll
-        for (int dh = 0; dh < 3; ++dh)
-#pragma unroll
-            for (int dw = 0; dw < 3; ++dw)
-                hwmask[j] |= (unsigned)((unsigned)(o.h + dh - 1) < (unsigned)g.Hi && (unsigned)(o.w + dw - 1) < (unsigned)g.Wi) << (dh * 3 + dw);
-    }
-    unsigned xvo[X_ITERS];
-    int xlds[X_ITERS];
-#pragma unroll
-    for (int i = 0; i < X_ITERS; ++i) {
-        const int item = tid + DNT * i;
-        const int cp = item & 7, q = item >> 3;
-        const bool used = q < nq;
-        xvo[i] = used ? tile_off + (unsigned)((2 * cp * scs + XV * q) * ESZ) : 0xffffffffu;
-        if constexpr (H)
-            xlds[i] = PX == 48 ? (8 * q) * PX + cp * 4 : (8 * q) * PX + ((((cp >> 2) ^ q) & 1) << 4) + (cp & 3) * 4;
-        else
-            xlds[i] = PX == 48 ? (4 * q) * PX + cp * 4
-                               : (4 * q) * PX + ((((cp >> 2) ^ (q >> 1)) & 1) << 4) + (cp & 3) * 4;
-    }
-    unsigned avo[A_PIECES];
-#pragma unroll
-    for (int j = 0; j < A_PIECES; ++j) {
-        const int p = tid + DNT * j;
-        avo[j] = (unsigned)(((m0 + p / 18) * d.Ktot * 2) + (p % 18) * 16);
-    }
-    unsigned rxs[XPF2 ? 2 : 1][X_ITERS][2][4];
-    Words4 ra[A_PIECES];
-    const int nsteps = (d.C >> 4) * 3;
-    auto load_x = [&](int s, auto SET) {
-        unsigned (&rx)[X_ITERS][2][4] = rxs[decltype(SET)::value];
-        const int cb = s / 3, dt = s - cb * 3;
-        const unsigned so = (unsigned)(((int64_t)cb * 16 * scs + (int64_t)(dt - 1) * HW) * ESZ);
-#pragma unroll
-        for (int i = 0; i < X_ITERS; ++i) {
-            const unsigned vo = xvo[i] == 0xffffffffu ? a.src_bytes : xvo[i] + so;
-#pragma unroll
-            for (int h = 0; h < 2; ++h) {
-                const Words4 v = __builtin_bit_cast(Words4, __builtin_amdgcn_raw_buffer_load_b128(rs, vo, h ? (int)(scs * ESZ) : 0, 0));
-                rx[i][h][0] = v.a; rx[i][h][1] = v.b; rx[i][h][2] = v.c; rx[i][h][3] = v.d;
-            }
-        }
-    };
-    auto load_a = [&](int s) {
-#pragma unroll
-        for (int j = 0; j < A_PIECES; ++j)
-            if ((BM * 18) % DNT == 0 || tid + DNT * j < BM * 18)
-                ra[j] = __builtin_bit_cast(Words4, __builtin_amdgcn_raw_buffer_load_b128(rw, avo[j], s * 288, 0));
-    };
-    auto store = [&](int buf, int s, auto SET) {
-        unsigned (&rx)[X_ITERS][2][4] = rxs[decltype(SET)::value];
-        const int cb = s / 3, dt = s - cb * 3;
-        const unsigned so = (unsigned)(((int64_t)cb * 16 * scs + (int64_t)(dt - 1) * HW) * ESZ);
-#pragma unroll
-        for (int i = 0; i < X_ITERS; ++i) {
-            if (xvo[i] == 0xffffffffu) continue;
-            const unsigned vo = xvo[i] + so;
-            const bool neg = vo >= 0xfffffff0u;
-            if (__builtin_amdgcn_ballot_w64(neg) != 0ull) {
-#pragma unroll
-                for (int h = 0; h < 2; ++h) {
-                    if constexpr (H) {
-#pragma unroll
-                        for (int e = 1; e < 4; ++e) {
-                            const unsigned v = __builtin_amdgcn_raw_buffer_load_b32(rs, neg ? wrap_add(vo, 4u * e) : a.src_bytes,
-                                                                                     h ? (int)(scs * ESZ) : 0, 0);
-                            rx[i][h][e] = neg ? v : rx[i][h][e];
-                        }
-                    } else {
-#pragma unroll
-                        for (int e = 1; e < 4; ++e) {
-                            const unsigned v = __builtin_amdgcn_raw_buffer_load_b32(rs, neg ? wrap_add(vo, 4u * e) : a.src_bytes,
-                                                                                     h ? (int)(scs * 4) : 0, 0);
-                            rx[i][h][e] = neg ? v : rx[i][h][e];
-                        }
-                    }
-                }
-            }
-            if constexpr (H) {
-#pragma unroll
-                for (int e = 0; e < 8; ++e)
-                    *reinterpret_cast<unsigned*>(smX(buf) + xlds[i] + e * PX) =
-                        (e & 1) ? pair_hi(rx[i][0][e >> 1], rx[i][1][e >> 1]) : pair_lo(rx[i][0][e >> 1], rx[i][1][e >> 1]);
-            } else {
-#pragma unroll
-                for (int e = 0; e < 4; ++e)
-                    *reinterpret_cast<unsigned*>(smX(buf) + xlds[i] + e * PX) =
-                        cvt_pk_bf16(__uint_as_float(rx[i][0][e]), __uint_as_float(rx[i][1][e]));
-            }
-        }
-#pragma unroll
-        for (int j = 0; j < A_PIECES; ++j) {
-            const int p = tid + DNT * j;
-            if ((BM * 18) % DNT == 0 || p < BM * 18) *reinterpret_cast<Words4*>(smA(buf) + (p / 18) * PA + (p % 18) * 16) = ra[j];
-        }
-    };
-
-    f32x16 acc[WM][WN];
-#pragma unroll
-    for (int i = 0; i < WM; ++i)
-#pragma unroll
-        for (int j = 0; j < WN; ++j)
-#pragma unroll
-            for (int r = 0; r < 16; ++r) acc[i][j][r] = 0.f;
-
-    using Set0 = std::integral_constant<int, 0>;
-    using Set1 = std::integral_constant<int, XPF2 ? 1 : 0>;
-    load_x(0, Set0{});
-    load_a(0);
-    store(0, 0, Set0{});
-    if constexpr (XPF2) load_x(nsteps > 1 ? 1 : 0, Set1{});
-    __syncthreads();
-    const int xpos = wave * WN * 32 + (lane & 31) + XO;
-    const int xrow = xpos * PX + (lane >> 5) * 16;
-    auto frag_a = [&](int buf, int g9, int i) -> bf16x8 {
-        return *reinterpret_cast<const bf16x8*>(smA(buf) + (i * 32 + (lane & 31)) * PA + g9 * 32 + (lane >> 5) * 16);
-    };
-    auto frag_b = [&](int buf, int dt, int g9, int j) -> bf16x8 {
-        const int dh = g9 / 3, dw = g9 - dh * 3;
-        const unsigned char* src;
-        if (PX == 48) {
-            src = smX(buf) + xrow + (j * 32 + (dh - 1) * W + (dw - 1)) * PX;
-        } else {
-            const int p = xpos + j * 32 + (dh - 1) * W + (dw - 1);
-            src = smX(buf) + p * PX + ((((lane >> 5) ^ (p >> 3)) & 1) << 4);
-        }
-        const bool ok = ((tmask[j] >> dt) & 1u) && ((hwmask[j] >> g9) & 1u);
-        return *reinterpret_cast<const bf16x8*>(ok ? src : smZero);
-    };
-    auto kstep = [&](int s, auto CUR, auto OTHER) {
-        const int buf = s & 1;
-        const int dt = s % 3;
-        const int sn = s + 1 < nsteps ? s + 1 : s;
-        const int sx = XPF2 ? (s + 2 < nsteps ? s + 2 : nsteps - 1) : sn;
-        bf16x8 avA[WM], bvA[WN], avB[WM], bvB[WN];
-#pragma unroll
-        for (int i = 0; i < WM; ++i) avA[i] = frag_a(buf, 0, i);
-#pragma unroll
-        for (int j = 0; j < WN; ++j) bvA[j] = frag_b(buf, dt, 0, j);
-#pragma unroll
-        for (int g9 = 0; g9 < 9; ++g9) {
-            if (g9 == 0) load_x(sx, OTHER);
-            if (g9 == 1) load_a(sn);
-            bf16x8 (&av)[WM] = (g9 & 1) ? avB : avA;
-            bf16x8 (&bv)[WN] = (g9 & 1) ? bvB : bvA;
-            bf16x8 (&avn)[WM] = (g9 & 1) ? avA : avB;
-            bf16x8 (&bvn)[WN] = (g9 & 1) ? bvA : bvB;
-            int n = 0;
-#pragma unroll
-            for (int i = 0; i < WM; ++i)
-#pragma unroll
-                for (int j = 0; j < WN; ++j) {
-                    acc[i][j] = __builtin_amdgcn_mfma_f32_32x32x16_bf16(av[i], bv[j], acc[i][j], 0, 0, 0);
-                    if (g9 < 8) {
-                        if (n < WM) avn[n] = frag_a(buf, g9 + 1, n);
-                        else if (n < WM + WN) bvn[n - WM] = frag_b(buf, dt, g9 + 1, n - WM);
-                    }
-                    ++n;
-                }
-            if (WM * WN < WM + WN && g9 < 8) {
-#pragma unroll
-                for (int r = WM * WN; r < WM + WN; ++r) {
-                    if (r < WM) avn[r] = frag_a(buf, g9 + 1, r);
-                    else bvn[r - WM] = frag_b(buf, dt, g9 + 1, r - WM);
-                }
-            }
-            __builtin_amdgcn_sched_barrier(0);
-        }
-        store(buf ^ 1, sn, CUR);
-        __syncthreads();
-    };
-    if constexpr (XPF2) {
-        for (int s = 0; s < nsteps; s += 2) {
-            kstep(s, Set1{}, Set0{});
-            if (s + 1 < nsteps) kstep(s + 1, Set0{}, Set1{});
-        }
+#define OTAL_DIRECT_TILE xcd_tile(true)
+#include "conv3_direct_body.inc"
+#undef OTAL_DIRECT_TILE
+}
+
+constexpr bool GROUP_A_FIRST = true;
+template <int BMA, int BMB, int MODE, int BNP, bool XPF2A, bool H>
+__global__ __launch_bounds__(BNP * 2, 1) void conv3_direct_group_kernel(const DirectArgs a, const DirectArgs b, const int tiles_a) {
+    static_assert(2 * sizeof(DirectArgs) + sizeof(int) <= 4096, "kernel arguments stay under 4 KB");
+    const int tiles_b = (int)gridDim.x - tiles_a;
+    const int gya = (a.c.M + BMA - 1) / BMA, gyb = (b.c.M + BMB - 1) / BMB;
+    const GroupTile t = GROUP_A_FIRST ? group_tile(blockIdx.x, tiles_a, gya, tiles_b, gyb) : group_tile(blockIdx.x, tiles_b, gyb, tiles_a, gya);
+#define OTAL_DIRECT_TILE (TileId{t.x, t.y, 0})
+    constexpr int WN = 1, PX = 48;
+    if ((t.problem == 0) == GROUP_A_FIRST) {
+        constexpr int BM = BMA;
+        constexpr bool XPF2 = XPF2A;
+        const DirectArgs& d = a;
+#include "conv3_direct_body.inc"
     } else {
-        for (int s = 0; s < nsteps; ++s) kstep(s, Set0{}, Set0{});
-    }
-    if ((MODE == MODE_FWD && a.half) || (MODE == MODE_DGRAD && a.xhalf)) {
-        constexpr int PT = BNP * 2 + 16;
-        static_assert(BM * PT + BM * 8 <= 2 * BM * PA + 2 * SPAN_MAX * PX, "staging tile fits in the operand buffers");
-        unsigned char* tile = dsm;
-        float* rows = reinterpret_cast<float*>(dsm + BM * PT);
-        __syncthreads();
-        for (int r = tid; r < BM; r += DNT) {
-            const int m = m0 + r;
-            if constexpr (MODE == MODE_FWD) {
-                rows[2 * r] = (m < a.M && a.scale) ? a.scale[m] : 1.f;
-                rows[2 * r + 1] = (m < a.M && a.shift) ? a.shift[m] : 0.f;
-            } else {
-                rows[2 * r] = (m < a.M && a.escale) ? a.escale[m] : 1.f;
-                rows[2 * r + 1] = 0.f;
-            }
-        }
-        __syncthreads();
-        const bool relu = MODE == MODE_FWD && (a.flags & EPI_RELU) != 0;
-#pragma unroll
-        for (int i = 0; i < WM; ++i)
-#pragma unroll
-            for (int j = 0; j < WN; ++j) {
-                const int nl = (wave * WN + j) * 32 + (lane & 31);
-#pragma unroll
-                for (int r = 0; r < 16; ++r) {
-                    const int lr = i * 32 + (r & 3) + 8 * (r >> 2) + 4 * (lane >> 5);
-                    float v = acc[i][j][r] * rows[2 * lr] + rows[2 * lr + 1];
-                    if (relu) v = fmaxf(v, 0.f);
-                    *reinterpret_cast<unsigned short*>(tile + lr * PT + nl * 2) = (unsigned short)(cvt_pk_bf16(v, 0.f) & 0xffffu);
-                }
-            }
-        __syncthreads();
-        unsigned short* yh = reinterpret_cast<unsigned short*>(a.out);
-        const unsigned short* mk = MODE == MODE_DGRAD ? reinterpret_cast<const unsigned short*>(a.emask) : nullptr;
-        const int64_t ocs = MODE == MODE_FWD ? g.y_cs : g.x_cs;
-        const int64_t ybase = (int64_t)bsm * (MODE == MODE_FWD ? g.y_bs : g.x_bs) + p0;
-        constexpr int U = 4;
-        for (int p0 = tid; p0 < BM * (BNP / 8); p0 += U * DNT) {
-            int64_t off[U];
-            bool ok[U];
-            Words4 m4[U];
-#pragma unroll
-            for (int u = 0; u < U; ++u) {
-                const int p = p0 + u * DNT;
-                const int row = p / (BNP / 8), q = p - row * (BNP / 8);
-                ok[u] = p < BM * (BNP / 8) && m0 + row < a.M && n0 + q * 8 < a.N;
-                off[u] = ok[u] ? ybase + (int64_t)(m0 + row) * ocs + q * 8 : 0;
-                if (mk) m4[u] = *reinterpret_cast<const Words4*>(mk + off[u]);
-            }
-#pragma unroll
-            for (int u = 0; u < U; ++u) {
-                if (!ok[u]) continue;
-                const int p = p0 + u * DNT;
-                const int row = p / (BNP / 8), q = p - row * (BNP / 8);
-                Words4 v = *reinterpret_cast<const Words4*>(tile + row * PT + q * 16);
-                if (mk) {
-                    v.a &= bf16_relu_mask2(m4[u].a); v.b &= bf16_relu_mask2(m4[u].b);
-                    v.c &= bf16_relu_mask2(m4[u].c); v.d &= bf16_relu_mask2(m4[u].d);
-                }
-                *reinterpret_cast<Words4*>(yh + off[u]) = v;
-            }
-        }
-        return;
-    }
-    store_acc<MODE, WM, WN, BM>(a, acc, m0, n0, 0, wave * WN * 32, lane, 0, reinterpret_cast<float*>(smA(0)));
+        constexpr int BM = BMB;
+        constexpr bool XPF2 = false;
+        const DirectArgs& d = b;
+#include "conv3_direct_body.inc"
+    }
+#undef OTAL_DIRECT_TILE
 }
 
 template <int MODE>
@@ -2726,7 +2471,7 @@
 }
 
 template <int MODE, bool H = false>
-int launch_direct(ConvArgs& a, void* ws, size_t ws_bytes, hipStream_t st) {
+int prepare_direct(ConvArgs& a, void* ws, size_t ws_bytes, hipStream_t st, DirectArgs& d) {
     if (H && ((a.g.Wi & 1) || (a.flags & EPI_ACCUM))) return OTAL_E_UNSUPPORTED;
     const int C = MODE == MODE_FWD ? a.g.Cin : a.g.Cout;
     const int BM = direct_bm(a.g, a.M);
@@ -2742,7 +2487,6 @@
                            a.M, Mpad, C, a.w_natural, make_fastdiv((uint32_t)(C * 27 / 2)));
         if (int e = otal_launch_status()) return e;
     }
-    DirectArgs d;
     a.fd = make_conv_fastdiv(a.g);
     a.src_bytes = (unsigned)gather_extent_bytes(a.g, MODE, H ? 2 : 4);
     a.splits = 1; a.k_per_split = 0; a.slab = nullptr;
@@ -2750,6 +2494,15 @@
     d.c = a;
     d.wp = reinterpret_cast<const unsigned short*>(ws);
     d.C = C; d.Ktot = C * 27; d.wp_bytes = (unsigned)wb;
+    return 0;
+}
+
+template <int MODE, bool H = false>
+int launch_direct(ConvArgs& a, void* ws, size_t ws_bytes, hipStream_t st) {
+    DirectArgs d;
+    if (int e = prepare_direct<MODE, H>(a, ws, ws_bytes, st, d)) return e;
+    const int BM = direct_bm(a.g, a.M);
+    const int tm = (a.M + BM - 1) / BM;
     const int bnp = direct_bnp(a.g, a.M);
     if (bnp == 128) {
         const dim3 grid(a.N / 128, tm, 1);
@@ -2758,23 +2511,56 @@
         else hipLaunchKernelGGL((conv3_direct_kernel<64, MODE, 128, 1, 48, 1, false, H>), grid, dim3(256), (direct_lds_bytes<64, 128, 48, H>()), st, d);
         return otal_launch_status();
     }
-    const int xpf2 = OTAL_OPT("OTAL_CONV_DIRECT_XPF2");
     if (bnp == 512) {
         const dim3 grid(a.N / 512, tm, 1);
         if constexpr (MODE == MODE_FWD) {
-            if (BM == 96 && (xpf2 & 2)) return launch_direct512<96, MODE, true, H>(d, grid, st);
+            if (BM == 96 && (OTAL_OPT("OTAL_CONV_DIRECT_XPF2") & 2)) return launch_direct512<96, MODE, true, H>(d, grid, st);
         }
         if (BM == 96) return launch_direct512<96, MODE, false, H>(d, grid, st);
         return launch_direct512<64, MODE, false, H>(d, grid, st);
     }
     const dim3 grid(a.N / 256, tm, 1);
-    if (BM == 96 && (xpf2 & 1)) hipLaunchKernelGGL((conv3_direct_kernel<96, MODE, 256, 1, 48, 1, true, H>), grid, dim3(512), (direct_lds_bytes<96, 256, 48, H>()), st, d);
-    else if (BM == 64 && ((xpf2 & 4) || ((xpf2 & 1) && (int64_t)grid.x * grid.y <= 256))) hipLaunchKernelGGL((conv3_direct_kernel<64, MODE, 256, 1, 48, 1, true, H>), grid, dim3(512), (direct_lds_bytes<64, 256, 48, H>()), st, d);
+    const bool x2 = direct_xpf2_256(BM, (int64_t)grid.x * grid.y);
+    if (BM == 96 && x2) hipLaunchKernelGGL((conv3_direct_kernel<96, MODE, 256, 1, 48, 1, true, H>), grid, dim3(512), (direct_lds_bytes<96, 256, 48, H>()), st, d);
+    else if (BM == 64 && x2) hipLaunchKernelGGL((conv3_direct_kernel<64, MODE, 256, 1, 48, 1, true, H>), grid, dim3(512), (direct_lds_bytes<64, 256, 48, H>()), st, d);
     else if (BM == 96) hipLaunchKernelGGL((conv3_direct_kernel<96, MODE, 256, 1, 48, 1, false, H>), grid, dim3(512), (direct_lds_bytes<96, 256, 48, H>()), st, d);
     else if (BM == 32) hipLaunchKernelGGL((conv3_direct_kernel<32, MODE, 256, 1, 48, 1, false, H>), grid, dim3(512), (direct_lds_bytes<32, 256, 48, H>()), st, d);
     else hipLaunchKernelGGL((conv3_direct_kernel<64, MODE, 256, 1, 48, 1, false, H>), grid, dim3(512), (direct_lds_bytes<64, 256, 48, H>()), st, d);
     return otal_launch_status();
 }
+
+#if OTAL_CONV_PART == 1
+template <int BMA, int BNP, bool XPF2A>
+static int launch_direct_group_kernel(const DirectArgs& da, const DirectArgs& db, int tiles_a, int tiles_b, hipStream_t st) {
+    constexpr int la = direct_lds_bytes<BMA, BNP, 48, true>(), lb = direct_lds_bytes<32, BNP, 48, true>();
+    constexpr int lds = la > lb ? la : lb;
+    static bool configured = false;
+    if (!configured) {
+        hipError_t e = hipFuncSetAttribute(reinterpret_cast<const void*>(conv3_direct_group_kernel<BMA, 32, MODE_DGRAD, BNP, XPF2A, true>),
+                                           hipFuncAttributeMaxDynamicSharedMemorySize, lds);
+        if (e != hipSuccess) return (int)e;
+        configured = true;
+    }
+    hipLaunchKernelGGL((conv3_direct_group_kernel<BMA, 32, MODE_DGRAD, BNP, XPF2A, true>), dim3(tiles_a + tiles_b), dim3(BNP * 2),
+                       lds, st, da, db, tiles_a);
+    return otal_launch_status();
+}
+}
+int otal_conv::launch_direct_group_half(ConvArgs& a, ConvArgs& b, const int* plan, void* ws, size_t ws_bytes, hipStream_t st) {
+    const int bm_a = plan[0], bnp = plan[1], xpf2_a = plan[2], ta = plan[3], tb = plan[4];
+    const size_t wa = a.pre ? 0 : direct_wp_bytes(a.g, a.M, a.g.Cout);
+    if (wa && (!ws || ws_bytes < wa)) return OTAL_E_UNSUPPORTED;
+    DirectArgs da, db;
+    if (int e = prepare_direct<MODE_DGRAD, true>(a, ws, ws_bytes, st, da)) return e;
+    if (int e = prepare_direct<MODE_DGRAD, true>(b, ws ? reinterpret_cast<char*>(ws) + wa : nullptr, ws ? ws_bytes - wa : 0, st, db)) return e;
+    if (bnp == 128 && bm_a == 96) return launch_direct_group_kernel<96, 128, false>(da, db, ta, tb, st);
+    if (bnp != 256) return OTAL_E_UNSUPPORTED;
+    if (bm_a == 96) return xpf2_a ? launch_direct_group_kernel<96, 256, true>(da, db, ta, tb, st) : launch_direct_group_kernel<96, 256, false>(da, db, ta, tb, st);
+    if (bm_a == 64) return xpf2_a ? launch_direct_group_kernel<64, 256, true>(da, db, ta, tb, st) : launch_direct_group_kernel<64, 256, false>(da, db, ta, tb, st);
+    return OTAL_E_UNSUPPORTED;
+}
+namespace {
+#endif
 
 #include "conv_wgrad_direct.inc"
 #include "conv1d_tile.inc"
@@ -2984,13 +2770,11 @@
     return launch_mode<MODE_FWD>(a, precision, ws, ws_bytes, (hipStream_t)stream);
 }
 
-extern "C" int otal_conv_dgrad(const int* geom, const int64_t* strides, const float* dy, const float* wt_packed,
-                               float* dx, int accumulate, const float* out_mask, const float* out_scale,
-                               int precision, const void* prologue, void* ws, size_t ws_bytes, void* stream) {
-    g_last_kernel = "";
+namespace {
+int fill_dgrad_args(ConvArgs& a, const int* geom, const int64_t* strides, const float* dy, const float* wt_packed, float* dx,
+                    int accumulate, const float* out_mask, const float* out_scale, int precision, const void* prologue) {
     if (!geom || !strides || !dy || !wt_packed || !dx) return OTAL_E_NULL;
     if ((out_mask == nullptr) != (out_scale == nullptr)) return OTAL_E_NULL;
-    ConvArgs a = {};
     if (int e = fill_geom(a.g, geom)) return e;
     a.g.x_bs = strides[0]; a.g.x_cs = strides[1]; a.g.y_bs = strides[2]; a.g.y_cs = strides[3];
     a.dy = dy; a.w = wt_packed; a.out = dx;
@@ -3006,7 +2790,48 @@
     if ((a.half || a.xhalf || a.mhalf) && !a.prec) return OTAL_E_UNSUPPORTED;
     if (a.half != a.xhalf || (a.mhalf && !a.xhalf) || (out_mask && a.xhalf && !a.mhalf)) return OTAL_E_UNSUPPORTED;
     a.pre = prologue;
+    return 0;
+}
+ConvQuery dgrad_query(const ConvArgs& a, int precision) {
+    ConvQuery q = {};
+    q.g = a.g;
+    q.mode = MODE_DGRAD;
+    q.precision = precision;
+    q.accumulate = (a.flags & EPI_ACCUM) ? 1 : 0;
+    q.has_mask = a.emask ? 1 : 0;
+    q.w = (uintptr_t)a.w; q.dy = (uintptr_t)a.dy; q.out = (uintptr_t)a.out; q.mask = (uintptr_t)a.emask;
+    return q;
+}
+}
+
+extern "C" int otal_conv_dgrad(const int* geom, const int64_t* strides, const float* dy, const float* wt_packed,
+                               float* dx, int accumulate, const float* out_mask, const float* out_scale,
+                               int precision, const void* prologue, void* ws, size_t ws_bytes, void* stream) {
+    g_last_kernel = "";
+    ConvArgs a = {};
+    if (int e = fill_dgrad_args(a, geom, strides, dy, wt_packed, dx, accumulate, out_mask, out_scale, precision, prologue)) return e;
     return launch_mode<MODE_DGRAD>(a, precision, ws, ws_bytes, (hipStream_t)stream);
+}
+
+extern "C" int otal_conv_dgrad_group(const int* const* geom, const int64_t* const* strides, const float* const* dy,
+                                     const float* const* w, float* const* dx, const float* const* out_mask,
+                                     const float* const* out_scale, int precision, const void* const* prologue, void* ws,
+                                     size_t ws_bytes, void* stream) {
+    g_last_kernel = "";
+    if (!geom || !strides || !dy || !w || !dx) return OTAL_E_NULL;
+    ConvArgs a[2] = {};
+    for (int i = 0; i < 2; ++i)
+        if (int e = fill_dgrad_args(a[i], geom[i], strides[i], dy[i], w[i], dx[i], 0, out_mask ? out_mask[i] : nullptr,
+                                    out_scale ? out_scale[i] : nullptr, precision, prologue ? prologue[i] : nullptr)) return e;
+    const ConvQuery qa = dgrad_query(a[0], precision), qb = dgrad_query(a[1], precision);
+    const DirectGroupPlan p = direct_group_plan(qa, qb);
+    if (!p.ok) return OTAL_E_UNSUPPORTED;
+    if (conv_plan(qa).prologue != PRO_DIRECT) a[0].pre = nullptr;
+    if (conv_plan(qb).prologue != PRO_DIRECT) a[1].pre = nullptr;
+    const int plan[5] = {p.bm_a, p.bnp, p.xpf2_a, p.tiles_a, p.tiles_b};
+    const int e = otal_conv::launch_direct_group_half(a[0], a[1], plan, ws, ws_bytes, (hipStream_t)stream);
+    if (e == 0) g_last_kernel = "direct+direct";
+    return e;
 }
 
 extern "C" int otal_conv_wgrad(const int* geom, const int64_t* strides, const float* x, const float* dy,
diff --git a/opental_amd/csrc/conv_index.h b/opental_amd/csrc/conv_index.h
--- a/opental_amd/csrc/conv_index.h
+++ b/opental_amd/csrc/conv_index.h
@@ -152,6 +152,23 @@
     return (int64_t)i.b * g.x_bs + (int64_t)ci * g.x_cs + ((int64_t)i.t * g.Hi + i.h) * g.Wi + i.w;
 }
 
+struct GroupTile { int problem, x, y; };
+OTAL_HD int group_xcd_below(int v, int k) { return (v >> 3) * k + ((v & 7) < k ? (v & 7) : k); }
+OTAL_HD int group_xcd_rank(int v, int k) { return (v + 7 - k) >> 3; }
+OTAL_HD int group_logical_tile(int id, int s, int e) {
+    const int k = id & 7;
+    return group_xcd_below(e, k) - group_xcd_below(s, k) + group_xcd_rank(id, k) - group_xcd_rank(s, k);
+}
+OTAL_HD GroupTile group_tile(int id, int n_first, int gy_first, int n_second, int gy_second) {
+    GroupTile t;
+    t.problem = id < n_first ? 0 : 1;
+    const int l = t.problem ? group_logical_tile(id, n_first, n_first + n_second) : group_logical_tile(id, 0, n_first);
+    const int gy = t.problem ? gy_second : gy_first;
+    t.y = l % gy;
+    t.x = l / gy;
+    return t;
+}
+
 inline void same_pad(int size, int k, int s, int& front, int& out) {
     int total = (size % s == 0) ? (k - s) : (k - size % s);
     if (total < 0) total = 0;
diff --git a/opental_amd/csrc/conv_select.h b/opental_amd/csrc/conv_select.h
--- a/opental_amd/csrc/conv_select.h
+++ b/opental_amd/csrc/conv_select.h
@@ -174,6 +174,12 @@
 static inline size_t direct_wp_bytes(const ConvGeom& g, int M, int C) {
     const int BM = direct_bm(g, M);
     return align256((size_t)((M + BM - 1) / BM * BM) * C * 27 * 2 + 1024);
+}
+static inline bool direct_xpf2_256(int BM, int64_t tiles) {
+    const int xpf2 = OTAL_OPT("OTAL_CONV_DIRECT_XPF2");
+    if (BM == 96) return (xpf2 & 1) != 0;
+    if (BM == 64) return (xpf2 & 4) || ((xpf2 & 1) && tiles <= 256);
+    return false;
 }
 
 static inline bool wgrad_direct_eligible(const ConvGeom& g, int prec, const void* x, const void* dy) {
@@ -354,6 +360,33 @@
     return p;
 }
 
+struct DirectGroupPlan {
+    int ok;
+    int bm_a, bm_b, bnp;
+    int xpf2_a;
+    int tiles_a, tiles_b;
+};
+static inline DirectGroupPlan direct_group_plan(const ConvQuery& a, const ConvQuery& b) {
+    DirectGroupPlan p = {};
+    if (OTAL_OPT("OTAL_CONV_NOGROUP")) return p;
+    if (a.mode != MODE_DGRAD || b.mode != MODE_DGRAD || a.precision != b.precision || !(a.precision & 8)) return p;
+    if (a.accumulate || b.accumulate) return p;
+    const ConvGeom &ga = a.g, &gb = b.g;
+    if (ga.B != gb.B || ga.Ti != gb.Ti || ga.Hi != gb.Hi || ga.Wi != gb.Wi || ga.Cin < gb.Cin) return p;
+    const ConvPlan pa = conv_plan(a), pb = conv_plan(b);
+    if (!pa.n || !pb.n || pa.step[0].kernel != CK_DIRECT || pb.step[0].kernel != CK_DIRECT) return p;
+    p.bm_a = direct_bm(ga, ga.Cin);
+    p.bm_b = direct_bm(gb, gb.Cin);
+    p.bnp = direct_bnp(ga, ga.Cin);
+    if (p.bm_b != 32 || !(p.bnp == 256 ? (p.bm_a == 64 || p.bm_a == 96) : (p.bnp == 128 && p.bm_a == 96))) return p;
+    const int64_t nt = (int64_t)ga.B * conv_in_positions(ga) / p.bnp;
+    const int64_t ta = (ga.Cin + p.bm_a - 1) / p.bm_a * nt, tb = (gb.Cin + p.bm_b - 1) / p.bm_b * nt;
+    p.tiles_a = (int)ta; p.tiles_b = (int)tb;
+    p.xpf2_a = p.bnp == 256 && direct_xpf2_256(p.bm_a, ta) ? 1 : 0;
+    p.ok = 1;
+    return p;
+}
+
 static inline int conv_half_storage(const ConvGeom& g, int mode, int precision) {
     if (!(precision & 1) || g.y_bs % 8 || g.y_cs % 8) return 0;
     ConvQuery q = {};
diff --git a/opental_amd/csrc/options.h b/opental_amd/csrc/options.h
--- a/opental_amd/csrc/options.h
+++ b/opental_amd/csrc/options.h
@@ -7,11 +7,12 @@
     {"OTAL_CONV_DIRECT_XPF2", 3},         {"OTAL_CONV_NO1A", 0},
     {"OTAL_CONV_NO1AW", 0},               {"OTAL_CONV_NO1DTILE", 0},
     {"OTAL_CONV_NO1X1STREAM", 0},         {"OTAL_CONV_NODIRECT", 0},
-    {"OTAL_CONV_NOPROJ", 0},              {"OTAL_CONV_NOPROJW", 0},
-    {"OTAL_CONV_NOW1D", 0},               {"OTAL_CONV_NOW1X1", 0},
-    {"OTAL_CONV_NOWDIRECT", 0},           {"OTAL_LOSS_NOSTAGE", 0},
-    {"OTAL_POOL_NO133", 0},               {"OTAL_POOL_NOROWS", 0},
-    {"OTAL_W1A_SPLITS", 0},               {"OTAL_WDIRECT_BLOCKS", 0},
+    {"OTAL_CONV_NOGROUP", 0},             {"OTAL_CONV_NOPROJ", 0},
+    {"OTAL_CONV_NOPROJW", 0},             {"OTAL_CONV_NOW1D", 0},
+    {"OTAL_CONV_NOW1X1", 0},              {"OTAL_CONV_NOWDIRECT", 0},
+    {"OTAL_LOSS_NOSTAGE", 0},             {"OTAL_POOL_NO133", 0},
+    {"OTAL_POOL_NOROWS", 0},              {"OTAL_W1A_SPLITS", 0},
+    {"OTAL_WDIRECT_BLOCKS", 0},
 };
 constexpr int OTAL_NUM_OPTIONS = sizeof(OTAL_OPTIONS) / sizeof(OTAL_OPTIONS[0]);
 constexpr bool otal_streq(const char* a, const char* b) { return *a == *b && (*a == 0 || otal_streq(a + 1, b + 1)); }
```
